# DecaYale/RSLO

Hardware: AMD Instinct MI355X
Metric: frame-pairs/sec fwd+bwd (synthetic KITTI-shaped ~122k-pt scans) (higher is better)
Workload: dtype f32; 1 GPU; C3: full fwd+bwd (voxelize + GU encoder + BEV head/vote + chamfer/ICP loss + Adam step), bs=4 frame pairs/GPU, fp32, 64-ring scans (~122412 pts/frame), dp1; frame_pairs_per_gpu=4, points_per_frame=122412, voxelize_in_step=True, voxelize_prefetch_stream=True, distinct_batches=3, optimizer_in_step=True, head_graph=fwd

## Files before the change

### include/rslo_hip.h

```cpp
#ifndef RSLO_HIP_H_
#define RSLO_HIP_H_

#include <stddef.h>
#include <stdint.h>

#ifdef __cplusplus
extern "C" {
#endif

#if defined(__GNUC__)
#define RSLO_API __attribute__((visibility("default")))
#else
#define RSLO_API
#endif

#define RSLO_OK 0
#define RSLO_EINVAL (-1)
#define RSLO_ELAUNCH (-2)
#define RSLO_ERANGE (-3)
#define RSLO_EWS (-4)

RSLO_API int rslo_abi_version(void);
RSLO_API const char *rslo_last_error(void);

RSLO_API size_t rslo_voxelize_ws_bytes(int64_t P);
RSLO_API int rslo_voxelize(const float *points, int64_t P, int F, const float *h_range6,
                  const float *h_vsize3, const int32_t *h_grid_xyz, int T, int max_voxels,
                  void *ws, size_t ws_bytes, float *voxels ,
                  int32_t *coords , int32_t *num_points ,
                  int32_t *d_nvox , void *stream);

RSLO_API int rslo_vfe_mean(const float *voxels , const int32_t *num_points , int64_t M,
                  int T, int F, float *out , void *stream);

RSLO_API int64_t rslo_hash_capacity(int64_t n);
RSLO_API int rslo_hash_build(const int32_t *coords , int64_t N, int B, const int32_t *h_dims3,
                    uint32_t *keys, int32_t *vals, int64_t cap, void *stream);
RSLO_API int rslo_rulebook_subm(const int32_t *coords, int64_t N, int B, const int32_t *h_dims3,
                       const int32_t *h_ks3, const uint32_t *keys, const int32_t *vals, int64_t cap,
                       int32_t *nbr , void *stream);
RSLO_API int64_t rslo_conv_bitmap_words(int B, const int32_t *h_out_dims3);
RSLO_API size_t rslo_scan_ws_bytes(int64_t n);
RSLO_API int rslo_conv_out_count(const int32_t *coords_in, int64_t N, int B, const int32_t *h_ks3,
                        const int32_t *h_stride3, const int32_t *h_pad3, const int32_t *h_out_dims3,
                        uint32_t *bitmap , int32_t *word_prefix , int64_t words,
                        void *scan_ws, size_t scan_ws_bytes, int32_t *d_count , void *stream);
RSLO_API int rslo_conv_out_coords(const uint32_t *bitmap, const int32_t *word_prefix, int64_t words, int B,
                         const int32_t *h_out_dims3, int32_t *out_coords , int64_t M,
                         void *stream);
RSLO_API int rslo_rulebook_conv(const int32_t *coords_out, int64_t M, int B, const int32_t *h_in_dims3,
                       const int32_t *h_ks3, const int32_t *h_stride3, const int32_t *h_pad3,
                       const uint32_t *in_keys, const int32_t *in_vals, int64_t in_cap,
                       int32_t *nbr , void *stream);
RSLO_API int rslo_rulebook_conv_T(const int32_t *coords_in, int64_t N, int B, const int32_t *h_out_dims3,
                         const int32_t *h_ks3, const int32_t *h_stride3, const int32_t *h_pad3,
                         const uint32_t *out_keys, const int32_t *out_vals, int64_t out_cap,
                         int32_t *nbrT , void *stream);

RSLO_API int rslo_spconv_fwd(const float *in, int cin, const float *W, const float *bias, const int32_t *nbr,
                    const int32_t *row_order, int64_t n_out, int K, int cout, int flip_k, float act_slope,
                    float *out, const int32_t *n_live_dev, void *stream);
RSLO_API int rslo_spconv_dgrad(const float *dout, int cout, const float *W, const int32_t *nbrT,
                      const int32_t *row_order, int64_t n_in, int K, int cin, int flip_k, float *din, void *stream);
RSLO_API int rslo_weight_transpose(const float *W, int K, int cin, int cout, float *Wt, void *stream);
RSLO_API size_t rslo_weight_split_bytes(int K, int cin, int cout);
RSLO_API int rslo_weight_split(const float *W, int K, int cin_op, int cout_op, int transpose, void *Ws, void *stream);
typedef struct {
  const float *W;
  void *ws_fwd;
  void *ws_dgrad;
  int32_t K, cin, cout;
} RsloWeightSplitDesc;
RSLO_API int rslo_weight_split_many(const RsloWeightSplitDesc *desc_dev, int n_layers, int64_t max_weight_elems,
                                    void *stream);
RSLO_API int rslo_spconv_fwd_split(const float *in, int cin, const void *Ws, const float *bias, const int32_t *nbr,
                                   const int32_t *row_order, int64_t n_out, int K, int cout, int flip_k,
                                   float act_slope, float *out, const int32_t *n_live_dev, void *stream);
RSLO_API int rslo_tuning_set(const char *name, int value);
RSLO_API int rslo_tuning_get(const char *name, int *value);
RSLO_API const char *rslo_tuning_name(int index);
RSLO_API int rslo_weight_to_bf16(const float *W, int K, int cin_op, int cout_op, int transpose, void *Wb, void *stream);
RSLO_API int rslo_spconv_fwd_bf16(const void *in, int cin, const void *Wb, const float *bias, const int32_t *nbr,
                                  const int32_t *row_order, int64_t n_out, int K, int cout, int flip_k,
                                  float act_slope, void *out, void *stream);
RSLO_API int64_t rslo_leaky_bwd_colsum_bf16_blocks(int64_t rows, int cols);
RSLO_API int rslo_leaky_bwd_colsum_bf16(const void *y, const void *dout, int64_t rows, int cols, float slope, void *g,
                                        float *partial, void *stream);
RSLO_API int rslo_spconv_wgrad_pairs_bf16(const void *in, int cin, const void *dout, int cout, const int32_t *pairs_in,
                                          const int32_t *pairs_out, const int32_t *koff, int64_t n_out, int K, void *ws,
                                          size_t ws_bytes, float *dW, float *dbias, const float *bias_partial,
                                          int n_bias_partial, void *stream);
RSLO_API size_t rslo_spconv_wgrad_ws_bytes(int64_t n_out, int K, int cin, int cout);
RSLO_API int rslo_spconv_wgrad(const float *in, int cin, const float *dout, int cout, const int32_t *nbr,
                      int64_t n_out, int K, void *ws, size_t ws_bytes, float *dW ,
                      float *dbias , void *stream);
RSLO_API int rslo_rulebook_row_order(const int32_t *nbr, int64_t n_rows, int K, int flip_k, int32_t *order,
                                     void *stream);
RSLO_API size_t rslo_rulebook_pairs_ws_bytes(int64_t n_rows, int K);
RSLO_API int rslo_rulebook_pairs(const int32_t *nbr, int64_t n_rows, int K, void *ws, size_t ws_bytes,
                        int32_t *pairs_in, int32_t *pairs_out, int32_t *koff , void *stream);
RSLO_API int rslo_tq_normalize_fwd(const float *tq, int B, int64_t cells, float *out, void *stream);
RSLO_API int rslo_tq_normalize_bwd(const float *tq, const float *grad, int B, int64_t cells, float *dtq, void *stream);
RSLO_API int rslo_conf_softmax_fwd(const float *t_logit, const float *r_logit, const unsigned char *outside, int B,
                                   int cells, float temperature, float *t_conf, float *r_conf, float *conf_temp,
                                   void *stream);
RSLO_API int rslo_conf_softmax_bwd(const float *t_conf, const float *r_conf, const float *g_t, const float *g_r,
                                   const unsigned char *outside, int B, int cells, float *d_t_logit, float *d_r_logit,
                                   void *stream);
typedef struct {
  const float *mask;
  const float *conf;
  const float *tq, *tq_g;
  const float *pred[3];
  float *w[4];
  float *occ[4];
  float *mpred[3];
  float *mtq, *mtq_g;
  int32_t B, H, W, levels;
} RsloHeadMasks;
typedef struct {
  const float *mask;
  const float *occ[4];
  const float *g_mpred[3];
  const float *g_mtq;
  float *d_pred[3];
  float *d_tq;
  int32_t B, H, W, levels;
} RsloHeadMasksBwd;
RSLO_API int rslo_head_masks_fwd(const RsloHeadMasks *h_a, void *stream);
RSLO_API int rslo_head_masks_bwd(const RsloHeadMasksBwd *h_a, void *stream);
RSLO_API int rslo_cat_upsample_fwd(const float *a, const float *b, int B, int Ca, int Cb, int H, int W, int scale, float *out,
                                   void *stream);
RSLO_API int rslo_cat_upsample_bwd(const float *grad, int B, int Ca, int Cb, int H, int W, int scale, float *da, float *db,
                                   void *stream);
RSLO_API int rslo_pose_tail_fwd(const float *odom, int B, float *t, float *r, void *stream);
RSLO_API int rslo_pose_tail_bwd(const float *odom, const float *g_t, const float *g_r, int B, float *d_odom, void *stream);

#define RSLO_LOSS_TAIL_MAX_LEVELS 8
#define RSLO_LOSS_TAIL_ALPHA_STRIDE 4
typedef struct {
  const float *t_pred, *t_tgt;
  const float *q_pred, *q_tgt;
  const float *alpha_T, *alpha_R;
  const float *pyr_loss_b;
  const float *alpha_pT, *alpha_pR;
  const float *pair_loss;
  const float *alpha_C;
  int32_t B, L, n_pairs, reserved;
  float w_T, w_R, w_pT, w_pR;
  float c_scale;
  float level_w[RSLO_LOSS_TAIL_MAX_LEVELS];
} RsloLossTail;
RSLO_API int rslo_loss_tail_fwd(const RsloLossTail *h_p, float *out5, void *stream);
RSLO_API int rslo_loss_tail_bwd(const RsloLossTail *h_p, const float *grad_out , float *d_t ,
                                float *d_q , float *d_pyr , float *d_pair ,
                                float *d_alpha5 , void *stream);

#define RSLO_PLAN_MAX_LEVELS 8
#define RSLO_PLAN_MAX_CLOUDS 64
#define RSLO_PLAN_CNT_OVERFLOW 0
#define RSLO_PLAN_CNT_ROWS 1
#define RSLO_PLAN_CNT_RAW 9
#define RSLO_PLAN_CNT_NVOX 32
#define RSLO_PLAN_CNT_BASE 96
#define RSLO_PLAN_CNT_BOFF 176
#define RSLO_PLAN_CNT_WORDS (176 + RSLO_PLAN_MAX_LEVELS * (RSLO_PLAN_MAX_CLOUDS + 1))
typedef struct {
  int32_t n_levels;
  int32_t dims0[3];
  int32_t subm_ks[RSLO_PLAN_MAX_LEVELS][3];
  int32_t conv_ks[RSLO_PLAN_MAX_LEVELS][3], conv_stride[RSLO_PLAN_MAX_LEVELS][3], conv_pad[RSLO_PLAN_MAX_LEVELS][3];
  int32_t want_pairs, want_orders;
  float range6[6], vsize3[3];
  int32_t grid_xyz[3], max_points, max_voxels, n_features;
  int64_t cap_rows[RSLO_PLAN_MAX_LEVELS];
} RsloEncoderSpec;
typedef struct {
  uint64_t total_bytes;
  int32_t dims[RSLO_PLAN_MAX_LEVELS][3];
  int64_t cap_rows[RSLO_PLAN_MAX_LEVELS], hash_cap[RSLO_PLAN_MAX_LEVELS];
  uint64_t counts_off;
  uint64_t voxels_off, num_points_off;
  uint64_t coords_frame_off;
  uint64_t coords_off[RSLO_PLAN_MAX_LEVELS];
  uint64_t keys_off[RSLO_PLAN_MAX_LEVELS], vals_off[RSLO_PLAN_MAX_LEVELS];
  uint64_t subm_nbr_off[RSLO_PLAN_MAX_LEVELS], subm_pin_off[RSLO_PLAN_MAX_LEVELS], subm_pout_off[RSLO_PLAN_MAX_LEVELS],
      subm_koff_off[RSLO_PLAN_MAX_LEVELS];
  uint64_t conv_nbr_off[RSLO_PLAN_MAX_LEVELS], conv_nbrT_off[RSLO_PLAN_MAX_LEVELS], conv_order_off[RSLO_PLAN_MAX_LEVELS],
      conv_pin_off[RSLO_PLAN_MAX_LEVELS], conv_pout_off[RSLO_PLAN_MAX_LEVELS], conv_koff_off[RSLO_PLAN_MAX_LEVELS];
  int64_t scratch_words;
  uint64_t vox_ws_off, bitmap_off, prefix_off, scan_ws_off, pair_ws_off;
  uint64_t keys_end_off;
  uint64_t bitmap_level_off[RSLO_PLAN_MAX_LEVELS], bitmap_end_off;
} RsloPlanLayout;
RSLO_API int rslo_plan_encoder_layout(const RsloEncoderSpec *h_spec, int n_clouds, const int64_t *h_n_points,
                                      RsloPlanLayout *h_layout);
RSLO_API int rslo_plan_encoder(const RsloEncoderSpec *h_spec, const RsloPlanLayout *h_layout, int n_clouds,
                               int clouds_per_frame, const float *const *h_points ,
                               const int64_t *h_n_points, void *arena, size_t arena_bytes,
                               int32_t *h_counts , void *stream);

RSLO_API int rslo_plan_encoder_pad_tails(const RsloEncoderSpec *h_spec, const RsloPlanLayout *h_layout, void *arena,
                                         void *stream);

RSLO_API size_t rslo_spconv_wgrad_pairs_ws_bytes(int64_t n_out, int K, int cin, int cout);
RSLO_API int rslo_spconv_wgrad_pairs(const float *in, int cin, const float *dout, int cout, const int32_t *pairs_in,
                            const int32_t *pairs_out, const int32_t *koff, int64_t n_out, int K, void *ws,
                            size_t ws_bytes, float *dW , float *dbias ,
                            const float *bias_partial ,
                            int n_bias_partial, void *stream);
RSLO_API int rslo_leaky_bwd(const float *y, const float *dout, int64_t n, float slope, float *g, void *stream);
RSLO_API int64_t rslo_leaky_bwd_colsum_blocks(int64_t rows, int cols);
RSLO_API int rslo_leaky_bwd_colsum(const float *y, const float *dout, int64_t rows, int cols, float slope, float *g,
                                   float *partial, void *stream);

RSLO_API size_t rslo_segbn_ws_bytes(int S, int64_t max_seg_len, int C);
RSLO_API int rslo_segbn_fwd(const float *x, int C, const int32_t *seg_off, int S, int64_t max_seg_len,
                   const float *gamma, const float *beta, float *running_mean ,
                   float *running_var , float momentum, float eps, float act_slope, void *ws,
                   size_t ws_bytes, float *y, float *save_mean, float *save_invstd, void *stream);
RSLO_API int rslo_bn1d_eval_act(const float *x, int64_t n, int C, const float *running_mean, const float *running_var,
                                const float *gamma, const float *beta, float eps, float act_slope, const int32_t *n_live_dev,
                                float *y, void *stream);
RSLO_API int rslo_segbn_bwd(const float *x, const float *y, const float *gy, int C, const int32_t *seg_off, int S,
                   int64_t max_seg_len, const float *gamma, const float *save_mean, const float *save_invstd,
                   float act_slope, void *ws, size_t ws_bytes, float *gx, float *dgamma, float *dbeta,
                   void *stream);

RSLO_API int rslo_dense_scatter(const float *feat, const int32_t *coords, int64_t M, int C, int B,
                       const int32_t *h_dims3, float *out, void *stream);
RSLO_API int rslo_dense_gather(const float *dense, const int32_t *coords, int64_t M, int C, int B,
                      const int32_t *h_dims3, float *dfeat, void *stream);
RSLO_API int rslo_dense_scatter_frames(const float *feat, const int32_t *coords, int64_t M, int C, int B, int frames,
                                       const int32_t *h_dims3, float *out, void *stream);
RSLO_API int rslo_dense_gather_frames(const float *dense, const int32_t *coords, int64_t M, int C, int B, int frames,
                                      const int32_t *h_dims3, float *dfeat, void *stream);
RSLO_API int rslo_bev_channel_sums(const float *in, int B, int G, int Cg, int64_t HW, float *out, void *stream);
RSLO_API int rslo_bev_channel_sums_masks(const float *in, int B, int G, int Cg, int64_t HW, float *out, float *mask_f,
                                         unsigned char *mask_b, unsigned char *outside_b, void *stream);
RSLO_API size_t rslo_bev_display_ws_bytes(int T);
RSLO_API int rslo_bev_display(const float *sums, int B, int T, int Cg, int64_t HW, float *mask, float *disp, void *ws,
                              size_t ws_bytes, void *stream);

RSLO_API size_t rslo_chamfer_ws_bytes(int B, int N, int M);
RSLO_API int rslo_chamfer_nn(const float *xyz1 , const float *xyz2 , int B, int N, int M,
                    float *dist , int32_t *idx , void *ws, size_t ws_bytes,
                    void *stream);
RSLO_API int rslo_chamfer_nn_ragged(const float *xyz1, const float *xyz2, int B, int N, int M, const int32_t *ncnt,
                           const int32_t *mcnt, float *dist, int32_t *idx, void *ws, size_t ws_bytes,
                           void *stream);
RSLO_API int rslo_chamfer_brute_nn(const float *xyz1, const float *xyz2, int B, int N, int M, const int32_t *ncnt,
                                   const int32_t *mcnt, float *dist, int32_t *idx, void *ws, size_t ws_bytes,
                                   void *stream);
RSLO_API size_t rslo_chamfer_grid_ws_bytes(int B, int N, int M);
RSLO_API int rslo_chamfer_grid_nn(const float *xyz1, const float *xyz2, int B, int N, int M, const int32_t *ncnt,
                                  const int32_t *mcnt, float *dist, int32_t *idx, void *ws, size_t ws_bytes,
                                  void *stream);
RSLO_API int rslo_chamfer_grad(const float *xyz1, const float *xyz2, int B, int N, int M,
                      const float *graddist1, const int32_t *idx1, float *gradxyz1 ,
                      float *gradxyz2 , void *stream);

RSLO_API size_t rslo_cov_residual_ws_bytes(int B, int N);
RSLO_API int rslo_cov_residual_fwd(const float *p1, const float *tgt, const float *cov1, const float *cov2,
                          const int32_t *idx, const float *dist, const float *thr, const float *Rd, int B, int N,
                          int M, float reg_weight, void *ws, size_t ws_bytes, float *loss ,
                          float *cnt , void *stream);
RSLO_API int rslo_cov_residual_bwd(const float *p1, const float *tgt, const float *cov1, const float *cov2,
                          const int32_t *idx, const float *dist, const float *thr, const float *Rd,
                          const float *gloss , const float *cnt , int B, int N, int M,
                          float reg_weight, float *gp1 , float *gtgt ,
                          float *gcov1 , float *gcov2 , void *ws, size_t ws_bytes, void *stream);
RSLO_API size_t rslo_cov_residual_bwd_ws_bytes(int B, int N, int M);
RSLO_API size_t rslo_icp_ws_bytes(int B, int N);
RSLO_API int rslo_icp_step(const float *p1, const float *n1, const float *tgt, const int32_t *idx, const float *dist,
                  const float *thr, int B, int N, int M, void *ws, size_t ws_bytes, float *res_r ,
                  float *res_t , float *step_R , float *step_t ,
                  void *stream);
RSLO_API int rslo_icp_step_first(const float *p1, const float *n1, const float *tgt, const int32_t *idx, const float *dist,
                  const float *thr, int B, int N, int M, void *ws, size_t ws_bytes, float *res_r ,
                  float *res_t , float *step_R , float *step_t ,
                  void *stream);
RSLO_API int rslo_roi_threshold(const float *dist, int B, int N, const int32_t *counts, double ratio, float *thr,
                                void *stream);
RSLO_API int rslo_transform_points(const float *x, const float *R, const float *t, int B, int M, float *out,
                          void *stream);
RSLO_API int rslo_transform_rows(const float *x, int row_stride, const float *R, const float *t, int B, int M,
                                 float *out, void *stream);
RSLO_API size_t rslo_transform_rows_bwd_ws_bytes(int B, int M);
RSLO_API int rslo_transform_rows_bwd(const float *x, int row_stride, const float *gout, int B, int M, void *ws,
                                     size_t ws_bytes, int32_t *done, float *dR, float *dt, void *stream);

typedef struct {
  const float *pred;
  const float *mask;
  float *dpred;
  int32_t h, w, mask_channels;
} RsloPyramidLevel;
RSLO_API size_t rslo_pyramid_l2_ws_bytes(const RsloPyramidLevel *h_levels, int n_levels, int B);
RSLO_API int rslo_pyramid_l2_fwd(const RsloPyramidLevel *h_levels, int n_levels, int B, const float *tq, int H0,
                                 int W0, const float *h_origin3, const float *h_vsize3, void *ws, size_t ws_bytes,
                                 int32_t *done, float *loss_b, float *den, void *stream);
RSLO_API int rslo_pyramid_l2_bwd(const RsloPyramidLevel *h_levels, int n_levels, int B, const float *tq, int H0,
                                 int W0, const float *h_origin3, const float *h_vsize3, const float *grad_loss_b,
                                 const float *den, void *stream);

RSLO_API int rslo_pad_rows_fwd(const float *src, int64_t N, int C, const int32_t *off, const int32_t *len, int B,
                               int Lmax, float *out, void *stream);
RSLO_API int rslo_pad_rows_bwd(const float *dout, int64_t N, int C, const int32_t *off, const int32_t *len, int B,
                               int Lmax, float *dsrc, void *stream);
RSLO_API int rslo_pair_rows_fwd(const float *feats, int64_t N, int F, const float *conf, int Cc, const int32_t *off,
                                const int32_t *len, int B, int Lmax, float *xyz, float *nrm, float *cov, void *stream);

RSLO_API size_t rslo_bn2d_ws_bytes(int N, int C, int HW);
RSLO_API int rslo_bn2d_stats(const float *x, int N, int C, int HW, void *ws, size_t ws_bytes, int32_t *done,
                             double *stats, void *stream);
RSLO_API int rslo_bn2d_apply(const float *x, const float *res, const double *stats, const float *gamma,
                             const float *beta, int N, int C, int HW, float eps, float momentum, float act_slope,
                             float *running_mean, float *running_var, float *save_mean, float *save_invstd, float *y,
                             void *stream);
RSLO_API int rslo_bn2d_bwd_reduce(const float *dy, const float *y, const float *x, const float *save_mean,
                                  const float *save_invstd, int N, int C, int HW, float act_slope, int has_act,
                                  void *ws, size_t ws_bytes, int32_t *done, double *red, float *dgamma, float *dbeta,
                                  void *stream);
RSLO_API int rslo_bn2d_bwd_apply(const float *dy, const float *y, const float *x, const float *gamma,
                                 const float *save_mean, const float *save_invstd, const double *red, double count,
                                 const double *count_dev ,
                                 int N, int C, int HW, float act_slope, int has_act, float *dx, float *dres,
                                 void *stream);

RSLO_API int rslo_bn2d_fwd_local(const float *x, const float *res, const float *gamma, const float *beta, int N, int C,
                                 int HW, float eps, float momentum, float act_slope, float *running_mean,
                                 float *running_var, float *save_mean, float *save_invstd, float *y, void *ws,
                                 size_t ws_bytes, void *stream);
RSLO_API int rslo_bn2d_bwd_local(const float *dy, const float *y, const float *x, const float *gamma,
                                 const float *save_mean, const float *save_invstd, int N, int C, int HW,
                                 float act_slope, int has_act, float *dx, float *dres, float *dgamma, float *dbeta,
                                 void *ws, size_t ws_bytes, void *stream);

RSLO_API size_t rslo_vote_ws_bytes(int B, int H, int W);
RSLO_API int rslo_vote_fwd(const float *tq_map, const float *t_conf, const float *r_conf, int B, int H, int W,
                           const float *h_origin3, const float *h_vsize3, void *ws, size_t ws_bytes, int32_t *done,
                           float *tq_map_g, float *odom, float *sums, void *stream);
RSLO_API int rslo_vote_bwd(const float *tq_map, const float *t_conf, const float *r_conf, int B, int H, int W,
                           const float *h_origin3, const float *h_vsize3, const float *odom, const float *sums,
                           const float *g_odom, float *d_tq_map, float *d_t_conf, float *d_r_conf, void *stream);

RSLO_API int rslo_conv2d_wgrad_supported(int cin, int cout, int H, int W, int stride);
RSLO_API size_t rslo_conv2d_wgrad_ws_bytes(int B, int cin, int cout, int H, int W, int stride);
RSLO_API int rslo_conv2d_wgrad(const float *in, const float *dout, int B, int cin, int cout, int H, int W, int stride,
                               float *dW, float *dbias, void *ws, size_t ws_bytes, void *stream);

RSLO_API int rslo_conv2d_fwd_supported(int cin, int cout, int H, int W);
RSLO_API size_t rslo_conv2d_wsplit_bytes(int cin, int cout);
RSLO_API int rslo_conv2d_wsplit(const float *W, int cin, int cout, int transpose, void *Ws, void *stream);
typedef struct {
  const float *W;
  void *ws_fwd;
  void *ws_dgrad;
  int32_t cin, cout;
  int32_t ntap;
  int32_t reserved;
} RsloConv2dSplitDesc;
RSLO_API int rslo_conv2d_wsplit_many(const RsloConv2dSplitDesc *desc_dev, int n_layers, int64_t max_weight_elems,
                                     void *stream);
RSLO_API int rslo_conv2d_fwd(const float *in, const void *Ws, const float *bias, int B, int cin, int cout, int H, int W,
                             float *out, void *stream);
RSLO_API int rslo_conv2d_fwd_add(const float *in, const void *Ws, const float *bias, const float *res, int B, int cin,
                                 int cout, int H, int W, float *out, void *stream);
RSLO_API size_t rslo_opl_bytes(int B, int C, int H, int W);
RSLO_API int rslo_opl_from_nchw(const float *in, int B, int C, int H, int W, void *planes, void *stream);
RSLO_API int rslo_conv2d_fwd_p_supported(int cin, int cout, int H, int W);
RSLO_API int rslo_conv2d_fwd_p(const void *planes, const void *Ws, const float *bias, const float *res ,
                               int B, int cin, int cout, int H, int W, float *out, void *stream);
RSLO_API int rslo_conv2d_s2_supported(int cin, int cout, int ksize);
RSLO_API int rslo_conv2d_wsplit_k(const float *W, int cin, int cout, int ksize, int transpose, void *Ws, void *stream);
RSLO_API int rslo_conv2d_fwd_s2(const float *in, const void *Ws, int B, int cin, int cout, int H, int W, int ksize,
                                float *out, void *stream);
RSLO_API int rslo_conv2d_dgrad_s2(const float *dout, const void *Ws, int B, int cin, int cout, int H, int W, int ksize,
                                  float *din, void *stream);
RSLO_API int rslo_conv2d_dgrad_s2_add(const float *dout, const void *Ws, const float *res, int B, int cin, int cout, int H,
                                      int W, int ksize, float *din, void *stream);
RSLO_API int rslo_conv2d_fwd_bn(const float *in, const void *Ws, const float *bias, const float *scale, const float *shift,
                                const float *res, int B, int cin, int cout, int H, int W, int act, float slope, float *out,
                                void *stream);
RSLO_API int rslo_conv2d_fwd_s2_bn(const float *in, const void *Ws, const float *bias, const float *scale,
                                   const float *shift, const float *res, int B, int cin, int cout, int H, int W, int ksize,
                                   int act, float slope, float *out, void *stream);
typedef struct {
  const float *gamma, *beta;
  const float *mean, *var;
  float *scale, *shift;
  int32_t C;
  float eps;
} RsloBnFoldDesc;
RSLO_API int rslo_bn_fold_many(const RsloBnFoldDesc *desc_dev, int n_layers, int max_c, void *stream);
RSLO_API int rslo_pose_chain(const float *t, const float *q, double *state, int32_t *count, float *rel_rows, double *traj,
                             int cap, void *stream);
RSLO_API int rslo_conv2d_fwd_bf16(const float *in, const void *Ws, const float *bias, int B, int cin, int cout, int H,
                                  int W, float *out, void *stream);
RSLO_API int rslo_conv1x1s2_wgrad_supported(int cin, int cout, int H, int W);
RSLO_API size_t rslo_conv1x1s2_wgrad_ws_bytes(int B, int cin, int cout, int H, int W);
RSLO_API int rslo_conv1x1s2_wgrad(const float *in, const float *dout, int B, int cin, int cout, int H, int W, float *dW,
                                  void *ws, size_t ws_bytes, void *stream);
RSLO_API int rslo_conv2d_fwd_add_bf16(const float *in, const void *Ws, const float *bias, const float *res, int B,
                                      int cin, int cout, int H, int W, float *out, void *stream);
RSLO_API int rslo_conv2d_wgrad_bf16(const float *in, const float *dout, int B, int cin, int cout, int H, int W,
                                    int stride, float *dW, float *dbias, void *ws, size_t ws_bytes, void *stream);

RSLO_API int rslo_conv1x1_supported(int cin, int cout);
RSLO_API int rslo_conv1x1_fwd(const float *x, const float *W, const float *bias, int B, int cin, int cout, int HW,
                              float *out, void *stream);
RSLO_API int rslo_conv1x1_dgrad(const float *dy, const float *W, int B, int cin, int cout, int HW, float *dx, void *stream);
RSLO_API size_t rslo_conv1x1_wgrad_ws_bytes(int B, int cin, int cout, int HW);
RSLO_API int rslo_conv1x1_wgrad(const float *x, const float *dy, int B, int cin, int cout, int HW, float *dW, float *dbias,
                                void *ws, size_t ws_bytes, void *stream);

RSLO_API int rslo_quat_to_rot(const float *q_wxyz, int B, float *R, void *stream);
RSLO_API int rslo_quat_to_rot_bwd(const float *q_wxyz, const float *gR, int B, float *gq, void *stream);
RSLO_API int rslo_pose_targets(const float *res_r, const float *res_t, const float *R_pred, const float *T_pred, int B,
                               float *rot_targets_wxyz, float *trans_targets, void *stream);
RSLO_API int rslo_pose_targets_tq(const float *res_r, const float *res_t, const float *R_pred, const float *T_pred, int B,
                                  float *rot_targets_wxyz, float *trans_targets, float *tq, void *stream);

typedef struct {
  float *param, *grad, *exp_avg, *exp_avg_sq, *step;
  int32_t group;
  int32_t step_offset;
} RsloOptTensor;
typedef struct {
  int32_t tensor, count;
  int64_t offset;
} RsloOptChunk;
typedef struct {
  double lr, beta1, beta2, eps, weight_decay;
} RsloOptGroup;
#define RSLO_OPT_MAX_GROUPS 16
typedef struct {
  RsloOptGroup group[RSLO_OPT_MAX_GROUPS];
} RsloOptHyper;
RSLO_API int rslo_opt_clip_grad_norm(const RsloOptTensor *tensors_dev, const RsloOptChunk *chunks_dev, int n_chunks,
                                     float max_norm, double *partial_ws, float *total_norm, void *stream);
RSLO_API int rslo_opt_adam_step(const RsloOptTensor *tensors_dev, const RsloOptChunk *chunks_dev, int n_chunks,
                                const RsloOptHyper *hyper, float step, void *stream);

typedef struct RsloWgradReduce {
  int32_t kind;
  int32_t n_blocks;
  const void *ws;
  void *dW;
  const void *aux;
  void *dbias;
  const void *koff;
  int32_t p[8];
} RsloWgradReduce;
RSLO_API int rslo_wgrad_reduce_defer(RsloWgradReduce *sink, int capacity, int *count);
RSLO_API int rslo_wgrad_reduce_many(const RsloWgradReduce *reduces, int n, void *stream);

RSLO_API int rslo_peer_create_host(const char *name, int rank, int world, int max_n, void **comm_out);
RSLO_API int rslo_peer_host_unlink(void *comm);
RSLO_API int rslo_peer_ipc_handle_bytes(void);
RSLO_API int rslo_peer_create_device_begin(int rank, int world, int max_n, void **comm_out, void *handle_out);
RSLO_API int rslo_peer_create_device_finish(void *comm, const void *all_handles);
RSLO_API int rslo_peer_set_timeout_ms(void *comm, int ms);
RSLO_API int rslo_peer_allreduce_f64(void *comm, double *t, int n, void *stream);
RSLO_API unsigned long long rslo_peer_status(void *comm, int *peer);
RSLO_API int rslo_peer_wait_samples(void *comm, float *out_us, int max_out);
RSLO_API int rslo_bn2d_peer_supported(int N, int C, int HW);
RSLO_API int rslo_bn2d_fwd_peer(void *comm, const float *x, const float *res, const float *gamma, const float *beta, int N,
                                int C, int HW, float eps, float momentum, float act_slope, float *running_mean,
                                float *running_var, float *save_mean, float *save_invstd, double *count_out, float *y,
                                void *stream);
RSLO_API int rslo_bn2d_bwd_peer(void *comm, const float *dy, const float *y, const float *x, const float *gamma,
                                const float *save_mean, const float *save_invstd, const double *count_all, int N, int C,
                                int HW, float act_slope, int has_act, float *dx, float *dres, float *dgamma, float *dbeta,
                                void *stream);
RSLO_API int rslo_peer_capture_begin(void *comm);
RSLO_API int rslo_peer_capture_end(void *comm, int *n_exchanges);
RSLO_API int rslo_peer_replay_prepare(void *comm, int n_exchanges, void *stream);
RSLO_API int rslo_peer_destroy(void *comm);

RSLO_API size_t rslo_normals_ws_bytes(int N);
RSLO_API int rslo_estimate_normals(const float *points, int stride_floats, int N, float radius, int max_nn,
                                   const float *h_viewpoint3, int zero_vertical, float *normals ,
                                   int32_t *counts , void *ws, size_t ws_bytes, void *stream);

RSLO_API size_t rslo_voxel_downsample_ws_bytes(int N);
RSLO_API int rslo_voxel_downsample(const float *points, int stride_floats, const float *normals ,
                                   int nstride_floats, int N, double voxel_size, float *out ,
                                   int32_t *voxel_of_point , int32_t *npts ,
                                   int32_t *counts , void *ws, size_t ws_bytes, void *stream);

#define RSLO_MAP_MAX_PROBE 128
#define RSLO_MAP_HDR_COUNTERS 8
#define RSLO_MAP_HDR_PRUNE 5
RSLO_API size_t rslo_map_bytes(int64_t capacity);
RSLO_API int rslo_map_reset(void *map, size_t map_bytes, int64_t capacity, double voxel_size, double min_range,
                            double max_range, void *stream);
RSLO_API size_t rslo_map_insert_ws_bytes(int N);
RSLO_API int rslo_map_insert(void *map, size_t map_bytes, const float *points, int stride_floats, int width, int N,
                             const double *pose7, void *ws, size_t ws_bytes, void *stream);
RSLO_API int rslo_map_lookup(const void *map, size_t map_bytes, const float *points, int stride_floats, int N,
                             const double *pose7, int32_t *hits_out , uint64_t *tags_out ,
                             void *stream);
RSLO_API int rslo_map_export(const void *map, size_t map_bytes, int min_hits, const double *center3 ,
                             double radius, float *rows , uint64_t *tags ,
                             int32_t *hits , int64_t max_rows, int64_t *counts , void *stream);
RSLO_API int rslo_map_insert_frames(void *map, size_t map_bytes, const void *store, size_t store_bytes, int64_t capacity,
                                    int K, const double *poses , int n_poses, void *stream);
RSLO_API size_t rslo_map_prune_ws_bytes(int64_t capacity);
RSLO_API int rslo_map_prune(void *map, size_t map_bytes, const double *center3 , double radius,
                            int min_hits, int grace, void *ws, size_t ws_bytes, void *stream);

#define RSLO_MAP_HDR_CARVE 14
RSLO_API int rslo_range_image(const float *points, int stride_floats, int N, int H, int W, double tan_lo, double tan_hi,
                              uint32_t *img , void *stream);
RSLO_API size_t rslo_map_carve_ws_bytes(int64_t capacity);
RSLO_API int rslo_map_carve(void *map, size_t map_bytes, const uint32_t *img , int H, int W, double tan_lo,
                            double tan_hi, const double *pose7 , int win_rows, int win_cols, double margin_abs,
                            double margin_rel, double max_range, int grace, void *ws, size_t ws_bytes, void *stream);

RSLO_API int rslo_map_params(const void *map, size_t map_bytes, double *params3_host, void *stream);
RSLO_API int rslo_map_nearest(const void *map, size_t map_bytes, double voxel_size, const float *points,
                              int stride_floats, int N, const double *pose7, double max_dist, int min_hits,
                              int64_t *tags_out , double *d2_out , float *rows_out ,
                              void *stream);
RSLO_API size_t rslo_map_register_ws_bytes(int N);
RSLO_API int rslo_map_normal_eq(const void *map, size_t map_bytes, double voxel_size, const float *points,
                                int stride_floats, int width, int N, const double *pose7, int metric, double max_dist,
                                int min_hits, double *out29, void *ws, size_t ws_bytes, void *stream);
RSLO_API int rslo_map_register(const void *map, size_t map_bytes, double voxel_size, const float *points,
                               int stride_floats, int width, int N, double *pose7, int iters, int metric,
                               double max_dist, int min_hits, double damping, int min_pairs, double tol_t, double tol_r,
                               double *info , void *ws, size_t ws_bytes, void *stream);
RSLO_API int rslo_map_normal_eq_w(const void *map, size_t map_bytes, double voxel_size, const float *points,
                                  int stride_floats, int width, int N, const double *pose7, int metric, double max_dist,
                                  int min_hits, double robust_scale, double *out29, void *ws, size_t ws_bytes,
                                  void *stream);
RSLO_API int rslo_map_register_w(const void *map, size_t map_bytes, double voxel_size, const float *points,
                                 int stride_floats, int width, int N, double *pose7, int iters, int metric,
                                 double max_dist, int min_hits, double damping, int min_pairs, double tol_t, double tol_r,
                                 double robust_scale, double *info , void *ws, size_t ws_bytes, void *stream);
RSLO_API int rslo_map_register_sched(const void *const *maps , const size_t *map_bytes ,
                                     const double *voxel_sizes , int n_levels,
                                     const double *stages , int n_stages, const float *points,
                                     int stride_floats, int width, int N, double *pose7, int metric, int min_hits,
                                     double damping, int min_pairs, double tol_t, double tol_r,
                                     double *info , void *ws, size_t ws_bytes, void *stream);

RSLO_API size_t rslo_place_bytes(int64_t capacity, int R, int S);
RSLO_API int rslo_place_reset(void *db, size_t db_bytes, int64_t capacity, int R, int S, void *stream);
RSLO_API int rslo_place_describe(const float *points, int stride_floats, int N, int R, int S,
                                 const double *tables , float z_offset, float *D ,
                                 int32_t *key , double *norm , int64_t *counters4, void *stream);
RSLO_API int rslo_place_add(void *db, size_t db_bytes, int64_t capacity, int R, int S, const float *D,
                            const int32_t *key, const double *norm, void *stream);
RSLO_API size_t rslo_place_query_ws_bytes(int64_t capacity);
RSLO_API int rslo_place_query(const void *db, size_t db_bytes, int64_t capacity, int R, int S, const float *Dq,
                              const int32_t *keyq, const double *normq, int64_t exclude_recent, int num_candidates,
                              int top_k, double *out , void *ws, size_t ws_bytes, void *stream);

// ... 94 lines not shown
```

### rslo_amd/capi.py

```python
import ctypes as C
import os

import torch

_HERE = os.path.dirname(os.path.abspath(__file__))
LIB_PATH = os.environ.get("RSLO_HIP_LIB") or os.path.join(_HERE, "librslo_hip.so")
_lib = None

_I3 = C.c_int32 * 3
_F3 = C.c_float * 3
_F6 = C.c_float * 6

_vp, _i, _i64, _sz, _f = C.c_void_p, C.c_int, C.c_int64, C.c_size_t, C.c_float
SIGNATURES = {
    "rslo_abi_version": (C.c_int, []),
    "rslo_last_error": (C.c_char_p, []),
    "rslo_voxelize_ws_bytes": (_sz, [_i64]),
    "rslo_voxelize": (C.c_int, [_vp, _i64, _i, _vp, _vp, _vp, _i, _i, _vp, _sz, _vp, _vp, _vp, _vp, _vp]),
    "rslo_vfe_mean": (C.c_int, [_vp, _vp, _i64, _i, _i, _vp, _vp]),
    "rslo_hash_capacity": (_i64, [_i64]),
    "rslo_hash_build": (C.c_int, [_vp, _i64, _i, _vp, _vp, _vp, _i64, _vp]),
    "rslo_rulebook_subm": (C.c_int, [_vp, _i64, _i, _vp, _vp, _vp, _vp, _i64, _vp, _vp]),
    "rslo_conv_bitmap_words": (_i64, [_i, _vp]),
    "rslo_scan_ws_bytes": (_sz, [_i64]),
    "rslo_conv_out_count": (C.c_int, [_vp, _i64, _i, _vp, _vp, _vp, _vp, _vp, _vp, _i64, _vp, _sz, _vp, _vp]),
    "rslo_conv_out_coords": (C.c_int, [_vp, _vp, _i64, _i, _vp, _vp, _i64, _vp]),
    "rslo_rulebook_conv": (C.c_int, [_vp, _i64, _i, _vp, _vp, _vp, _vp, _vp, _vp, _i64, _vp, _vp]),
    "rslo_rulebook_conv_T": (C.c_int, [_vp, _i64, _i, _vp, _vp, _vp, _vp, _vp, _vp, _i64, _vp, _vp]),
    "rslo_spconv_fwd": (C.c_int, [_vp, _i, _vp, _vp, _vp, _vp, _i64, _i, _i, _i, _f, _vp, _vp, _vp]),
    "rslo_spconv_dgrad": (C.c_int, [_vp, _i, _vp, _vp, _vp, _i64, _i, _i, _i, _vp, _vp]),
    "rslo_weight_transpose": (C.c_int, [_vp, _i, _i, _i, _vp, _vp]),
    "rslo_weight_split_bytes": (_sz, [_i, _i, _i]),
    "rslo_weight_split": (C.c_int, [_vp, _i, _i, _i, _i, _vp, _vp]),
    "rslo_weight_split_many": (C.c_int, [_vp, _i, _i64, _vp]),
    "rslo_spconv_fwd_split": (C.c_int, [_vp, _i, _vp, _vp, _vp, _vp, _i64, _i, _i, _i, C.c_float, _vp, _vp, _vp]),
    "rslo_peer_create_host": (C.c_int, [C.c_char_p, _i, _i, _i, C.POINTER(C.c_void_p)]),
    "rslo_peer_host_unlink": (C.c_int, [_vp]),
    "rslo_peer_ipc_handle_bytes": (C.c_int, []),
    "rslo_peer_create_device_begin": (C.c_int, [_i, _i, _i, C.POINTER(C.c_void_p), _vp]),
    "rslo_peer_create_device_finish": (C.c_int, [_vp, _vp]),
    "rslo_peer_set_timeout_ms": (C.c_int, [_vp, _i]),
    "rslo_peer_allreduce_f64": (C.c_int, [_vp, _vp, _i, _vp]),
    "rslo_peer_status": (C.c_ulonglong, [_vp, C.POINTER(C.c_int)]),
    "rslo_peer_destroy": (C.c_int, [_vp]),
    "rslo_tuning_set": (C.c_int, [C.c_char_p, _i]),
    "rslo_tuning_get": (C.c_int, [C.c_char_p, _vp]),
    "rslo_tuning_name": (C.c_char_p, [_i]),
    "rslo_weight_to_bf16": (C.c_int, [_vp, _i, _i, _i, _i, _vp, _vp]),
    "rslo_spconv_fwd_bf16": (C.c_int, [_vp, _i, _vp, _vp, _vp, _vp, _i64, _i, _i, _i, C.c_float, _vp, _vp]),
    "rslo_spconv_wgrad_ws_bytes": (_sz, [_i64, _i, _i, _i]),
    "rslo_spconv_wgrad": (C.c_int, [_vp, _i, _vp, _i, _vp, _i64, _i, _vp, _sz, _vp, _vp, _vp]),
    "rslo_rulebook_row_order": (C.c_int, [_vp, _i64, _i, _i, _vp, _vp]),
    "rslo_leaky_bwd_colsum_bf16_blocks": (_i64, [_i64, _i]),
    "rslo_leaky_bwd_colsum_bf16": (C.c_int, [_vp, _vp, _i64, _i, C.c_float, _vp, _vp, _vp]),
    "rslo_spconv_wgrad_pairs_bf16": (C.c_int, [_vp, _i, _vp, _i, _vp, _vp, _vp, _i64, _i, _vp, _sz, _vp, _vp, _vp, _i,
                                               _vp]),
    "rslo_rulebook_pairs_ws_bytes": (_sz, [_i64, _i]),
    "rslo_rulebook_pairs": (C.c_int, [_vp, _i64, _i, _vp, _sz, _vp, _vp, _vp, _vp]),
    "rslo_spconv_wgrad_pairs_ws_bytes": (_sz, [_i64, _i, _i, _i]),
    "rslo_spconv_wgrad_pairs": (C.c_int, [_vp, _i, _vp, _i, _vp, _vp, _vp, _i64, _i, _vp, _sz, _vp, _vp, _vp, _i, _vp]),
    "rslo_leaky_bwd_colsum_blocks": (_i64, [_i64, _i]),
    "rslo_leaky_bwd_colsum": (C.c_int, [_vp, _vp, _i64, _i, C.c_float, _vp, _vp, _vp]),
    "rslo_leaky_bwd": (C.c_int, [_vp, _vp, _i64, _f, _vp, _vp]),
    "rslo_segbn_ws_bytes": (_sz, [_i, _i64, _i]),
    "rslo_segbn_fwd": (C.c_int, [_vp, _i, _vp, _i, _i64, _vp, _vp, _vp, _vp, _f, _f, _f, _vp, _sz, _vp, _vp, _vp, _vp]),
    "rslo_segbn_bwd": (C.c_int, [_vp, _vp, _vp, _i, _vp, _i, _i64, _vp, _vp, _vp, _f, _vp, _sz, _vp, _vp, _vp, _vp]),
    "rslo_dense_scatter": (C.c_int, [_vp, _vp, _i64, _i, _i, _vp, _vp, _vp]),
    "rslo_dense_gather": (C.c_int, [_vp, _vp, _i64, _i, _i, _vp, _vp, _vp]),
    "rslo_dense_scatter_frames": (C.c_int, [_vp, _vp, _i64, _i, _i, _i, _vp, _vp, _vp]),
    "rslo_dense_gather_frames": (C.c_int, [_vp, _vp, _i64, _i, _i, _i, _vp, _vp, _vp]),
    "rslo_bev_channel_sums": (C.c_int, [_vp, _i, _i, _i, _i64, _vp, _vp]),
    "rslo_chamfer_ws_bytes": (_sz, [_i, _i, _i]),
    "rslo_chamfer_nn": (C.c_int, [_vp, _vp, _i, _i, _i, _vp, _vp, _vp, _sz, _vp]),
    "rslo_chamfer_nn_ragged": (C.c_int, [_vp, _vp, _i, _i, _i, _vp, _vp, _vp, _vp, _vp, _sz, _vp]),
    "rslo_chamfer_brute_nn": (C.c_int, [_vp, _vp, _i, _i, _i, _vp, _vp, _vp, _vp, _vp, _sz, _vp]),
    "rslo_chamfer_grid_ws_bytes": (_sz, [_i, _i, _i]),
    "rslo_chamfer_grid_nn": (C.c_int, [_vp, _vp, _i, _i, _i, _vp, _vp, _vp, _vp, _vp, _sz, _vp]),
    "rslo_chamfer_grad": (C.c_int, [_vp, _vp, _i, _i, _i, _vp, _vp, _vp, _vp, _vp]),
    "rslo_cov_residual_ws_bytes": (_sz, [_i, _i]),
    "rslo_cov_residual_fwd": (C.c_int, [_vp] * 8 + [_i, _i, _i, _f, _vp, _sz, _vp, _vp, _vp]),
    "rslo_cov_residual_bwd": (C.c_int, [_vp] * 10 + [_i, _i, _i, _f, _vp, _vp, _vp, _vp, _vp, _sz, _vp]),
    "rslo_cov_residual_bwd_ws_bytes": (_sz, [_i, _i, _i]),
    "rslo_icp_ws_bytes": (_sz, [_i, _i]),
    "rslo_icp_step": (C.c_int, [_vp] * 6 + [_i, _i, _i, _vp, _sz, _vp, _vp, _vp, _vp, _vp]),
    "rslo_icp_step_first": (C.c_int, [_vp] * 6 + [_i, _i, _i, _vp, _sz, _vp, _vp, _vp, _vp, _vp]),
    "rslo_transform_points": (C.c_int, [_vp, _vp, _vp, _i, _i, _vp, _vp]),
    "rslo_transform_rows": (C.c_int, [_vp, _i, _vp, _vp, _i, _i, _vp, _vp]),
    "rslo_transform_rows_bwd_ws_bytes": (_sz, [_i, _i]),
    "rslo_transform_rows_bwd": (C.c_int, [_vp, _i, _vp, _i, _i, _vp, _sz, _vp, _vp, _vp, _vp]),
    "rslo_bn2d_ws_bytes": (_sz, [_i, _i, _i]),
    "rslo_bn2d_stats": (C.c_int, [_vp, _i, _i, _i, _vp, _sz, _vp, _vp, _vp]),
    "rslo_bn2d_apply": (C.c_int, [_vp, _vp, _vp, _vp, _vp, _i, _i, _i, C.c_float, C.c_float, C.c_float, _vp, _vp, _vp,
                                  _vp, _vp, _vp]),
    "rslo_bn2d_bwd_reduce": (C.c_int, [_vp, _vp, _vp, _vp, _vp, _i, _i, _i, C.c_float, _i, _vp, _sz, _vp, _vp, _vp, _vp,
                                       _vp]),
    "rslo_bn2d_bwd_apply": (C.c_int, [_vp, _vp, _vp, _vp, _vp, _vp, _vp, C.c_double, _vp, _i, _i, _i, C.c_float, _i, _vp,
                                      _vp, _vp]),
    "rslo_bn2d_fwd_local": (C.c_int, [_vp, _vp, _vp, _vp, _i, _i, _i, C.c_float, C.c_float, C.c_float, _vp, _vp, _vp, _vp,
                                      _vp, _vp, _sz, _vp]),
    "rslo_bn2d_bwd_local": (C.c_int, [_vp, _vp, _vp, _vp, _vp, _vp, _i, _i, _i, C.c_float, _i, _vp, _vp, _vp, _vp, _vp,
                                      _sz, _vp]),
    "rslo_roi_threshold": (C.c_int, [_vp, _i, _i, _vp, C.c_double, _vp, _vp]),
    "rslo_vote_ws_bytes": (_sz, [_i, _i, _i]),
    "rslo_vote_fwd": (C.c_int, [_vp, _vp, _vp, _i, _i, _i, _vp, _vp, _vp, _sz, _vp, _vp, _vp, _vp, _vp]),
    "rslo_vote_bwd": (C.c_int, [_vp, _vp, _vp, _i, _i, _i, _vp, _vp, _vp, _vp, _vp, _vp, _vp, _vp, _vp]),
    "rslo_conv2d_wgrad_supported": (C.c_int, [_i, _i, _i, _i, _i]),
    "rslo_conv2d_wgrad_ws_bytes": (_sz, [_i, _i, _i, _i, _i, _i]),
    "rslo_conv1x1s2_wgrad_supported": (C.c_int, [_i, _i, _i, _i]),
    "rslo_conv1x1s2_wgrad_ws_bytes": (_sz, [_i, _i, _i, _i, _i]),
    "rslo_conv1x1s2_wgrad": (C.c_int, [_vp, _vp, _i, _i, _i, _i, _i, _vp, _vp, _sz, _vp]),
    "rslo_conv2d_wgrad": (C.c_int, [_vp, _vp, _i, _i, _i, _i, _i, _i, _vp, _vp, _vp, _sz, _vp]),
    "rslo_conv2d_fwd_supported": (C.c_int, [_i, _i, _i, _i]),
    "rslo_conv2d_wsplit_bytes": (_sz, [_i, _i]),
    "rslo_conv2d_wsplit": (C.c_int, [_vp, _i, _i, _i, _vp, _vp]),
    "rslo_conv2d_wsplit_k": (C.c_int, [_vp, _i, _i, _i, _i, _vp, _vp]),
    "rslo_conv2d_s2_supported": (C.c_int, [_i, _i, _i]),
    "rslo_conv2d_fwd_s2": (C.c_int, [_vp, _vp, _i, _i, _i, _i, _i, _i, _vp, _vp]),
    "rslo_conv2d_dgrad_s2": (C.c_int, [_vp, _vp, _i, _i, _i, _i, _i, _i, _vp, _vp]),
    "rslo_conv2d_wsplit_many": (C.c_int, [_vp, _i, _i64, _vp]),
    "rslo_conv2d_fwd": (C.c_int, [_vp, _vp, _vp, _i, _i, _i, _i, _i, _vp, _vp]),
    "rslo_conv2d_fwd_bf16": (C.c_int, [_vp, _vp, _vp, _i, _i, _i, _i, _i, _vp, _vp]),
    "rslo_cat_upsample_fwd": (C.c_int, [_vp, _vp, _i, _i, _i, _i, _i, _i, _vp, _vp]),
    "rslo_cat_upsample_bwd": (C.c_int, [_vp, _i, _i, _i, _i, _i, _i, _vp, _vp, _vp]),
    "rslo_bev_channel_sums_masks": (C.c_int, [_vp, _i, _i, _i, C.c_int64, _vp, _vp, _vp, _vp, _vp]),
    "rslo_pose_tail_fwd": (C.c_int, [_vp, _i, _vp, _vp, _vp]),
    "rslo_pose_tail_bwd": (C.c_int, [_vp, _vp, _vp, _i, _vp, _vp]),
    "rslo_bev_display_ws_bytes": (_sz, [_i]),
    "rslo_bev_display": (C.c_int, [_vp, _i, _i, _i, C.c_int64, _vp, _vp, _vp, _sz, _vp]),
    "rslo_conv2d_dgrad_s2_add": (C.c_int, [_vp, _vp, _vp, _i, _i, _i, _i, _i, _i, _vp, _vp]),
    "rslo_conv2d_fwd_add": (C.c_int, [_vp, _vp, _vp, _vp, _i, _i, _i, _i, _i, _vp, _vp]),
    "rslo_conv2d_fwd_add_bf16": (C.c_int, [_vp, _vp, _vp, _vp, _i, _i, _i, _i, _i, _vp, _vp]),
    "rslo_conv2d_wgrad_bf16": (C.c_int, [_vp, _vp, _i, _i, _i, _i, _i, _i, _vp, _vp, _vp, _sz, _vp]),
    "rslo_conv1x1_supported": (C.c_int, [_i, _i]),
    "rslo_conv1x1_fwd": (C.c_int, [_vp, _vp, _vp, _i, _i, _i, _i, _vp, _vp]),
    "rslo_conv1x1_dgrad": (C.c_int, [_vp, _vp, _i, _i, _i, _i, _vp, _vp]),
    "rslo_conv1x1_wgrad_ws_bytes": (_sz, [_i, _i, _i, _i]),
    "rslo_conv1x1_wgrad": (C.c_int, [_vp, _vp, _i, _i, _i, _i, _vp, _vp, _vp, _sz, _vp]),
    "rslo_quat_to_rot": (C.c_int, [_vp, _i, _vp, _vp]),
    "rslo_quat_to_rot_bwd": (C.c_int, [_vp, _vp, _i, _vp, _vp]),
    "rslo_pose_targets": (C.c_int, [_vp, _vp, _vp, _vp, _i, _vp, _vp, _vp]),
    "rslo_pose_targets_tq": (C.c_int, [_vp, _vp, _vp, _vp, _i, _vp, _vp, _vp, _vp]),
    "rslo_pair_rows_fwd": (C.c_int, [_vp, _i64, _i, _vp, _i, _vp, _vp, _i, _i, _vp, _vp, _vp, _vp]),
    "rslo_pad_rows_fwd": (C.c_int, [_vp, _i64, _i, _vp, _vp, _i, _i, _vp, _vp]),
    "rslo_pad_rows_bwd": (C.c_int, [_vp, _i64, _i, _vp, _vp, _i, _i, _vp, _vp]),
    "rslo_pyramid_l2_ws_bytes": (_sz, [_vp, _i, _i]),
    "rslo_pyramid_l2_fwd": (C.c_int, [_vp, _i, _i, _vp, _i, _i, _vp, _vp, _vp, _sz, _vp, _vp, _vp, _vp]),
    "rslo_pyramid_l2_bwd": (C.c_int, [_vp, _i, _i, _vp, _i, _i, _vp, _vp, _vp, _vp, _vp]),
    "rslo_plan_encoder_layout": (C.c_int, [_vp, _i, _vp, _vp]),
    "rslo_plan_encoder_pad_tails": (C.c_int, [_vp, _vp, _vp, _vp]),
    "rslo_plan_encoder": (C.c_int, [_vp, _vp, _i, _i, _vp, _vp, _vp, _sz, _vp, _vp]),
    "rslo_tq_normalize_fwd": (C.c_int, [_vp, _i, _i64, _vp, _vp]),
    "rslo_tq_normalize_bwd": (C.c_int, [_vp, _vp, _i, _i64, _vp, _vp]),
    "rslo_conf_softmax_fwd": (C.c_int, [_vp, _vp, _vp, _i, _i, _f, _vp, _vp, _vp, _vp]),
    "rslo_conf_softmax_bwd": (C.c_int, [_vp, _vp, _vp, _vp, _vp, _i, _i, _vp, _vp, _vp]),
    "rslo_head_masks_fwd": (C.c_int, [_vp, _vp]),
    "rslo_head_masks_bwd": (C.c_int, [_vp, _vp]),
    "rslo_loss_tail_fwd": (C.c_int, [_vp, _vp, _vp]),
    "rslo_loss_tail_bwd": (C.c_int, [_vp, _vp, _vp, _vp, _vp, _vp, _vp, _vp]),
    "rslo_peer_wait_samples": (C.c_int, [_vp, _vp, _i]),
    "rslo_bn1d_eval_act": (C.c_int, [_vp, _i64, _i, _vp, _vp, _vp, _vp, _f, _f, _vp, _vp, _vp]),
    "rslo_wgrad_reduce_defer": (C.c_int, [_vp, _i, _vp]),
    "rslo_wgrad_reduce_many": (C.c_int, [_vp, _i, _vp]),
    "rslo_peer_capture_begin": (C.c_int, [_vp]),
    "rslo_peer_capture_end": (C.c_int, [_vp, _vp]),
    "rslo_peer_replay_prepare": (C.c_int, [_vp, _i, _vp]),
    "rslo_bn2d_peer_supported": (C.c_int, [_i, _i, _i]),
    "rslo_bn2d_fwd_peer": (C.c_int, [_vp, _vp, _vp, _vp, _vp, _i, _i, _i, C.c_float, C.c_float, C.c_float, _vp, _vp, _vp, _vp,
                                     _vp, _vp, _vp]),
    "rslo_bn2d_bwd_peer": (C.c_int, [_vp, _vp, _vp, _vp, _vp, _vp, _vp, _vp, _i, _i, _i, C.c_float, _i, _vp, _vp, _vp, _vp,
                                     _vp]),
    "rslo_opl_bytes": (_sz, [_i, _i, _i, _i]),
    "rslo_opl_from_nchw": (C.c_int, [_vp, _i, _i, _i, _i, _vp, _vp]),
    "rslo_conv2d_fwd_p_supported": (C.c_int, [_i, _i, _i, _i]),
    "rslo_conv2d_fwd_p": (C.c_int, [_vp, _vp, _vp, _vp, _i, _i, _i, _i, _i, _vp, _vp]),
    "rslo_opt_clip_grad_norm": (C.c_int, [_vp, _vp, _i, _f, _vp, _vp, _vp]),
    "rslo_opt_adam_step": (C.c_int, [_vp, _vp, _i, _vp, _f, _vp]),
    "rslo_conv2d_fwd_bn": (C.c_int, [_vp] * 6 + [_i, _i, _i, _i, _i, _i, _f, _vp, _vp]),
    "rslo_conv2d_fwd_s2_bn": (C.c_int, [_vp] * 6 + [_i, _i, _i, _i, _i, _i, _i, _f, _vp, _vp]),
    "rslo_bn_fold_many": (C.c_int, [_vp, _i, _i, _vp]),
    "rslo_pose_chain": (C.c_int, [_vp, _vp, _vp, _vp, _vp, _vp, _i, _vp]),
    "rslo_normals_ws_bytes": (_sz, [_i]),
    "rslo_estimate_normals": (C.c_int, [_vp, _i, _i, _f, _i, _vp, _i, _vp, _vp, _vp, _sz, _vp]),
    "rslo_voxel_downsample_ws_bytes": (_sz, [_i]),
    "rslo_voxel_downsample": (C.c_int, [_vp, _i, _vp, _i, _i, C.c_double, _vp, _vp, _vp, _vp, _vp, _sz, _vp]),
    "rslo_map_bytes": (_sz, [_i64]),
    "rslo_map_reset": (C.c_int, [_vp, _sz, _i64, C.c_double, C.c_double, C.c_double, _vp]),
    "rslo_map_insert_ws_bytes": (_sz, [_i]),
    "rslo_map_insert": (C.c_int, [_vp, _sz, _vp, _i, _i, _i, _vp, _vp, _sz, _vp]),
    "rslo_map_lookup": (C.c_int, [_vp, _sz, _vp, _i, _i, _vp, _vp, _vp, _vp]),
    "rslo_map_export": (C.c_int, [_vp, _sz, _i, _vp, C.c_double, _vp, _vp, _vp, _i64, _vp, _vp]),
    "rslo_map_insert_frames": (C.c_int, [_vp, _sz, _vp, _sz, _i64, _i, _vp, _i, _vp]),
    "rslo_map_prune_ws_bytes": (_sz, [_i64]),
    "rslo_map_prune": (C.c_int, [_vp, _sz, _vp, C.c_double, _i, _i, _vp, _sz, _vp]),
    "rslo_range_image": (C.c_int, [_vp, _i, _i, _i, _i, C.c_double, C.c_double, _vp, _vp]),
    "rslo_map_carve_ws_bytes": (_sz, [_i64]),
    "rslo_map_carve": (C.c_int, [_vp, _sz, _vp, _i, _i, C.c_double, C.c_double, _vp, _i, _i, C.c_double, C.c_double,
                                 C.c_double, _i, _vp, _sz, _vp]),
    "rslo_map_params": (C.c_int, [_vp, _sz, _vp, _vp]),
    "rslo_map_nearest": (C.c_int, [_vp, _sz, C.c_double, _vp, _i, _i, _vp, C.c_double, _i, _vp, _vp, _vp, _vp]),
    "rslo_map_register_ws_bytes": (_sz, [_i]),
    "rslo_map_normal_eq": (C.c_int, [_vp, _sz, C.c_double, _vp, _i, _i, _i, _vp, _i, C.c_double, _i, _vp, _vp, _sz, _vp]),
    "rslo_map_register": (C.c_int, [_vp, _sz, C.c_double, _vp, _i, _i, _i, _vp, _i, _i, C.c_double, _i, C.c_double, _i,
                                    C.c_double, C.c_double, _vp, _vp, _sz, _vp]),
    "rslo_map_normal_eq_w": (C.c_int, [_vp, _sz, C.c_double, _vp, _i, _i, _i, _vp, _i, C.c_double, _i, C.c_double, _vp, _vp,
                                       _sz, _vp]),
    "rslo_map_register_w": (C.c_int, [_vp, _sz, C.c_double, _vp, _i, _i, _i, _vp, _i, _i, C.c_double, _i, C.c_double, _i,
                                      C.c_double, C.c_double, C.c_double, _vp, _vp, _sz, _vp]),
    "rslo_map_register_sched": (C.c_int, [_vp, _vp, _vp, _i, _vp, _i, _vp, _i, _i, _i, _vp, _i, _i, C.c_double, _i,
                                          C.c_double, C.c_double, _vp, _vp, _sz, _vp]),
    "rslo_place_bytes": (_sz, [_i64, _i, _i]),
    "rslo_place_reset": (C.c_int, [_vp, _sz, _i64, _i, _i, _vp]),
    "rslo_place_describe": (C.c_int, [_vp, _i, _i, _i, _i, _vp, _f, _vp, _vp, _vp, _vp, _vp]),
    "rslo_place_add": (C.c_int, [_vp, _sz, _i64, _i, _i, _vp, _vp, _vp, _vp]),
    "rslo_place_query_ws_bytes": (_sz, [_i64]),
    "rslo_place_query": (C.c_int, [_vp, _sz, _i64, _i, _i, _vp, _vp, _vp, _i64, _i, _i, _vp, _vp, _sz, _vp]),
    "rslo_posegraph_ws_bytes": (_sz, [_i, _i]),
    "rslo_posegraph_optimize": (C.c_int, [_vp, _vp, _i, _vp, _vp, _vp, _vp, _vp, _i, _i, _i] + [C.c_double] * 5 +
                                [_vp, _vp, _sz, _vp]),
    "rslo_posegraph_cost": (C.c_int, [_vp, _vp, _i, _vp, _vp, _vp, _vp, _vp, _i, C.c_double, _vp, _vp, _sz, _vp]),
    "rslo_posegraph_linearize": (C.c_int, [_vp, _vp, _i, _vp, _vp, _vp, _vp, _vp, _i, C.c_double, _vp, _vp, _vp, _vp, _sz,
                                           _vp]),
    "rslo_posegraph_matvec": (C.c_int, [_vp, _vp, _i, _i, C.c_double, _vp, _sz, _vp]),
    "rslo_posegraph_chain_solve": (C.c_int, [_vp, _vp, _i, _i, _vp, _sz, _vp]),
    "rslo_pose_between": (C.c_int, [_vp, _vp, _i, _vp, _vp]),
    "rslo_keyframe_bytes": (_sz, [_i64, _i]),
    "rslo_keyframe_reset": (C.c_int, [_vp, _sz, _i64, _i, _vp]),
    "rslo_keyframe_prepare_ws_bytes": (_sz, [_i]),
    "rslo_keyframe_prepare": (C.c_int, [_vp, _i, _i, _i, C.c_double, C.c_double, C.c_double, _vp, _vp, _vp, _sz, _vp]),
    "rslo_keyframe_add": (C.c_int, [_vp, _sz, _i64, _i, _vp, _vp, _vp]),
    "rslo_loop_verify": (C.c_int, [_vp, _sz, _i64, _i, _vp, _vp, _vp, _i, _vp, _vp, _i] + [C.c_double] * 4 +
                         [_i, C.c_double, _vp, _vp, _vp, _vp]),
    "rslo_loop_edges_reset": (C.c_int, [_vp, _vp, _vp, _vp, _i, _vp]),
    "rslo_loop_emit": (C.c_int, [_vp, _i, _vp, _sz, _i64, _i, _vp, _vp, _vp, _vp, _i, C.c_double, C.c_double, _vp]),
    "rslo_surfel_bytes": (_sz, [_i64]),
    "rslo_surfel_reset": (C.c_int, [_vp, _sz, _i64, C.c_double, C.c_double, C.c_double, _i, C.c_double, C.c_double, _vp]),
    "rslo_surfel_insert_ws_bytes": (_sz, [_i]),
    "rslo_surfel_insert": (C.c_int, [_vp, _sz, _vp, _i, _i, _vp, _vp, _sz, _vp]),
    "rslo_surfel_insert_frames": (C.c_int, [_vp, _sz, _vp, _sz, _i64, _i, _vp, _i, _vp]),
    "rslo_surfel_export": (C.c_int, [_vp, _sz, _i, _vp, C.c_double, _vp, _vp, _vp, _i64, _vp, _vp]),
    "rslo_surfel_nearest": (C.c_int, [_vp, _sz, C.c_double, _vp, _i, _i, _vp, C.c_double, _vp, _vp, _vp, _vp]),
    "rslo_surfel_prune_ws_bytes": (_sz, [_i64]),
    "rslo_surfel_prune": (C.c_int, [_vp, _sz, _vp, C.c_double, C.c_double, _i, _vp, _sz, _vp]),
    "rslo_surfel_register_ws_bytes": (_sz, [_i]),
    "rslo_surfel_normal_eq": (C.c_int, [_vp, _sz, C.c_double, _vp, _i, _i, _vp, C.c_double, C.c_double, _vp, _vp, _sz, _vp]),
    "rslo_surfel_register": (C.c_int, [_vp, _sz, C.c_double, _vp, _i, _i, _vp, _i, C.c_double, C.c_double, _i, C.c_double,
                                       C.c_double, C.c_double, _vp, _vp, _sz, _vp]),
    "rslo_surfel_nearest_d": (C.c_int, [_vp, _sz, C.c_double, _vp, _i, _i, _vp, C.c_double, _i, C.c_double, C.c_double, _vp,
                                        _vp, _vp, _vp, _vp]),
    "rslo_surfel_normal_eq_d": (C.c_int, [_vp, _sz, C.c_double, _vp, _i, _i, _vp, C.c_double, _i, C.c_double, C.c_double,
                                          C.c_double, _vp, _vp, _sz, _vp]),
    "rslo_surfel_register_d": (C.c_int, [_vp, _sz, C.c_double, _vp, _i, _i, _vp, _i, C.c_double, C.c_double, _i, C.c_double,
                                         C.c_double, C.c_double, _i, C.c_double, C.c_double, _vp, _vp, _sz, _vp]),
    "rslo_deskew": (C.c_int, [_vp, _i, _i, _i, _i, _vp, _vp, _vp, _vp, C.c_double, C.c_double, _i, C.c_double, _vp, _i, _vp,
                              _vp]),
}


class RsloHipError(RuntimeError):
    pass


def lib():
    global _lib
    if _lib is None:
        if not os.path.exists(LIB_PATH):
            raise RsloHipError(
                "librslo_hip.so not found at %s -- build it with `python -m rslo_amd.build` "
                "(there is no CPU fallback for the RSLO hot path)" % LIB_PATH)
        l = C.CDLL(LIB_PATH)
        for name, (res, args) in SIGNATURES.items():
            fn = getattr(l, name)
            fn.restype = res
            fn.argtypes = args
        _lib = l
    return _lib if _proxy is None else _proxy


_proxy = None


def probe_streams(on, points_only=None):
    global _proxy
    from rslo_amd import streamprobe
    if on:
        _proxy = streamprobe.LibProxy(lib() if _proxy is None else _proxy._lib, SIGNATURES, points_only)
        streamprobe.start()
    else:
        streamprobe.stop()
        _proxy = None


def tuning_set(name, value):
    _chk(lib().rslo_tuning_set(name.encode(), int(value)), "rslo_tuning_set")


def tuning_get(name):
    v = C.c_int(0)
    _chk(lib().rslo_tuning_get(name.encode(), C.byref(v)), "rslo_tuning_get")
    return v.value


class tuning:

    def __init__(self, **kw):
        self.kw, self.old = kw, {}

    def __enter__(self):
        for k, v in self.kw.items():
            self.old[k] = tuning_get(k)
            tuning_set(k, v)
        return self

    def __exit__(self, *exc):
        for k, v in self.old.items():
            tuning_set(k, v)
        return False


def _chk(rc, name):
    if rc != 0:
        raise RsloHipError("%s failed (%d): %s" % (name, rc, lib().rslo_last_error().decode()))


_raw_stream = getattr(torch._C, "_cuda_getCurrentRawStream", None)
_raw_device = getattr(torch._C, "_cuda_getDevice", None)


def _stream():
    if _raw_stream is not None and _raw_device is not None:
        return _raw_stream(_raw_device())
    return torch.cuda.current_stream().cuda_stream


def _ptr(t, dtype=None, name="tensor"):
    if t is None:
        return None
    if not t.is_cuda:
        raise RsloHipError("%s must live on the GPU (the RSLO hot path has no CPU fallback)" % name)
    if dtype is not None and t.dtype != dtype:
        raise RsloHipError("%s must be %s, got %s" % (name, dtype, t.dtype))
    if not t.is_contiguous():
        raise RsloHipError("%s must be contiguous" % name)
    return t.data_ptr()


def _dp(t):
    return None if t is None else t.data_ptr()


def _i3(x):
    return _I3(*[int(v) for v in x])


def _ws(nbytes, device):
    return torch.empty((max(int(nbytes), 16),), dtype=torch.uint8, device=device)


class RsloWgradReduce(C.Structure):
    _fields_ = [("kind", C.c_int32), ("n_blocks", C.c_int32), ("ws", C.c_void_p), ("dW", C.c_void_p), ("aux", C.c_void_p),
                ("dbias", C.c_void_p), ("koff", C.c_void_p), ("p", C.c_int32 * 8)]


import threading as _threading
_tls = _threading.local()


class ReduceSink:
    CAP = 256

    def __init__(self):
        self.arr = (RsloWgradReduce * self.CAP)()
        self.count = C.c_int(0)
        self.keep = []

    class _Collect:
        def __init__(self, sink):
            self.sink = sink

        def __enter__(self):
            self.prev = getattr(_tls, "sink", None)
# ... 259 lines not shown
                                    _ptr(order, torch.int32, "order"), n_out, K, cout_op,
                                    int(flip_k), float(act_slope), _ptr(out), _stream()), "rslo_spconv_fwd_bf16")
    return out


def _splittable(cin, cout):
    return SPLIT_BF16 and cin in (32, 64) and cout in (32, 64)


def spconv_fwd(x, W, bias, nbr, flip_k=False, act_slope=1.0, order=None, n_live=None):
    n_out, K = nbr.shape
    Kw, cin, cout = W.shape
    if Kw != K or x.shape[1] != cin:
        raise RsloHipError("spconv_fwd: shape mismatch x%s W%s nbr%s" % (tuple(x.shape), tuple(W.shape), tuple(nbr.shape)))
    if _splittable(cin, cout):
        return spconv_fwd_split(x, weight_split(W), bias, nbr, cin, cout, flip_k, act_slope, order, n_live)
    return spconv_fwd_direct(x, W, bias, nbr, flip_k, act_slope, order, n_live)


def spconv_fwd_direct(x, W, bias, nbr, flip_k=False, act_slope=1.0, order=None, n_live=None):
    n_out, K = nbr.shape
    Kw, cin, cout = W.shape
    out = torch.empty((n_out, cout), dtype=torch.float32, device=x.device)
    _chk(lib().rslo_spconv_fwd(_ptr(x, torch.float32, "x"), cin, _ptr(W, torch.float32, "W"),
                               _ptr(bias, torch.float32, "bias"), _ptr(nbr, torch.int32, "nbr"),
                               _ptr(order, torch.int32, "order"), n_out, K, cout,
                               int(flip_k), float(act_slope), _ptr(out),
                               _ptr(n_live, torch.int32, "n_live") if order is None else None, _stream()),
         "rslo_spconv_fwd")
    return out


def weight_transpose(W):
    K, cin, cout = W.shape
    Wt = torch.empty((K, cout, cin), dtype=torch.float32, device=W.device)
    _chk(lib().rslo_weight_transpose(_ptr(W, torch.float32, "W"), K, cin, cout, _ptr(Wt), _stream()),
         "rslo_weight_transpose")
    return Wt


def spconv_dgrad(dout, W, nbrT, flip_k=False, order=None):
    Kw, cin, cout = W.shape
    if _splittable(cout, cin):
        return spconv_fwd_split(dout, weight_split(W, transpose=True), None, nbrT, cout, cin, flip_k, order=order)
    if cin % 16 == 0 and cout % 16 == 0:
        return spconv_fwd(dout, weight_transpose(W), None, nbrT, flip_k=flip_k, order=order)
    return spconv_dgrad_direct(dout, W, nbrT, flip_k, order)


def spconv_dgrad_direct(dout, W, nbrT, flip_k=False, order=None):
    n_in, K = nbrT.shape
    Kw, cin, cout = W.shape
    if Kw != K or dout.shape[1] != cout:
        raise RsloHipError("spconv_dgrad: shape mismatch")
    din = torch.empty((n_in, cin), dtype=torch.float32, device=dout.device)
    _chk(lib().rslo_spconv_dgrad(_ptr(dout, torch.float32, "dout"), cout, _ptr(W, torch.float32, "W"),
                                 _ptr(nbrT, torch.int32, "nbrT"), _ptr(order, torch.int32, "order"), n_in, K, cin,
                                 int(flip_k), _ptr(din), _stream()), "rslo_spconv_dgrad")
    return din


def spconv_wgrad(x, dout, nbr, cin, cout, with_bias=True):
    n_out, K = nbr.shape
    dev = x.device
    dW = torch.empty((K, cin, cout), dtype=torch.float32, device=dev)
    db = torch.empty((cout,), dtype=torch.float32, device=dev) if with_bias else None
    wsb = lib().rslo_spconv_wgrad_ws_bytes(n_out, K, cin, cout)
    ws = _ws(wsb, dev)
    _chk(lib().rslo_spconv_wgrad(_ptr(x, torch.float32, "x"), cin, _ptr(dout, torch.float32, "dout"), cout,
                                 _ptr(nbr, torch.int32, "nbr"), n_out, K, _ptr(ws), wsb, _ptr(dW), _ptr(db),
                                 _stream()), "rslo_spconv_wgrad")
    return dW, db


def rulebook_pairs(nbr):
    n, K = nbr.shape
    dev = nbr.device
    cap = max(n * K, 1)
    pin = torch.empty((cap,), dtype=torch.int32, device=dev)
    pout = torch.empty((cap,), dtype=torch.int32, device=dev)
    koff = torch.empty((K + 1,), dtype=torch.int32, device=dev)
    wsb = lib().rslo_rulebook_pairs_ws_bytes(n, K)
    ws = _ws(wsb, dev)
    _chk(lib().rslo_rulebook_pairs(_ptr(nbr, torch.int32, "nbr"), n, K, _ptr(ws), wsb, _ptr(pin), _ptr(pout),
                                   _ptr(koff), _stream()), "rslo_rulebook_pairs")
    return pin, pout, koff


def spconv_wgrad_pairs(x, dout, pairs, n_out, K, cin, cout, with_bias=True, bias_partial=None):
    pin, pout, koff = pairs
    dev = x.device
    dW = torch.empty((K, cin, cout), dtype=torch.float32, device=dev)
    db = torch.empty((cout,), dtype=torch.float32, device=dev) if with_bias else None
    wsb = lib().rslo_spconv_wgrad_pairs_ws_bytes(n_out, K, cin, cout)
    ws = _ws(wsb, dev)
    _chk(lib().rslo_spconv_wgrad_pairs(_ptr(x, torch.float32, "x"), cin, _ptr(dout, torch.float32, "dout"), cout,
                                       _ptr(pin, torch.int32, "pairs_in"), _ptr(pout, torch.int32, "pairs_out"),
                                       _ptr(koff, torch.int32, "koff"), n_out, K, _ptr(ws), wsb, _ptr(dW), _ptr(db),
                                       _ptr(bias_partial if with_bias else None),
                                       0 if bias_partial is None else bias_partial.shape[0], _stream()),
         "rslo_spconv_wgrad_pairs")
    _keep_for_reduce(ws, bias_partial, koff)
    return dW, db


def leaky_bwd(y, dout, slope, colsum=False):
    g = torch.empty_like(dout)
    if colsum:
        rows, cols = dout.shape
        if cols >= 4 and 1024 % cols == 0:
            nblk = int(lib().rslo_leaky_bwd_colsum_blocks(rows, cols))
            part = torch.empty((nblk, cols), dtype=torch.float32, device=dout.device)
            _chk(lib().rslo_leaky_bwd_colsum(_ptr(y, torch.float32, "y"), _ptr(dout, torch.float32, "dout"), rows, cols,
                                             float(slope), _ptr(g), _ptr(part), _stream()), "rslo_leaky_bwd_colsum")
            return g, part
        colsum = None
    _chk(lib().rslo_leaky_bwd(_ptr(y, torch.float32, "y"), _ptr(dout, torch.float32, "dout"), y.numel(),
                              float(slope), _ptr(g), _stream()), "rslo_leaky_bwd")
    return (g, None) if colsum is None else g


def leaky_bwd_bf16(y, dout, slope, colsum=False):
    rows, cols = dout.shape
    g = torch.empty_like(dout)
    part = None
    if colsum:
        nblk = int(lib().rslo_leaky_bwd_colsum_bf16_blocks(rows, cols))
        part = torch.empty((nblk, cols), dtype=torch.float32, device=dout.device)
    _chk(lib().rslo_leaky_bwd_colsum_bf16(_ptr(y, torch.bfloat16, "y"), _ptr(dout, torch.bfloat16, "dout"), rows, cols,
                                          float(slope), _ptr(g), _ptr(part), _stream()), "rslo_leaky_bwd_colsum_bf16")
    return (g, part) if colsum else g


def spconv_wgrad_pairs_bf16(x, dout, pairs, n_out, K, cin, cout, bias_partial=None):
    pin, pout, koff = pairs
    dev = x.device
    dW = torch.empty((K, cin, cout), dtype=torch.float32, device=dev)
    db = torch.empty((cout,), dtype=torch.float32, device=dev) if bias_partial is not None else None
    wsb = lib().rslo_spconv_wgrad_pairs_ws_bytes(n_out, K, cin, cout)
    ws = _ws(wsb, dev)
    _chk(lib().rslo_spconv_wgrad_pairs_bf16(_ptr(x, torch.bfloat16, "x"), cin, _ptr(dout, torch.bfloat16, "dout"), cout,
                                            _ptr(pin, torch.int32, "pairs_in"), _ptr(pout, torch.int32, "pairs_out"),
                                            _ptr(koff, torch.int32, "koff"), n_out, K, _ptr(ws), wsb, _ptr(dW), _ptr(db),
                                            _ptr(bias_partial), 0 if bias_partial is None else bias_partial.shape[0],
                                            _stream()), "rslo_spconv_wgrad_pairs_bf16")
    _keep_for_reduce(ws, bias_partial, koff)
    return dW, db


def segbn_fwd(x, seg_off, S, max_len, gamma, beta, running_mean, running_var, momentum, eps, act_slope):
    n, Cc = x.shape
    dev = x.device
    y = torch.empty_like(x)
    mean = torch.empty((S, Cc), dtype=torch.float32, device=dev)
    invstd = torch.empty((S, Cc), dtype=torch.float32, device=dev)
    wsb = lib().rslo_segbn_ws_bytes(S, max_len, Cc)
    ws = _ws(wsb, dev)
    _chk(lib().rslo_segbn_fwd(_ptr(x, torch.float32, "x"), Cc, _ptr(seg_off, torch.int32, "seg_off"), S, max_len,
                              _ptr(gamma, torch.float32, "gamma"), _ptr(beta, torch.float32, "beta"),
                              _ptr(running_mean, torch.float32, "running_mean"),
                              _ptr(running_var, torch.float32, "running_var"), float(momentum), float(eps),
                              float(act_slope), _ptr(ws), wsb, _ptr(y), _ptr(mean), _ptr(invstd), _stream()),
         "rslo_segbn_fwd")
    return y, mean, invstd


def bn1d_eval_act(x, running_mean, running_var, gamma, beta, eps, act_slope=1.0, n_live=None):
    n, Cc = x.shape
    y = torch.empty_like(x)
    _chk(lib().rslo_bn1d_eval_act(_ptr(x, torch.float32, "x"), n, Cc, _ptr(running_mean, torch.float32, "running_mean"),
                                  _ptr(running_var, torch.float32, "running_var"), _ptr(gamma, torch.float32, "gamma"),
                                  _ptr(beta, torch.float32, "beta"), float(eps), float(act_slope),
                                  _ptr(n_live, torch.int32, "n_live"), _ptr(y), _stream()), "rslo_bn1d_eval_act")
    return y


def segbn_bwd(x, y, gy, seg_off, S, max_len, gamma, mean, invstd, act_slope):
    n, Cc = x.shape
    dev = x.device
    gx = torch.empty_like(x)
    dgamma = torch.empty((Cc,), dtype=torch.float32, device=dev)
    dbeta = torch.empty((Cc,), dtype=torch.float32, device=dev)
    wsb = lib().rslo_segbn_ws_bytes(S, max_len, Cc) + 2 * S * Cc * 4
    ws = _ws(wsb, dev)
    _chk(lib().rslo_segbn_bwd(_ptr(x, torch.float32, "x"), _ptr(y, torch.float32, "y"), _ptr(gy, torch.float32, "gy"),
                              Cc, _ptr(seg_off, torch.int32, "seg_off"), S, max_len,
                              _ptr(gamma, torch.float32, "gamma"), _ptr(mean), _ptr(invstd), float(act_slope),
                              _ptr(ws), wsb, _ptr(gx), _ptr(dgamma), _ptr(dbeta), _stream()), "rslo_segbn_bwd")
    return gx, dgamma, dbeta


def dense_scatter(feat, coords, batch, dims, frames=1, out=None):
    M, Cc = feat.shape
    shape = (batch, Cc, dims[0], dims[1], dims[2]) if frames == 1 else (batch // frames, frames, Cc, dims[0], dims[1], dims[2])
    if out is not None:
        n = 1
        for v in shape:
            n *= int(v)
        if not (out.is_contiguous() and out.dtype == torch.float32 and out.device == feat.device and out.numel() == n):
            raise RsloHipError("dense_scatter: `out` must be a contiguous fp32 buffer of %d elements on %s" % (n, feat.device))
        strides, acc = [], 1
        for v in reversed(shape):
            strides.append(acc)
            acc *= int(v)
        out = torch.empty(0, dtype=torch.float32, device=feat.device).set_(out.untyped_storage(), out.storage_offset(), shape,
                                                                          tuple(reversed(strides)))
    else:
        out = torch.empty(shape, dtype=torch.float32, device=feat.device)
    _chk(lib().rslo_dense_scatter_frames(_ptr(feat, torch.float32, "feat"), _ptr(coords, torch.int32, "coords"), M, Cc,
                                         int(batch), int(frames), _i3(dims), _ptr(out), _stream()), "rslo_dense_scatter")
    return out


def dense_gather(dense, coords, C_, batch, dims, frames=1):
    M = coords.shape[0]
    out = torch.empty((M, C_), dtype=torch.float32, device=dense.device)
    _chk(lib().rslo_dense_gather_frames(_ptr(dense, torch.float32, "dense"), _ptr(coords, torch.int32, "coords"), M, C_,
                                        int(batch), int(frames), _i3(dims), _ptr(out), _stream()), "rslo_dense_gather")
    return out


def bev_channel_sums(bev, groups, masks=False):
    B, Ct, H, W = bev.shape
    out = torch.empty((B, groups, H, W), dtype=torch.float32, device=bev.device)
    if masks:
        mf = torch.empty((B, 1, H, W), dtype=torch.float32, device=bev.device)
        mb = torch.empty((B, 1, H, W), dtype=torch.bool, device=bev.device)
        ob = torch.empty((B, 1, H, W), dtype=torch.bool, device=bev.device)
        _chk(lib().rslo_bev_channel_sums_masks(_ptr(bev, torch.float32, "bev"), B, int(groups), Ct // int(groups), H * W,
                                               _ptr(out), _ptr(mf), _ptr(mb), _ptr(ob), _stream()),
             "rslo_bev_channel_sums_masks")
        return out, mf, mb, ob
    _chk(lib().rslo_bev_channel_sums(_ptr(bev, torch.float32, "bev"), B, int(groups), Ct // int(groups), H * W, _ptr(out),
                                     _stream()), "rslo_bev_channel_sums")
    return out


def pose_tail_fwd(odom):
    B = odom.shape[0]
    t = torch.empty((B, 3), dtype=torch.float32, device=odom.device)
    r = torch.empty((B, 4), dtype=torch.float32, device=odom.device)
    _chk(lib().rslo_pose_tail_fwd(_ptr(odom, torch.float32, "odom"), B, _ptr(t), _ptr(r), _stream()), "rslo_pose_tail_fwd")
    return t, r


def pose_tail_bwd(odom, g_t, g_r):
    B = odom.shape[0]
    d = torch.empty((B, 7), dtype=torch.float32, device=odom.device)
    _chk(lib().rslo_pose_tail_bwd(_ptr(odom, torch.float32, "odom"), _dp(g_t), _dp(g_r), B, _ptr(d), _stream()),
         "rslo_pose_tail_bwd")
    return d


def cat_upsample_fwd(a, b, scale):
    B, Ca, H, W = a.shape
    Cb = b.shape[1]
    if tuple(b.shape) != (B, Cb, H, W):
        raise ValueError("cat_upsample_fwd: shapes %s / %s" % (tuple(a.shape), tuple(b.shape)))
    out = torch.empty((B, Ca + Cb, H * scale, W * scale), dtype=torch.float32, device=a.device)
    _chk(lib().rslo_cat_upsample_fwd(_ptr(a, torch.float32, "a"), _ptr(b, torch.float32, "b"), B, Ca, Cb, H, W, int(scale),
                                     _ptr(out), _stream()), "rslo_cat_upsample_fwd")
    return out


def cat_upsample_bwd(grad, Ca, Cb, scale, need_a=True, need_b=True):
    B, Ct, Hs, Ws = grad.shape
    H, W = Hs // scale, Ws // scale
    da = torch.empty((B, Ca, H, W), dtype=torch.float32, device=grad.device) if need_a else None
    db = torch.empty((B, Cb, H, W), dtype=torch.float32, device=grad.device) if need_b else None
    _chk(lib().rslo_cat_upsample_bwd(_ptr(grad, torch.float32, "grad"), B, Ca, Cb, H, W, int(scale), _dp(da), _dp(db),
                                     _stream()), "rslo_cat_upsample_bwd")
    return da, db


def bev_display(sums, channels):
    B, T, H, W = sums.shape
    mask = torch.empty((B, 1, H, W), dtype=torch.float32, device=sums.device)
    disp = torch.empty((T, B, 1, H, W), dtype=torch.float32, device=sums.device)
    wsb = lib().rslo_bev_display_ws_bytes(T)
    ws = torch.empty((wsb,), dtype=torch.uint8, device=sums.device)
    _chk(lib().rslo_bev_display(_ptr(sums, torch.float32, "sums"), B, T, int(channels), H * W, _ptr(mask), _ptr(disp),
                                ws.data_ptr(), wsb, _stream()), "rslo_bev_display")
    return mask, list(disp.unbind(0))


def chamfer_nn(xyz1, xyz2, dist=None, idx=None, ncnt=None, mcnt=None, method=None):
    entry = {None: "rslo_chamfer_nn_ragged", "brute": "rslo_chamfer_brute_nn", "grid": "rslo_chamfer_grid_nn"}[method]
    B, N, _ = xyz1.shape
    M = xyz2.shape[1]
    dev = xyz1.device
    if dist is None:
        dist = torch.empty((B, N), dtype=torch.float32, device=dev)
    if idx is None:
        idx = torch.empty((B, N), dtype=torch.int32, device=dev)
    wsb = lib().rslo_chamfer_ws_bytes(B, N, M)
    ws = _ws(wsb, dev)
    _chk(getattr(lib(), entry)(_ptr(xyz1, torch.float32, "xyz1"), _ptr(xyz2, torch.float32, "xyz2"), B, N, M,
                               _ptr(ncnt, torch.int32, "ncnt"), _ptr(mcnt, torch.int32, "mcnt"),
                               _ptr(dist, torch.float32, "dist"), _ptr(idx, torch.int32, "idx"), _ptr(ws), wsb,
                               _stream()), entry)
    return dist, idx


def estimate_normals(points, radius=0.6, max_nn=30, viewpoint=None, zero_vertical=False, out=None, counts=None, ws=None):
    src = _ptr(points, torch.float32, "points")
    if points.dim() != 2 or points.shape[1] < 3:
        raise RsloHipError("estimate_normals: points must be [P, F >= 3], got %s" % (tuple(points.shape),))
    P, F = points.shape
    dev = points.device
    if out is None:
        out = torch.empty((P, 3), dtype=torch.float32, device=dev)
    if counts is None:
        counts = torch.empty((P,), dtype=torch.int32, device=dev)
    if out.shape != (P, 3) or counts.shape != (P,):
        raise RsloHipError("estimate_normals: out must be [P, 3] and counts [P]")
    wsb = lib().rslo_normals_ws_bytes(P)
    if ws is None:
        ws = _ws(wsb, dev)
    vp = None if viewpoint is None else _F3(*[float(v) for v in viewpoint])
    _chk(lib().rslo_estimate_normals(src, F, P, float(radius), int(max_nn), vp, int(bool(zero_vertical)),
                                     _ptr(out, torch.float32, "out"), _ptr(counts, torch.int32, "counts"), _ptr(ws),
                                     ws.numel() * ws.element_size(), _stream()), "rslo_estimate_normals")
    return out, counts


def append_normals(points_xyzi, radius=0.6, max_nn=30, viewpoint=None, out=None, counts=None, ws=None, normals=None):
    _ptr(points_xyzi, torch.float32, "points")
    if points_xyzi.dim() != 2 or points_xyzi.shape[1] not in (3, 4):
        raise RsloHipError("append_normals: a raw scan is [P, 4] (x, y, z, intensity) or [P, 3], got %s"
                           % (tuple(points_xyzi.shape),))
    P, F = points_xyzi.shape
    if out is None:
        out = torch.empty((P, 7), dtype=torch.float32, device=points_xyzi.device)
    if out.dim() != 2 or out.shape[1] != 7 or out.shape[0] < P or not out.is_contiguous():
        raise RsloHipError("append_normals: out must be a contiguous [>= P, 7] buffer")
    cloud = out[:P]
    cloud[:, :F].copy_(points_xyzi)
    if F == 3:
        cloud[:, 3].zero_()
    nrm, _ = estimate_normals(points_xyzi, radius, max_nn, viewpoint, True, out=None if normals is None else normals[:P],
                              counts=None if counts is None else counts[:P], ws=ws)
    cloud[:, 4:].copy_(nrm)
    return cloud


def _rows3(t, name):
    if not t.is_cuda:
        raise RsloHipError("%s must live on the GPU (the RSLO hot path has no CPU fallback)" % name)
    if t.dtype != torch.float32 or t.dim() != 2 or t.shape[1] < 3:
        raise RsloHipError("%s must be fp32 [P, >= 3], got %s %s" % (name, t.dtype, tuple(t.shape)))
    if t.shape[0] > 1 and (t.stride(1) != 1 or t.stride(0) < 3):
        raise RsloHipError("%s: rows must be unit-stride with a row stride >= 3, got strides %s" % (name, t.stride()))
    return t.data_ptr(), (int(t.stride(0)) if t.shape[0] > 1 else max(int(t.shape[1]), 3))


def voxel_downsample(points, normals=None, voxel_size=0.1, *, out=None, index=None, npts=None, counts=None, ws=None,
                     sync=True):
    src, stride = _rows3(points, "points")
    P = points.shape[0]
    dev = points.device
    nsrc, nstride = None, 0
    if normals is not None:
        nsrc, nstride = _rows3(normals, "normals")
        if normals.shape != (P, 3):
            raise RsloHipError("voxel_downsample: normals must be [P, 3], got %s" % (tuple(normals.shape),))
    width = 3 if normals is None else 6
    if out is None:
        out = torch.empty((P, width), dtype=torch.float32, device=dev)
    if out.shape != (P, width):
        raise RsloHipError("voxel_downsample: out must be [P, %d], got %s" % (width, tuple(out.shape)))
    if index is True:
        index = torch.empty((P,), dtype=torch.int32, device=dev)
    if npts is True:
        npts = torch.empty((P,), dtype=torch.int32, device=dev)
    for name, t in (("index", index), ("npts", npts)):
        if t is not None and t.shape != (P,):
            raise RsloHipError("voxel_downsample: %s must be [P]" % name)
    if counts is None:
        counts = torch.empty((2,), dtype=torch.int32, device=dev)
    if counts.shape != (2,):
        raise RsloHipError("voxel_downsample: counts must be [2]")
    if ws is None:
        ws = _ws(lib().rslo_voxel_downsample_ws_bytes(P), dev)
    _chk(lib().rslo_voxel_downsample(src, stride, nsrc, nstride, P, float(voxel_size), _ptr(out, torch.float32, "out"),
                                     _ptr(index, torch.int32, "index"), _ptr(npts, torch.int32, "npts"),
                                     _ptr(counts, torch.int32, "counts"), _ptr(ws), ws.numel() * ws.element_size(),
                                     _stream()), "rslo_voxel_downsample")
    if not sync:
        return out, index, npts, counts
    Q, flags = counts.tolist()
    if flags & 1:
        raise RsloHipError("voxel_downsample: the cloud spans 2^21 or more cells of %g along an axis" % float(voxel_size))
    res = (out[:Q],) + (() if index is None else (index,)) + (() if npts is None else (npts[:Q],))
    return res[0] if len(res) == 1 else res


MAP_HDR_COUNTERS = 8
MAP_COUNTERS = ("n_scans", "n_cells", "n_points", "dropped_invalid", "dropped_range", "dropped_full")


def map_bytes(capacity):
    return int(lib().rslo_map_bytes(int(capacity)))


def _map_buf(buf):
    if not (torch.is_tensor(buf) and buf.is_cuda and buf.dtype == torch.int64 and buf.dim() == 1 and buf.is_contiguous()):
        raise RsloHipError("map: the buffer must be a contiguous int64 CUDA vector of rslo_map_bytes(capacity) bytes")
    return buf.data_ptr(), buf.numel() * 8


def _pose7(pose, name):
    if not (torch.is_tensor(pose) and pose.is_cuda and pose.dtype == torch.float64 and pose.numel() == 7
            and pose.is_contiguous()):
        raise RsloHipError("%s: pose must be 7 contiguous float64 values (t, q wxyz) on the GPU" % name)
    return pose.data_ptr()


def _insert_frames(name, buf, store_buf, capacity, K, poses):
    ptr, nbytes = _map_buf(buf)
    sptr, sbytes = _map_buf(store_buf)
    if not (torch.is_tensor(poses) and poses.is_cuda and poses.dtype == torch.float64 and poses.dim() == 2
            and poses.shape[1] == 7 and poses.is_contiguous()):
        raise RsloHipError("%s: poses must be contiguous float64 [n, 7] rows (t, q wxyz) on the GPU" % name)
    if poses.device != buf.device or store_buf.device != buf.device:
        raise RsloHipError("%s: the map, the store and the poses must live on one device" % name)
    if poses.shape[0] == 0:
        return
    _chk(getattr(lib(), "rslo_" + name)(ptr, nbytes, sptr, sbytes, int(capacity), int(K), poses.data_ptr(),
                                        int(poses.shape[0]), _stream()), "rslo_" + name)


def _prune_ws(name, capacity, device):
    nbytes = int(getattr(lib(), "rslo_%s_bytes" % name)(int(capacity)))
    if nbytes == 0:
        raise RsloHipError("%s: capacity must be a power of two >= 1024, got %r" % (name, capacity))
    return torch.empty((nbytes // 8,), dtype=torch.int64, device=device)


def _center3(name, center, exact):
    if center is None:
        return None
    if not (torch.is_tensor(center) and center.is_cuda and center.dtype == torch.float64 and center.is_contiguous()
            and (center.numel() == 3 if exact else center.numel() >= 3)):
        raise RsloHipError("%s: center must be %s contiguous float64 values on the GPU" % (name, "3" if exact else ">= 3"))
    return center.data_ptr()


def map_reset(buf, capacity, voxel_size, min_range=0.0, max_range=float("inf")):
    ptr, nbytes = _map_buf(buf)
    _chk(lib().rslo_map_reset(ptr, nbytes, int(capacity), float(voxel_size), float(min_range), float(max_range),
                              _stream()), "rslo_map_reset")


def map_insert(buf, points, pose, ws):
    ptr, nbytes = _map_buf(buf)
    src, stride = _rows3(points, "points")
    _chk(lib().rslo_map_insert(ptr, nbytes, src, stride, int(points.shape[1]), int(points.shape[0]),
                               _pose7(pose, "map_insert"), _ptr(ws), ws.numel() * ws.element_size(), _stream()),
         "rslo_map_insert")


def map_insert_frames(buf, store_buf, capacity, K, poses):
    _insert_frames("map_insert_frames", buf, store_buf, capacity, K, poses)


def map_lookup(buf, points, pose, hits=None, tags=None):
    ptr, nbytes = _map_buf(buf)
    src, stride = _rows3(points, "points")
    P = points.shape[0]
    if hits is None:
        hits = torch.empty((P,), dtype=torch.int32, device=points.device)
    if tags is True:
        tags = torch.empty((P,), dtype=torch.int64, device=points.device)
    if hits.shape != (P,) or (tags is not None and tags.shape != (P,)):
        raise RsloHipError("map_lookup: hits and tags must be [P]")
    _chk(lib().rslo_map_lookup(ptr, nbytes, src, stride, P, _pose7(pose, "map_lookup"), _ptr(hits, torch.int32, "hits"),
                               _ptr(tags, torch.int64, "tags"), _stream()), "rslo_map_lookup")
    return hits if tags is None else (hits, tags)


def map_export(buf, min_hits=1, center=None, radius=0.0, rows=None, tags=None, hits=None, counts=None):
    ptr, nbytes = _map_buf(buf)
    R = 0 if rows is None else rows.shape[0]
    if R and (rows.shape != (R, 4) or tags is None or hits is None or tags.shape != (R,) or hits.shape != (R,)):
        raise RsloHipError("map_export: rows [R, 4], tags [R] and hits [R] go together")
    cptr = _center3("map_export", center, exact=True)
    if counts is None:
        counts = torch.empty((2,), dtype=torch.int64, device=buf.device)
    _chk(lib().rslo_map_export(ptr, nbytes, int(min_hits), cptr, float(radius),
                               _ptr(rows, torch.float32, "rows") if R else None,
                               _ptr(tags, torch.int64, "tags") if R else None,
                               _ptr(hits, torch.int32, "hits") if R else None, R,
                               _ptr(counts, torch.int64, "counts"), _stream()), "rslo_map_export")
    return counts


MAP_HDR_PRUNE = 5
MAP_PRUNE_COUNTERS = ("n_prunes", "n_evicted", "n_lost")


def map_prune_ws(capacity, device):
    return _prune_ws("map_prune_ws", capacity, device)


def map_prune(buf, ws, center=None, radius=0.0, min_hits=1, grace=0):
    ptr, nbytes = _map_buf(buf)
    cptr = _center3("map_prune", center, exact=False)
    if not (torch.is_tensor(ws) and ws.is_cuda and ws.is_contiguous()):
        raise RsloHipError("map_prune: ws must be a contiguous CUDA tensor (map_prune_ws)")
    _chk(lib().rslo_map_prune(ptr, nbytes, cptr, float(radius), int(min_hits),
                              int(grace), ws.data_ptr(), ws.numel() * ws.element_size(), _stream()), "rslo_map_prune")


MAP_HDR_CARVE = 14
MAP_CARVE_COUNTERS = ("n_carves", "n_carved")


def _range_img(img, H, W, name):
    if not (torch.is_tensor(img) and img.is_cuda and img.dtype == torch.int32 and img.shape == (int(H), int(W))
            and img.is_contiguous()):
        raise RsloHipError("%s: the image must be a contiguous int32 CUDA [%d, %d] tensor (the uint32 range words)"
                           % (name, H, W))
    return img.data_ptr()


def range_image(points, img, tan_lo, tan_hi):
    src, stride = _rows3(points, "range_image: points")
    H, W = img.shape if torch.is_tensor(img) and img.dim() == 2 else (0, 0)
    N = int(points.shape[0])
    _chk(lib().rslo_range_image(src if N else None, stride, N, int(H), int(W), float(tan_lo), float(tan_hi),
                                _range_img(img, H, W, "range_image"), _stream()), "rslo_range_image")
    return img


def map_carve(buf, ws, img, tan_lo, tan_hi, pose, win_rows=1, win_cols=1, margin_abs=0.3, margin_rel=0.0,
              max_range=60.0, grace=1):
    ptr, nbytes = _map_buf(buf)
    H, W = img.shape if torch.is_tensor(img) and img.dim() == 2 else (0, 0)
    if not (torch.is_tensor(ws) and ws.is_cuda and ws.is_contiguous()):
        raise RsloHipError("map_carve: ws must be a contiguous CUDA tensor (map_prune_ws)")
    _chk(lib().rslo_map_carve(ptr, nbytes, _range_img(img, H, W, "map_carve"), int(H), int(W), float(tan_lo), float(tan_hi),
                              _pose7(pose, "map_carve"), int(win_rows), int(win_cols), float(margin_abs), float(margin_rel),
                              float(max_range), int(grace), ws.data_ptr(), ws.numel() * ws.element_size(), _stream()),
         "rslo_map_carve")


MAP_METRICS = {"point": 0, "plane": 1}


def map_params(buf):
    ptr, nbytes = _map_buf(buf)
    out = (C.c_double * 3)()
    _chk(lib().rslo_map_params(ptr, nbytes, out, _stream()), "rslo_map_params")
    return tuple(out)


def _map_metric(metric):
    if metric not in MAP_METRICS:
        raise RsloHipError("map: metric must be \"point\" or \"plane\", got %r" % (metric,))
    return MAP_METRICS[metric]


def map_nearest(buf, points, pose, voxel_size=None, max_dist=None, min_hits=1, rows=None, tags=None, d2=None):
    ptr, nbytes = _map_buf(buf)
    src, stride = _rows3(points, "points")
    P = points.shape[0]
    if voxel_size is None:
        voxel_size = map_params(buf)[0]
    if tags is None:
        tags = torch.empty((P,), dtype=torch.int64, device=points.device)
    if d2 is None:
        d2 = torch.empty((P,), dtype=torch.float64, device=points.device)
    if rows is True:
        rows = torch.empty((P, 4), dtype=torch.float32, device=points.device)
    if tags.shape != (P,) or d2.shape != (P,) or (rows is not None and rows.shape != (P, 4)):
        raise RsloHipError("map_nearest: tags and d2 must be [P], rows [P, 4]")
    _chk(lib().rslo_map_nearest(ptr, nbytes, float(voxel_size), src, stride, P, _pose7(pose, "map_nearest"),
                                float(voxel_size if max_dist is None else max_dist), int(min_hits),
                                _ptr(tags, torch.int64, "tags"), _ptr(d2, torch.float64, "d2"),
                                _ptr(rows, torch.float32, "rows"), _stream()), "rslo_map_nearest")
    return (tags, d2) if rows is None else (tags, d2, rows)


def map_register_ws(n_points, device):
    return torch.empty((int(lib().rslo_map_register_ws_bytes(int(n_points))) // 8,), dtype=torch.int64, device=device)


def _register_ws(family, ws, P, device):
    if ws is None:
        return (map_register_ws if family == "map" else surfel_register_ws)(P, device)
    if not (ws.is_cuda and ws.is_contiguous()):
        raise RsloHipError("%s: the workspace must be a contiguous CUDA tensor" % family)
    return ws


def _gn_args(name, buf, points, voxel_size, max_dist, result, ws, iters=None):
    family = name.split("_")[0]
    ptr, nbytes = _map_buf(buf)
    src, stride = _rows3(points, "points")
    P = points.shape[0]
    if voxel_size is None and family == "map":
        voxel_size = map_params(buf)[0]
    shape, what = ((29,), "out must be [29]") if iters is None else ((iters, 8), "info must be [iters, 8]")
    if result is None:
        result = torch.empty(tuple(max(n, 0) for n in shape), dtype=torch.float64, device=points.device)
    if result.shape != shape:
# ... 1258 lines not shown
```

### rslo_amd/csrc/chamfer.hip

```cpp
#include "rslo_common.h"

#define CH_THREADS 256
#define CH_QPT 4
#define CH_TILE 2048
#define CH_CHUNK 64

typedef float f32x2 __attribute__((ext_vector_type(2)));

__device__ __forceinline__ f32x2 dist2(f32x2 tx, f32x2 ty, f32x2 tz, float qx, float qy, float qz) {
#pragma clang fp contract(off)
  const f32x2 dx = tx - qx, dy = ty - qy, dz = tz - qz;
  return (dx * dx + dy * dy) + dz * dz;
}

__global__ __launch_bounds__(CH_THREADS) void k_chamfer_part(const float *__restrict__ xyz1,
                                                             const float *__restrict__ xyz2, int N, int M,
                                                             int seg_len, int S, const int32_t *__restrict__ mcnt,
                                                             float *__restrict__ pdist,
                                                             int32_t *__restrict__ pidx) {
  __shared__ f32x2 tx[CH_TILE / 2], ty[CH_TILE / 2], tz[CH_TILE / 2];
  const int b = blockIdx.z, s = blockIdx.y;
  const int Mb = mcnt ? mcnt[b] : M;
  const int m0 = s * seg_len;
  const int m1 = (m0 + seg_len < Mb) ? m0 + seg_len : Mb;
  const float *q = xyz1 + (int64_t)b * N * 3;
  const float *t = xyz2 + (int64_t)b * M * 3;
  const int q0 = blockIdx.x * (CH_THREADS * CH_QPT) + threadIdx.x;
  const float INF = __builtin_inff();

  float qx[CH_QPT], qy[CH_QPT], qz[CH_QPT], best[CH_QPT];
  int bchunk[CH_QPT];
#pragma unroll
  for (int j = 0; j < CH_QPT; ++j) {
    const int qi = q0 + j * CH_THREADS;
    const bool ok = qi < N;
    qx[j] = ok ? q[qi * 3 + 0] : 0.f;
    qy[j] = ok ? q[qi * 3 + 1] : 0.f;
    qz[j] = ok ? q[qi * 3 + 2] : 0.f;
    best[j] = INF;
    bchunk[j] = m0;
  }

  for (int k0 = m0; k0 < m1; k0 += CH_TILE) {
    const int cnt = (m1 - k0 < CH_TILE) ? (m1 - k0) : CH_TILE;
    __syncthreads();
    for (int e = threadIdx.x; e < CH_TILE / 2; e += CH_THREADS) {
      const int a = 2 * e, c = 2 * e + 1;
      const float *pa = t + (int64_t)(k0 + a) * 3, *pc = t + (int64_t)(k0 + c) * 3;
      const bool va = a < cnt, vc = c < cnt;
      tx[e] = (f32x2){va ? pa[0] : INF, vc ? pc[0] : INF};
      ty[e] = (f32x2){va ? pa[1] : INF, vc ? pc[1] : INF};
      tz[e] = (f32x2){va ? pa[2] : INF, vc ? pc[2] : INF};
    }
    __syncthreads();
    const int nchunk = (cnt + CH_CHUNK - 1) / CH_CHUNK;
    for (int c = 0; c < nchunk; ++c) {
      float cmin[CH_QPT];
#pragma unroll
      for (int j = 0; j < CH_QPT; ++j) cmin[j] = INF;
#pragma unroll 8
      for (int e = c * (CH_CHUNK / 2); e < (c + 1) * (CH_CHUNK / 2); ++e) {
        const f32x2 x = tx[e], y = ty[e], z = tz[e];
#pragma unroll
        for (int j = 0; j < CH_QPT; ++j) {
          const f32x2 d = dist2(x, y, z, qx[j], qy[j], qz[j]);
          cmin[j] = fminf(cmin[j], fminf(d.x, d.y));
        }
      }
#pragma unroll
      for (int j = 0; j < CH_QPT; ++j)
        if (cmin[j] < best[j]) {
          best[j] = cmin[j];
          bchunk[j] = k0 + c * CH_CHUNK;
        }
    }
  }

#pragma unroll
  for (int j = 0; j < CH_QPT; ++j) {
    const int qi = q0 + j * CH_THREADS;
    if (qi >= N) continue;
    int bi = m0;
    if (best[j] < INF) {
      const int c0 = bchunk[j];
      const int c1 = (c0 + CH_CHUNK < m1) ? c0 + CH_CHUNK : m1;
      bi = c0;
      for (int k = c1 - 1; k >= c0; --k) {
#pragma clang fp contract(off)
        const float dx = t[(int64_t)k * 3 + 0] - qx[j], dy = t[(int64_t)k * 3 + 1] - qy[j],
                    dz = t[(int64_t)k * 3 + 2] - qz[j];
        const float d = (dx * dx + dy * dy) + dz * dz;
        if (d == best[j]) bi = k;
      }
    }
    pdist[((int64_t)b * S + s) * N + qi] = best[j];
    pidx[((int64_t)b * S + s) * N + qi] = bi;
  }
}

__global__ void k_chamfer_merge(const float *__restrict__ pdist, const int32_t *__restrict__ pidx, int N, int S,
                                const int32_t *__restrict__ ncnt, float *__restrict__ dist,
                                int32_t *__restrict__ idx) {
  const int b = blockIdx.y;
  const int i = blockIdx.x * blockDim.x + threadIdx.x;
  if (i >= N) return;
  if (ncnt && i >= ncnt[b]) {
    dist[(int64_t)b * N + i] = __builtin_inff();
    idx[(int64_t)b * N + i] = 0;
    return;
  }
  float best = pdist[((int64_t)b * S) * N + i];
  int besti = pidx[((int64_t)b * S) * N + i];
  for (int s = 1; s < S; ++s) {
    const float d = pdist[((int64_t)b * S + s) * N + i];
    if (d < best) {
      best = d;
      besti = pidx[((int64_t)b * S + s) * N + i];
    }
  }
  dist[(int64_t)b * N + i] = best;
  idx[(int64_t)b * N + i] = besti;
}

static int chamfer_segments(int B, int N, int M) {
  const int64_t qblocks = rslo_cdiv(N > 0 ? N : 1, CH_THREADS * CH_QPT) * (B > 0 ? B : 1);
  int S = (int)rslo_cdiv(1024, qblocks);
  const int maxS = (int)rslo_cdiv(M > 0 ? M : 1, 256);
  if (S > maxS) S = maxS;
  if (S < 1) S = 1;
  return S;
}

extern "C" size_t rslo_chamfer_grid_ws_bytes(int B, int N, int M);
extern "C" int rslo_chamfer_brute_nn(const float *xyz1, const float *xyz2, int B, int N, int M, const int32_t *ncnt,
                                     const int32_t *mcnt, float *dist, int32_t *idx, void *ws, size_t ws_bytes,
                                     void *stream);
extern "C" int rslo_chamfer_grid_nn(const float *xyz1, const float *xyz2, int B, int N, int M, const int32_t *ncnt,
                                    const int32_t *mcnt, float *dist, int32_t *idx, void *ws, size_t ws_bytes,
                                    void *stream);

static bool chamfer_use_grid(int N, int M) {
  const int force = rslo_tune(RSLO_TUNE_CHAMFER);
  if (force == 1) return false;
  if (force == 2) return true;
  return N >= 1024 && M >= 2048;
}

static size_t chamfer_brute_ws_bytes(int B, int N, int M) {
  return (size_t)chamfer_segments(B, N, M) * (size_t)(B > 0 ? B : 1) * (size_t)(N > 0 ? N : 1) * 8;
}

extern "C" size_t rslo_chamfer_ws_bytes(int B, int N, int M) {
  const size_t a = chamfer_brute_ws_bytes(B, N, M), g = rslo_chamfer_grid_ws_bytes(B, N, M);
  return a > g ? a : g;
}

extern "C" int rslo_chamfer_nn_ragged(const float *xyz1, const float *xyz2, int B, int N, int M,
                                      const int32_t *ncnt, const int32_t *mcnt, float *dist, int32_t *idx,
                                      void *ws, size_t ws_bytes, void *stream);

extern "C" int rslo_chamfer_nn(const float *xyz1, const float *xyz2, int B, int N, int M, float *dist,
                               int32_t *idx, void *ws, size_t ws_bytes, void *stream) {
  return rslo_chamfer_nn_ragged(xyz1, xyz2, B, N, M, nullptr, nullptr, dist, idx, ws, ws_bytes, stream);
}

extern "C" int rslo_chamfer_nn_ragged(const float *xyz1, const float *xyz2, int B, int N, int M,
                                      const int32_t *ncnt, const int32_t *mcnt, float *dist, int32_t *idx,
                                      void *ws, size_t ws_bytes, void *stream) {
  hipStream_t st = (hipStream_t)stream;
  RSLO_CHECK_ARG(B >= 0 && N >= 0 && M >= 1, "chamfer_nn: need M >= 1");
  if (B == 0 || N == 0) return RSLO_OK;
  if (chamfer_use_grid(N, M)) return rslo_chamfer_grid_nn(xyz1, xyz2, B, N, M, ncnt, mcnt, dist, idx, ws, ws_bytes, stream);
  return rslo_chamfer_brute_nn(xyz1, xyz2, B, N, M, ncnt, mcnt, dist, idx, ws, ws_bytes, stream);
}

extern "C" int rslo_chamfer_brute_nn(const float *xyz1, const float *xyz2, int B, int N, int M, const int32_t *ncnt,
                                     const int32_t *mcnt, float *dist, int32_t *idx, void *ws, size_t ws_bytes,
                                     void *stream) {
  hipStream_t st = (hipStream_t)stream;
  RSLO_CHECK_ARG(B >= 0 && N >= 0 && M >= 1, "chamfer_nn: need M >= 1");
  if (B == 0 || N == 0) return RSLO_OK;
  const int S = chamfer_segments(B, N, M);
  if (ws_bytes < chamfer_brute_ws_bytes(B, N, M)) {
    rslo_set_error("chamfer_nn: workspace too small");
    return RSLO_EWS;
  }
  const int seg_len = (int)rslo_cdiv(M, S);
  float *pdist = (float *)ws;
  int32_t *pidx = (int32_t *)(pdist + (int64_t)S * B * N);
  dim3 grid((unsigned)rslo_cdiv(N, CH_THREADS * CH_QPT), (unsigned)S, (unsigned)B);
  hipLaunchKernelGGL(k_chamfer_part, grid, dim3(CH_THREADS), 0, st, xyz1, xyz2, N, M, seg_len, S, mcnt, pdist,
                     pidx);
  hipLaunchKernelGGL(k_chamfer_merge, dim3((unsigned)rslo_cdiv(N, 256), (unsigned)B), dim3(256), 0, st, pdist,
                     pidx, N, S, ncnt, dist, idx);
  RSLO_CHECK_LAUNCH("chamfer_nn");
  return RSLO_OK;
}

__global__ void k_chamfer_grad(const float *__restrict__ xyz1, const float *__restrict__ xyz2, int N, int M,
                               const float *__restrict__ gd, const int32_t *__restrict__ idx,
                               float *__restrict__ g1, float *__restrict__ g2) {
  const int b = blockIdx.y;
  const int i = blockIdx.x * blockDim.x + threadIdx.x;
  if (i >= N) return;
  const float *p = xyz1 + ((int64_t)b * N + i) * 3;
  const int j2 = idx[(int64_t)b * N + i];
  const float *q = xyz2 + ((int64_t)b * M + j2) * 3;
  const float g = gd[(int64_t)b * N + i] * 2.f;
#pragma unroll
  for (int a = 0; a < 3; ++a) {
    const float v = g * (p[a] - q[a]);
    g1[((int64_t)b * N + i) * 3 + a] = v;
    atomicAdd(&g2[((int64_t)b * M + j2) * 3 + a], -v);
  }
}

extern "C" int rslo_chamfer_grad(const float *xyz1, const float *xyz2, int B, int N, int M,
                                 const float *graddist1, const int32_t *idx1, float *gradxyz1,
                                 float *gradxyz2, void *stream) {
  hipStream_t st = (hipStream_t)stream;
  RSLO_HIP(hipMemsetAsync(gradxyz2, 0, (size_t)B * M * 3 * sizeof(float), st));
  if (B == 0 || N == 0) return RSLO_OK;
  hipLaunchKernelGGL(k_chamfer_grad, dim3((unsigned)rslo_cdiv(N, 256), (unsigned)B), dim3(256), 0, st, xyz1,
                     xyz2, N, M, graddist1, idx1, gradxyz1, gradxyz2);
  RSLO_CHECK_LAUNCH("chamfer_grad");
  return RSLO_OK;
}
```

### rslo_amd/csrc/chamfer_grid.hip

```cpp
#include "rslo_common.h"

#pragma clang fp contract(off)

#define CG_XB 7
#define CG_YB 7
#define CG_ZB 3
#define CG_BINS (1 << (CG_XB + CG_YB + CG_ZB))
#define CG_CELL_XY 1.25f
#define CG_CELL_Z 2.5f
#define CG_TILE 64
#define CG_LDS_TILES 1024

__device__ __forceinline__ unsigned cg_spread7(unsigned v) {
  v &= 0x7f;
  v = (v | (v << 4)) & 0x070f;
  v = (v | (v << 2)) & 0x1333;
  v = (v | (v << 1)) & 0x1555;
  return v;
}

__device__ __forceinline__ int cg_key(float x, float y, float z) {
  int cx = (int)floorf((x + 80.0f) * (1.0f / CG_CELL_XY));
  int cy = (int)floorf((y + 80.0f) * (1.0f / CG_CELL_XY));
  int cz = (int)floorf((z + 10.0f) * (1.0f / CG_CELL_Z));
  cx = cx < 0 ? 0 : (cx > 127 ? 127 : cx);
  cy = cy < 0 ? 0 : (cy > 127 ? 127 : cy);
  cz = cz < 0 ? 0 : (cz > 7 ? 7 : cz);
  if (!(x == x)) cx = 0;
  if (!(y == y)) cy = 0;
  if (!(z == z)) cz = 0;
  return (int)(((cg_spread7((unsigned)cx) | (cg_spread7((unsigned)cy) << 1)) << CG_ZB) | (unsigned)cz);
}

__global__ void k_cg_hist(const float *__restrict__ xyz1, const float *__restrict__ xyz2, int N, int M,
                          const int32_t *__restrict__ ncnt, const int32_t *__restrict__ mcnt,
                          int32_t *__restrict__ hist, int B, float *__restrict__ dist, int32_t *__restrict__ idx) {
  const int cloud = blockIdx.z, b = blockIdx.y;
  const int n = cloud ? M : N;
  const int cnt = cloud ? (mcnt ? mcnt[b] : M) : (ncnt ? ncnt[b] : N);
  const int i = blockIdx.x * blockDim.x + threadIdx.x;
  if (i >= n) return;
  if (i >= cnt) {
    if (!cloud) {
      dist[(int64_t)b * N + i] = __builtin_inff();
      idx[(int64_t)b * N + i] = 0;
    }
    return;
  }
  const float *p = (cloud ? xyz2 : xyz1) + ((int64_t)b * n + i) * 3;
  atomicAdd(&hist[((int64_t)cloud * B + b) * CG_BINS + cg_key(p[0], p[1], p[2])], 1);
}

#define CG_CHUNK 1024
#define CG_NCHUNK (CG_BINS / CG_CHUNK)
__global__ __launch_bounds__(256) void k_cg_chunk_sums(const int32_t *__restrict__ hist, int32_t *__restrict__ sums) {
  __shared__ int32_t red[4];
  const int32_t *h = hist + ((int64_t)blockIdx.y * CG_NCHUNK + blockIdx.x) * CG_CHUNK;
  int32_t s = h[threadIdx.x] + h[threadIdx.x + 256] + h[threadIdx.x + 512] + h[threadIdx.x + 768];
  for (int d = 32; d > 0; d >>= 1) s += __shfl_down(s, d, 64);
  if ((threadIdx.x & 63) == 0) red[threadIdx.x >> 6] = s;
  __syncthreads();
  if (threadIdx.x == 0) sums[blockIdx.y * CG_NCHUNK + blockIdx.x] = red[0] + red[1] + red[2] + red[3];
}

__global__ __launch_bounds__(256) void k_cg_scan(int32_t *__restrict__ hist, const int32_t *__restrict__ sums) {
  __shared__ int32_t wsum[4];
  __shared__ int32_t carry_s;
  int32_t *h = hist + ((int64_t)blockIdx.y * CG_NCHUNK + blockIdx.x) * CG_CHUNK;
  int32_t c = 0;
  for (int k = threadIdx.x; k < (int)blockIdx.x; k += 256) c += sums[blockIdx.y * CG_NCHUNK + k];
  for (int d = 32; d > 0; d >>= 1) c += __shfl_down(c, d, 64);
  if ((threadIdx.x & 63) == 0) wsum[threadIdx.x >> 6] = c;
  __syncthreads();
  if (threadIdx.x == 0) carry_s = wsum[0] + wsum[1] + wsum[2] + wsum[3];
  __syncthreads();
  const int4 v = *reinterpret_cast<const int4 *>(h + threadIdx.x * 4);
  const int32_t tot = v.x + v.y + v.z + v.w;
  int32_t inc = tot;
  const int lane = threadIdx.x & 63;
  for (int d = 1; d < 64; d <<= 1) {
    const int32_t t = __shfl_up(inc, d, 64);
    if (lane >= d) inc += t;
  }
  __syncthreads();
  if (lane == 63) wsum[threadIdx.x >> 6] = inc;
  __syncthreads();
  int32_t base = carry_s + inc - tot;
  for (int w = 0; w < (int)(threadIdx.x >> 6); ++w) base += wsum[w];
  *reinterpret_cast<int4 *>(h + threadIdx.x * 4) = make_int4(base, base + v.x, base + v.x + v.y, base + v.x + v.y + v.z);
}

__global__ void k_cg_scatter(const float *__restrict__ xyz1, const float *__restrict__ xyz2, int N, int M, int Npad,
                             int Mpad, const int32_t *__restrict__ ncnt, const int32_t *__restrict__ mcnt,
                             const int32_t *__restrict__ off, int32_t *__restrict__ cursor, int B,
                             float4 *__restrict__ sq, float4 *__restrict__ st) {
  const int cloud = blockIdx.z, b = blockIdx.y;
  const int n = cloud ? M : N, npad = cloud ? Mpad : Npad;
  const int cnt = cloud ? (mcnt ? mcnt[b] : M) : (ncnt ? ncnt[b] : N);
  const int i = blockIdx.x * blockDim.x + threadIdx.x;
  float4 *dst = (cloud ? st : sq) + (int64_t)b * npad;
  if (i >= npad) return;
  if (i >= cnt) {
    const float inf = __builtin_inff();
    dst[i] = make_float4(inf, inf, inf, __int_as_float(-1));
    return;
  }
  const float *p = (cloud ? xyz2 : xyz1) + ((int64_t)b * n + i) * 3;
  const int64_t slot = ((int64_t)cloud * B + b) * CG_BINS + cg_key(p[0], p[1], p[2]);
  const int pos = off[slot] + atomicAdd(&cursor[slot], 1);
  dst[pos] = make_float4(p[0], p[1], p[2], __int_as_float(i));
}

__global__ __launch_bounds__(256) void k_cg_tiles(const float4 *__restrict__ st, int Mpad, int T,
                                                  float *__restrict__ boxes) {
  const int b = blockIdx.y;
  const int t = blockIdx.x * 4 + (threadIdx.x >> 6), lane = threadIdx.x & 63;
  if (t >= T) return;
  const float4 p = st[(int64_t)b * Mpad + t * CG_TILE + lane];
  const bool ok = __float_as_int(p.w) >= 0;
  const float inf = __builtin_inff();
  float lo[3] = {ok ? p.x : inf, ok ? p.y : inf, ok ? p.z : inf};
  float hi[3] = {ok ? p.x : -inf, ok ? p.y : -inf, ok ? p.z : -inf};
  for (int d = 32; d > 0; d >>= 1) {
#pragma unroll
    for (int k = 0; k < 3; ++k) {
      lo[k] = fminf(lo[k], __shfl_xor(lo[k], d, 64));
      hi[k] = fmaxf(hi[k], __shfl_xor(hi[k], d, 64));
    }
  }
  if (lane == 0) {
    float *o = boxes + ((int64_t)b * T + t) * 6;
    o[0] = lo[0]; o[1] = lo[1]; o[2] = lo[2];
    o[3] = hi[0]; o[4] = hi[1]; o[5] = hi[2];
  }
}

typedef unsigned long long u64;
#define CG_KEY_INIT ((u64)0x7f800000u << 32)

typedef float cg_f2 __attribute__((ext_vector_type(2)));
__device__ __forceinline__ void cg_eval_tile(const float4 *__restrict__ tile, float4 *slot, int lane, float qx, float qy,
                                             float qz, u64 &best) {
  const float4 mine = tile[lane];
  float *sf = reinterpret_cast<float *>(slot) + (lane >> 1) * 8 + (lane & 1);
  sf[0] = mine.x; sf[2] = mine.y; sf[4] = mine.z; sf[6] = mine.w;
  __builtin_amdgcn_wave_barrier();
  const cg_f2 qx2 = {qx, qx}, qy2 = {qy, qy}, qz2 = {qz, qz};
#pragma unroll 8
  for (int j = 0; j < CG_TILE / 2; ++j) {
    const float4 A = slot[2 * j], Bv = slot[2 * j + 1];
    const cg_f2 px = {A.x, A.y}, py = {A.z, A.w}, pz = {Bv.x, Bv.y};
    const cg_f2 dx = px - qx2, dy = py - qy2, dz = pz - qz2;
    const cg_f2 d = (dx * dx + dy * dy) + dz * dz;
    const u64 k0 = ((u64)(unsigned)__float_as_int(d.x) << 32) | (unsigned)__float_as_int(Bv.z);
    const u64 k1 = ((u64)(unsigned)__float_as_int(d.y) << 32) | (unsigned)__float_as_int(Bv.w);
    best = k0 < best ? k0 : best;
    best = k1 < best ? k1 : best;
  }
  __builtin_amdgcn_wave_barrier();
}

__device__ __forceinline__ float cg_box_lb(const float *bx, float qx, float qy, float qz) {
  const float ex = fmaxf(fmaxf(bx[0] - qx, qx - bx[3]), 0.0f);
  const float ey = fmaxf(fmaxf(bx[1] - qy, qy - bx[4]), 0.0f);
  const float ez = fmaxf(fmaxf(bx[2] - qz, qz - bx[5]), 0.0f);
  return (ex * ex + ey * ey) + ez * ez;
}

#define CG_GROUP 8
__global__ __launch_bounds__(256) void k_cg_search(const float4 *__restrict__ sq, const float4 *__restrict__ st,
                                                   const float *__restrict__ boxes, const int32_t *__restrict__ off,
                                                   int Npad, int Mpad, int T, int B, int S, int seg_tiles,
                                                   const int32_t *__restrict__ mcnt, int M, u64 *__restrict__ pkey) {
  __shared__ float sb[CG_LDS_TILES * 6];
  __shared__ float gb[(CG_LDS_TILES / CG_GROUP) * 6];
  __shared__ float4 slots[4][CG_TILE];
  const int b = blockIdx.z, seg = blockIdx.y, lane = threadIdx.x & 63, wid = threadIdx.x >> 6;
  const int qt = blockIdx.x * 4 + wid;
  const bool wave_on = qt * CG_TILE < Npad;
  const float4 q = wave_on ? sq[(int64_t)b * Npad + qt * CG_TILE + lane] : make_float4(0.f, 0.f, 0.f, __int_as_float(-1));
  const bool on = __float_as_int(q.w) >= 0;
  u64 best = CG_KEY_INIT;
  const int Mb = mcnt ? mcnt[b] : M;
  const int Tb = (Mb + CG_TILE - 1) / CG_TILE;
  const float4 *tb = st + (int64_t)b * Mpad;

  if (wave_on && Tb > 0) {
    int ts = on ? off[((int64_t)B + b) * CG_BINS + cg_key(q.x, q.y, q.z)] / CG_TILE : -1;
    ts = ts >= Tb ? Tb - 1 : ts;
    u64 todo = __ballot(on);
    int guard = 0;
    while (todo && guard++ < 12) {
      const int l = __builtin_ctzll(todo);
      const int t = __builtin_amdgcn_readlane(ts, l);
      cg_eval_tile(tb + t * CG_TILE, slots[wid], lane, q.x, q.y, q.z, best);
      todo &= ~__ballot(ts == t);
    }
  }

  const int tbeg = seg * seg_tiles, tend = (tbeg + seg_tiles < Tb) ? tbeg + seg_tiles : Tb;
  for (int t0 = tbeg; t0 < tend; t0 += CG_LDS_TILES) {
    const int nt = (tend - t0 < CG_LDS_TILES) ? (tend - t0) : CG_LDS_TILES;
    const int ng = (nt + CG_GROUP - 1) / CG_GROUP;
    __syncthreads();
    for (int e = threadIdx.x; e < nt * 6; e += 256) sb[e] = boxes[((int64_t)b * T + t0) * 6 + e];
    __syncthreads();
    for (int e = threadIdx.x; e < ng * 6; e += 256) {
      const int g = e / 6, k = e % 6;
      const int t1 = (g + 1) * CG_GROUP < nt ? (g + 1) * CG_GROUP : nt;
      float v = sb[g * CG_GROUP * 6 + k];
      for (int t = g * CG_GROUP + 1; t < t1; ++t) v = k < 3 ? fminf(v, sb[t * 6 + k]) : fmaxf(v, sb[t * 6 + k]);
      gb[e] = v;
    }
    __syncthreads();
    if (!wave_on) continue;
    for (int g = 0; g < ng; ++g) {
      float bd = __int_as_float((int)(best >> 32));
      if (__ballot(on && !(cg_box_lb(gb + g * 6, q.x, q.y, q.z) > bd)) == 0ull) continue;
      const int t1 = (g + 1) * CG_GROUP < nt ? (g + 1) * CG_GROUP : nt;
      for (int t = g * CG_GROUP; t < t1; ++t) {
        bd = __int_as_float((int)(best >> 32));
        if (__ballot(on && !(cg_box_lb(sb + t * 6, q.x, q.y, q.z) > bd)) == 0ull) continue;
        cg_eval_tile(tb + (t0 + t) * CG_TILE, slots[wid], lane, q.x, q.y, q.z, best);
      }
    }
  }
  if (wave_on) pkey[((int64_t)b * S + seg) * Npad + qt * CG_TILE + lane] = best;
}

__global__ void k_cg_merge(const float4 *__restrict__ sq, const u64 *__restrict__ pkey, int N, int Npad, int S,
                           float *__restrict__ dist, int32_t *__restrict__ idx) {
  const int b = blockIdx.y;
  const int i = blockIdx.x * blockDim.x + threadIdx.x;
  if (i >= Npad) return;
  const int qi = __float_as_int(sq[(int64_t)b * Npad + i].w);
  if (qi < 0) return;
  u64 best = pkey[((int64_t)b * S) * Npad + i];
  for (int s = 1; s < S; ++s) {
    const u64 k = pkey[((int64_t)b * S + s) * Npad + i];
    best = k < best ? k : best;
  }
  dist[(int64_t)b * N + qi] = __int_as_float((int)(best >> 32));
  idx[(int64_t)b * N + qi] = (int32_t)(unsigned)best;
}

static int cg_segments(int B, int N, int M) {
  const int forced = rslo_tune(RSLO_TUNE_CHAMFER_SEGMENTS);
  if (forced >= 1 && forced <= 8) {
    const int cap = (int)rslo_cdiv(rslo_cdiv(M > 0 ? M : 1, CG_TILE), CG_GROUP);
    return forced > cap ? (cap < 1 ? 1 : cap) : forced;
  }
  const int64_t qwaves = rslo_cdiv(N > 0 ? N : 1, CG_TILE) * (B > 0 ? B : 1);
  int S = (int)rslo_cdiv(8192, qwaves);
  const int maxS = (int)rslo_cdiv(rslo_cdiv(M > 0 ? M : 1, CG_TILE), 4 * CG_GROUP);
  if (S > maxS) S = maxS;
  if (S > 8) S = 8;
  return S < 1 ? 1 : S;
}

static inline int cg_pad(int n) { return (int)(rslo_cdiv(n > 0 ? n : 1, CG_TILE) * CG_TILE); }

extern "C" size_t rslo_chamfer_grid_ws_bytes(int B, int N, int M) {
  const size_t b = (size_t)(B > 0 ? B : 1);
  const size_t hist = 2 * b * CG_BINS * sizeof(int32_t);
  const size_t sorted = b * ((size_t)cg_pad(N) + (size_t)cg_pad(M)) * sizeof(float4);
  const size_t boxes = b * (size_t)(cg_pad(M) / CG_TILE) * 6 * sizeof(float);
  const size_t keys = b * (size_t)cg_segments(B, N, M) * (size_t)cg_pad(N) * sizeof(u64);
  return 2 * hist + sorted + boxes + 2 * b * CG_NCHUNK * sizeof(int32_t) + keys + 512;
}

extern "C" int rslo_chamfer_grid_nn(const float *xyz1, const float *xyz2, int B, int N, int M, const int32_t *ncnt,
                                    const int32_t *mcnt, float *dist, int32_t *idx, void *ws, size_t ws_bytes,
                                    void *stream) {
  hipStream_t s = (hipStream_t)stream;
  RSLO_CHECK_ARG(B >= 0 && N >= 0 && M >= 1, "chamfer_grid_nn: need M >= 1");
  if (B == 0 || N == 0) return RSLO_OK;
  if (ws_bytes < rslo_chamfer_grid_ws_bytes(B, N, M)) {
    rslo_set_error("chamfer_grid_nn: workspace too small");
    return RSLO_EWS;
  }
  const int Npad = cg_pad(N), Mpad = cg_pad(M), T = Mpad / CG_TILE;
  const size_t hist_n = (size_t)2 * B * CG_BINS;
  int32_t *hist = (int32_t *)ws;
  int32_t *cursor = hist + hist_n;
  float4 *sq = (float4 *)(((uintptr_t)(cursor + hist_n) + 15) & ~(uintptr_t)15);
  float4 *st = sq + (size_t)B * Npad;
  float *boxes = (float *)(st + (size_t)B * Mpad);
  int32_t *sums = (int32_t *)(boxes + (size_t)B * T * 6);
  u64 *pkey = (u64 *)(((uintptr_t)(sums + (size_t)2 * B * CG_NCHUNK) + 15) & ~(uintptr_t)15);
  const int S = cg_segments(B, N, M);
  const int seg_tiles = (int)(rslo_cdiv(rslo_cdiv(T, S), CG_GROUP) * CG_GROUP);
  RSLO_HIP(hipMemsetAsync(hist, 0, 2 * hist_n * sizeof(int32_t), s));
  const int nmax = N > M ? N : M, pmax = Npad > Mpad ? Npad : Mpad;
  hipLaunchKernelGGL(k_cg_hist, dim3((unsigned)rslo_cdiv(nmax, 256), (unsigned)B, 2), dim3(256), 0, s, xyz1, xyz2, N,
                     M, ncnt, mcnt, hist, B, dist, idx);
  hipLaunchKernelGGL(k_cg_chunk_sums, dim3(CG_NCHUNK, (unsigned)(2 * B)), dim3(256), 0, s, hist, sums);
  hipLaunchKernelGGL(k_cg_scan, dim3(CG_NCHUNK, (unsigned)(2 * B)), dim3(256), 0, s, hist, sums);
  hipLaunchKernelGGL(k_cg_scatter, dim3((unsigned)rslo_cdiv(pmax, 256), (unsigned)B, 2), dim3(256), 0, s, xyz1, xyz2,
                     N, M, Npad, Mpad, ncnt, mcnt, hist, cursor, B, sq, st);
  hipLaunchKernelGGL(k_cg_tiles, dim3((unsigned)rslo_cdiv(T, 4), (unsigned)B), dim3(256), 0, s, st, Mpad, T, boxes);
  hipLaunchKernelGGL(k_cg_search, dim3((unsigned)rslo_cdiv(Npad / CG_TILE, 4), (unsigned)S, (unsigned)B), dim3(256), 0, s,
                     sq, st, boxes, hist, Npad, Mpad, T, B, S, seg_tiles, mcnt, M, pkey);
  hipLaunchKernelGGL(k_cg_merge, dim3((unsigned)rslo_cdiv(Npad, 256), (unsigned)B), dim3(256), 0, s, sq, pkey, N, Npad, S,
                     dist, idx);
  RSLO_CHECK_LAUNCH("chamfer_grid_nn");
  return RSLO_OK;
}
```

### rslo_amd/csrc/rslo_common.h

```cpp
#pragma once
#include <hip/hip_runtime.h>
#include <stdint.h>
#include <stdio.h>

#include "../../include/rslo_hip.h"

#define RSLO_EMPTY_KEY 0xFFFFFFFFu

extern "C" void rslo_set_error(const char *fmt, ...);

#define RSLO_CHECK_ARG(cond, ...)        \
  do {                                   \
    if (!(cond)) {                       \
      rslo_set_error(__VA_ARGS__);       \
      return RSLO_EINVAL;                \
    }                                    \
  } while (0)

#define RSLO_CHECK_LAUNCH(name)                                              \
  do {                                                                       \
    hipError_t e_ = hipGetLastError();                                       \
    if (e_ != hipSuccess) {                                                  \
      rslo_set_error("%s: %s", name, hipGetErrorString(e_));                 \
      return RSLO_ELAUNCH;                                                   \
    }                                                                        \
  } while (0)

#define RSLO_HIP(call)                                                       \
  do {                                                                       \
    hipError_t e_ = (call);                                                  \
    if (e_ != hipSuccess) {                                                  \
      rslo_set_error("%s: %s", #call, hipGetErrorString(e_));                \
      return RSLO_ELAUNCH;                                                   \
    }                                                                        \
  } while (0)

static inline int64_t rslo_cdiv(int64_t a, int64_t b) { return (a + b - 1) / b; }

enum RsloTune {
  RSLO_TUNE_CONV2D_WGRAD_S2_FULLRES,
  RSLO_TUNE_CONV2D_WGRAD_NB,
  RSLO_TUNE_CONV2D_WGRAD_WGS,
  RSLO_TUNE_CONV2D_FWD_TR,
  RSLO_TUNE_CONV2D_FWD_MTW,
  RSLO_TUNE_CONV2D_FWD_OCC,
  RSLO_TUNE_CONV2D_FWD_KC,
  RSLO_TUNE_CONV2D_FWD_LEAN,
  RSLO_TUNE_CONV2D_FWD_XSC,
  RSLO_TUNE_CONV2D_S2_MTW,
  RSLO_TUNE_CONV2D_S2_XSC,
  RSLO_TUNE_BN_SMALL_RC,
  RSLO_TUNE_SPCONV_RBW,
  RSLO_TUNE_SPCONV_KS,
  RSLO_TUNE_SPCONV_V,
  RSLO_TUNE_SPCONV_WGRAD_SPLIT,
  RSLO_TUNE_WGRAD_XCD,
  RSLO_TUNE_VFE_LDS,
  RSLO_TUNE_CHAMFER,
  RSLO_TUNE_CHAMFER_SEGMENTS,
  RSLO_TUNE_DENSE_TILED,
  RSLO_TUNE_CONV1X1_SPLIT,
  RSLO_TUNE_CONV2D_FWD_WL,
  RSLO_TUNE_COUNT
};
extern int g_rslo_tune[RSLO_TUNE_COUNT];
static inline int rslo_tune(RsloTune t) { return g_rslo_tune[t]; }

struct Dims3 {
  int d, h, w;
};
struct Int3 {
  int a, b, c;
};

__device__ __forceinline__ uint32_t rslo_lin(int b, int z, int y, int x, Dims3 s) {
  return ((uint32_t)((b * s.d + z) * s.h + y)) * (uint32_t)s.w + (uint32_t)x;
}

__device__ __forceinline__ uint32_t rslo_hslot(uint32_t key, int shift) {
  return (key * 0x9E3779B1u) >> shift;
}

__device__ __forceinline__ int32_t rslo_hfind(const uint32_t *__restrict__ keys,
                                              const int32_t *__restrict__ vals, uint32_t mask,
                                              int shift, uint32_t key) {
  uint32_t s = rslo_hslot(key, shift);
  while (true) {
    uint32_t k = keys[s];
    if (k == key) return vals[s];
    if (k == RSLO_EMPTY_KEY) return -1;
    s = (s + 1) & mask;
  }
}

typedef __bf16 rslo_bf16x2 __attribute__((ext_vector_type(2)));
typedef float rslo_f32x2 __attribute__((ext_vector_type(2)));

__device__ __forceinline__ unsigned rslo_pk_bf16_rn(float x0, float x1) {
  const rslo_f32x2 v = {x0, x1};
  return __builtin_bit_cast(unsigned, __builtin_convertvector(v, rslo_bf16x2));
}

struct RsloSplit2 {
  unsigned h, m, l;
};

__device__ __forceinline__ RsloSplit2 rslo_split2(float x0, float x1) {
  RsloSplit2 o;
  o.h = rslo_pk_bf16_rn(x0, x1);
  const float r0 = x0 - __uint_as_float(o.h << 16), r1 = x1 - __uint_as_float(o.h & 0xffff0000u);
  o.m = rslo_pk_bf16_rn(r0, r1);
  const float s0 = r0 - __uint_as_float(o.m << 16), s1 = r1 - __uint_as_float(o.m & 0xffff0000u);
  o.l = rslo_pk_bf16_rn(s0, s1);
  return o;
}

__device__ __forceinline__ void rslo_split1(float x, unsigned short &h, unsigned short &m, unsigned short &l) {
  const RsloSplit2 s = rslo_split2(x, 0.f);
  h = (unsigned short)(s.h & 0xffffu);
  m = (unsigned short)(s.m & 0xffffu);
  l = (unsigned short)(s.l & 0xffffu);
}

static inline int rslo_log2_i64(int64_t v) {
  int l = 0;
  while ((int64_t(1) << l) < v) ++l;
  return l;
}
```

### rslo_amd/csrc/tuning.hip

```cpp
#include <string.h>

#include "rslo_common.h"

int g_rslo_tune[RSLO_TUNE_COUNT] = {
     1,  2,  768,
     0,  0,  0,  0,  -1,
     0,  0,  0,  1,
     0,  0,  0,  1,  1,
     1,  0,  0,  1,
     1,  0};

static const char *const k_tune_names[RSLO_TUNE_COUNT] = {
    "conv2d_wgrad_s2_fullres", "conv2d_wgrad_nb", "conv2d_wgrad_wgs", "conv2d_fwd_tr", "conv2d_fwd_mtw", "conv2d_fwd_occ",
    "conv2d_fwd_kc", "conv2d_fwd_lean", "conv2d_fwd_xsc", "conv2d_s2_mtw", "conv2d_s2_xsc", "bn_small_rc",
    "spconv_rbw", "spconv_ks", "spconv_v", "spconv_wgrad_split", "wgrad_xcd", "vfe_lds", "chamfer", "chamfer_segments", "dense_tiled",
    "conv1x1_split", "conv2d_fwd_wl"};

static int tune_index(const char *name) {
  if (name)
    for (int i = 0; i < RSLO_TUNE_COUNT; ++i)
      if (strcmp(name, k_tune_names[i]) == 0) return i;
  return -1;
}

extern "C" int rslo_tuning_set(const char *name, int value) {
  const int i = tune_index(name);
  RSLO_CHECK_ARG(i >= 0, "rslo_tuning_set: unknown switch '%s'", name ? name : "(null)");
  g_rslo_tune[i] = value;
  return RSLO_OK;
}

extern "C" int rslo_tuning_get(const char *name, int *value) {
  const int i = tune_index(name);
  RSLO_CHECK_ARG(i >= 0 && value, "rslo_tuning_get: unknown switch '%s'", name ? name : "(null)");
  *value = g_rslo_tune[i];
  return RSLO_OK;
}

extern "C" const char *rslo_tuning_name(int index) {
  return (index >= 0 && index < RSLO_TUNE_COUNT) ? k_tune_names[index] : nullptr;
}
```

### rslo_amd/rslo/core/losses.py

```python
from abc import ABCMeta, abstractmethod

import apex.amp as amp
import kornia
import torch
from torch import nn

from rslo.layers.svd import SVDHead, kabsch_rotation
from rslo_amd import capi


class Loss(nn.Module):
    __metaclass__ = ABCMeta

    def __init__(self, loss_weight=1):
        super().__init__()
        self._loss_weight = loss_weight

    def forward(self, prediction_tensor, target_tensor, ignore_nan_targets=False, scope=None, **params):
        if ignore_nan_targets:
            target_tensor = torch.where(torch.isnan(target_tensor), prediction_tensor, target_tensor)
        ret = self._compute_loss(prediction_tensor, target_tensor, **params)
        if isinstance(ret, (list, tuple)):
            return [self._loss_weight * ret[0]] + list(ret[1:])
        return self._loss_weight * ret

    @abstractmethod
    @amp.float_function
    def _compute_loss(self, prediction_tensor, target_tensor, **params):
        pass


def _adaptive_reduce(loss_b, alpha, focal_gamma):
    fw = (torch.exp(-alpha) * loss_b) ** focal_gamma
    fw = fw / (torch.sum(fw) + 1e-12)
    return (fw * (torch.exp(-alpha) * loss_b)).sum() + alpha


class AdaptiveWeightedL2Loss(Loss):
    def __init__(self, init_alpha, learn_alpha=True, loss_weight=1, focal_gamma=0, balance_scale=1):
        super().__init__(loss_weight)
        self.learn_alpha = learn_alpha
        self.alpha = nn.Parameter(torch.Tensor([init_alpha]), requires_grad=learn_alpha)
        self.focal_gamma = focal_gamma

    def _compute_loss(self, prediction_tensor, target_tensor, mask=None, alpha=None, focal_gamma=None):
        if focal_gamma is None:
            focal_gamma = self.focal_gamma
        mask = torch.ones_like(target_tensor) if mask is None else mask.expand_as(target_tensor)
        diff = prediction_tensor - target_tensor
        dims = list(range(1, prediction_tensor.dim()))
        loss_b = torch.sum(diff * diff * mask, dim=dims) / (torch.sum(mask, dim=dims) + 1e-12)
        return _adaptive_reduce(loss_b, self.alpha, focal_gamma)


class _PyramidL2Fn(torch.autograd.Function):

    @staticmethod
    def forward(ctx, tq, geom, masks, *preds):
        preds = [p.contiguous() for p in preds]
        loss_b, den = capi.pyramid_l2_fwd(preds, masks, tq, *geom)
        ctx.save_for_backward(tq, den, *preds)
        ctx.masks, ctx.geom = masks, geom
        return loss_b

    @staticmethod
    def backward(ctx, g):
        tq, den, *preds = ctx.saved_tensors
        dpreds = capi.pyramid_l2_bwd(preds, ctx.masks, tq, *ctx.geom, g.contiguous(), den)
        return (None, None, None, *dpreds)


class _LossTailFn(torch.autograd.Function):

    @staticmethod
    def _desc(t_pred, q_pred, pyr, pair, alphas, meta):
        d = capi.LossTail()
        d.t_pred, d.q_pred = t_pred.data_ptr(), q_pred.data_ptr()
        d.t_tgt, d.q_tgt = meta["t_tgt"].data_ptr(), meta["q_tgt"].data_ptr()
        d.alpha_T, d.alpha_R, d.alpha_pT, d.alpha_pR, d.alpha_C = [a.data_ptr() for a in alphas]
        d.pyr_loss_b = pyr.data_ptr() if pyr is not None else None
        d.pair_loss = pair.data_ptr() if pair is not None else None
        d.B, d.L = t_pred.shape[0], (pyr.shape[0] if pyr is not None else 0)
        d.n_pairs = pair.shape[0] if pair is not None else 0
        d.w_T, d.w_R, d.w_pT, d.w_pR, d.c_scale = meta["w"]
        for i, w in enumerate(meta["level_w"]):
            d.level_w[i] = w
        return d

    @staticmethod
    def forward(ctx, t_pred, q_pred, pyr, pair, aT, aR, apT, apR, aC, meta):
        t_pred, q_pred = t_pred.contiguous(), q_pred.contiguous()
        pyr = pyr.contiguous() if pyr is not None else None
        pair = pair.contiguous() if pair is not None else None
        alphas = (aT, aR, apT, apR, aC)
        out = capi.loss_tail_fwd(_LossTailFn._desc(t_pred, q_pred, pyr, pair, alphas, meta), t_pred.device)
        ctx.save_for_backward(t_pred, q_pred, pyr, pair, *alphas, meta["t_tgt"], meta["q_tgt"])
        ctx.meta = meta
        ctx.mark_non_differentiable(out)
        ctx.set_materialize_grads(False)
        return out[0:1], out

    @staticmethod
    def backward(ctx, g, _g_terms):
        t_pred, q_pred, pyr, pair, aT, aR, apT, apR, aC, _, _ = ctx.saved_tensors
        if g is None:
            return (None,) * 10
        desc = _LossTailFn._desc(t_pred, q_pred, pyr, pair, (aT, aR, apT, apR, aC), ctx.meta)
        d_t, d_q, d_pyr, d_pair, d_a = capi.loss_tail_bwd(desc, g.reshape(1).contiguous(), desc.B, desc.L, desc.n_pairs)
        need = ctx.needs_input_grad
        ptrs = [a.data_ptr() for a in (aT, aR, apT, apR, aC)]
        da = [d_a[i:i + 1] if need[4 + i] and ptrs[i] not in ptrs[:i] else None for i in range(5)]
        return d_t, d_q, d_pyr, d_pair, da[0], da[1], da[2], da[3], da[4], None


def loss_tail(raw, level_w):
    meta = {"t_tgt": raw["t_tgt"].detach().contiguous().float(), "q_tgt": raw["q_tgt"].detach().contiguous().float(),
            "w": tuple(float(v) for v in raw["w"]), "level_w": [float(v) for v in level_w]}
    return _LossTailFn.apply(raw["t_pred"], raw["q_pred"], raw["pyr_loss_b"], raw["pair_loss"], *raw["alphas"], meta)


class _PadRowsFn(torch.autograd.Function):

    @staticmethod
    def forward(ctx, src, off, length, Lmax):
        src = src.contiguous()
        ctx.save_for_backward(off, length)
        ctx.n = src.shape[0]
        return capi.pad_rows_fwd(src, off, length, Lmax)

    @staticmethod
    def backward(ctx, g):
        off, length = ctx.saved_tensors
        return capi.pad_rows_bwd(g.contiguous(), off, length, ctx.n), None, None, None


class _PairRowsFn(torch.autograd.Function):

    @staticmethod
    def forward(ctx, feats, conf, off, length, Lmax):
        ctx.save_for_backward(off, length)
        ctx.n = conf.shape[0]
        xyz, nrm, cov = capi.pair_rows_fwd(feats.contiguous(), conf.contiguous(), off, length, Lmax)
        ctx.mark_non_differentiable(xyz, nrm)
        ctx.set_materialize_grads(False)
        return xyz, nrm, cov

    @staticmethod
    def backward(ctx, _gx, _gn, g):
        off, length = ctx.saved_tensors
        if g is None:
            return None, None, None, None, None
        return None, capi.pad_rows_bwd(g.contiguous(), off, length, ctx.n), None, None, None


def pair_rows(feats, conf, off, length, Lmax):
    return _PairRowsFn.apply(feats.detach(), conf, off, length, Lmax)


def pad_rows(src, off, length, Lmax):
    if src.is_cuda:
        return _PadRowsFn.apply(src, off, length, Lmax)
    B = off.shape[0]
    out = src.new_zeros(B, Lmax, src.shape[1])
    for b, (o, n) in enumerate(zip(off.tolist(), length.tolist())):
        out[b, :n] = src[o:o + n]
    return out


class _RigidMoveFn(torch.autograd.Function):

    @staticmethod
    def forward(ctx, x, R, t):
        ctx.save_for_backward(x)
        ctx.has_t = t is not None
        return capi.transform_rows(x, R.contiguous(), None if t is None else t.contiguous())

    @staticmethod
    def backward(ctx, g):
        (x,) = ctx.saved_tensors
        dR, dt = capi.transform_rows_bwd(x, g.contiguous())
        return None, dR, (dt if ctx.has_t else None)


def rigid_move(x, R, t=None):
    if x.is_cuda:
        return _RigidMoveFn.apply(x.detach(), R, t)
    out = x.detach() @ R.transpose(-1, -2)
    return out if t is None else out + t[:, None]


class _QuatToRotFn(torch.autograd.Function):
    @staticmethod
    def forward(ctx, q):
        q = q.contiguous()
        ctx.save_for_backward(q)
        return capi.quat_to_rot(q)

    @staticmethod
    def backward(ctx, gR):
        (q,) = ctx.saved_tensors
        return capi.quat_to_rot_bwd(q, gR.contiguous())


def quat_wxyz_to_rot(q):
    if q.is_cuda and q.dtype == torch.float32 and q.dim() == 2:
        return _QuatToRotFn.apply(q)
    import torchplus
    return kornia.quaternion_to_rotation_matrix(torchplus.roll(q, shift=-1, dim=-1))


def icp_pose_targets(res_r, res_t, R_pred, T_pred, with_tq=False):
    R_pred, T_pred = R_pred.detach(), T_pred.detach()
    if res_r.is_cuda:
        return capi.pose_targets(res_r.contiguous(), res_t.contiguous(), R_pred.contiguous(), T_pred.contiguous(),
                                 with_tq=with_tq)
    assert not with_tq
    import torchplus
    rot = kornia.rotation_matrix_to_quaternion((res_r @ R_pred).contiguous())
    rot = torchplus.roll(rot, 1, dim=-1)
    rot = rot * torch.sign(rot[:, 0:1])
    return rot, (res_r @ T_pred[..., None] + res_t[..., None]).squeeze(-1)


_const_cache = {}


def _const(values, device):
    key = (tuple(float(v) for v in values), str(device))
    t = _const_cache.get(key)
    if t is None:
        t = _const_cache[key] = torch.tensor(key[0], dtype=torch.float32, device=device)
    return t


def pyramid_l2_losses(preds, masks, tq, geom, loss_T, loss_R):
    masks = [m.detach().contiguous().float() for m in masks]
    loss_b = _PyramidL2Fn.apply(tq.detach().contiguous().float(), geom, masks, *[p.float() for p in preds])
    return _adaptive_reduce_pair(loss_b, loss_T, loss_R)


def _adaptive_reduce_pair(loss_b, loss_T, loss_R):
    B = loss_b.shape[-2]
    alpha = torch.cat([loss_T.alpha, loss_R.alpha])
    y = torch.exp(-alpha) * loss_b
    if loss_T.focal_gamma == 0 and loss_R.focal_gamma == 0:
        out = y.sum(-2) / (B + 1e-12) + alpha
    else:
        cols = []
        for k, g in enumerate((loss_T.focal_gamma, loss_R.focal_gamma)):
            fw = y[..., k] ** g
            fw = fw / (fw.sum(-1, keepdim=True) + 1e-12)
            cols.append((fw * y[..., k]).sum(-1))
        out = torch.stack(cols, -1) + alpha
    return torch.cat([out[..., :1] * loss_T._loss_weight, out[..., 1:] * loss_R._loss_weight], -1)


def pose_l2_losses(T_pred, T_tgt, R_pred, R_tgt, loss_T, loss_R):
    d = torch.cat([T_pred - T_tgt, R_pred - R_tgt], 1)
    sq = d * d
    sq_t, sq_r = sq.split([3, 4], dim=1)
    loss_b = torch.stack([sq_t.sum(1) / (3 + 1e-12), sq_r.sum(1) / (4 + 1e-12)], 1)
    out = _adaptive_reduce_pair(loss_b, loss_T, loss_R)
    return out[0:1], out[1:2]


def span_cov2(cov_param):
    shp = cov_param.shape[:-1]
    p = cov_param.reshape(-1, 7)
    l1 = p[:, 0]
    l2 = l1 + p[:, 1]
    l3 = l2 + p[:, 2]
    lam = torch.stack([l1, l2, l3], -1)
    pq = p[:, 3:]
    q = pq / (torch.norm(pq, dim=-1, keepdim=True) + 1e-9)
    V = kornia.quaternion_to_rotation_matrix(q)
    sigma = (V * lam[:, None, :]) @ V.transpose(-1, -2)
    return sigma.reshape(*shp, 3, 3), V.reshape(*shp, 3, 3)


def sym3_inverse_det(S):
    a, b, c = S[..., 0, 0], S[..., 0, 1], S[..., 0, 2]
    d, e, f = S[..., 1, 0], S[..., 1, 1], S[..., 1, 2]
    g, h, i = S[..., 2, 0], S[..., 2, 1], S[..., 2, 2]
    A, B, C_ = e * i - f * h, -(d * i - f * g), d * h - e * g
    det = a * A + b * B + c * C_
    adj = torch.stack([torch.stack([A, -(b * i - c * h), b * f - c * e], -1),
                       torch.stack([B, a * i - c * g, -(a * f - c * d)], -1),
                       torch.stack([C_, -(a * h - b * g), a * e - b * d], -1)], -2)
    return adj / det[..., None, None], det


def roi_threshold(dist, penalize_ratio):
    N = dist.shape[-1]
    k = 1 + int(N * penalize_ratio)
    m, _ = torch.kthvalue(dist, min(k, N), dim=-1, keepdim=True)
    return torch.max(m, torch.ones_like(m))


def roi_threshold_ragged(dist, counts, penalize_ratio):
    k = 1 + (counts.double() * penalize_ratio).long()
    k = torch.minimum(k, counts.long()).clamp_min(1)
    srt, _ = torch.sort(dist, dim=-1)
    m = srt.gather(1, (k - 1)[:, None])
    return torch.max(m, torch.ones_like(m))


def points_roi(dist, penalize_ratio):
    return dist < roi_threshold(dist, penalize_ratio)


class _CovResidualFn(torch.autograd.Function):

    @staticmethod
    def forward(ctx, p1, tgt, cov1, cov2, idx, dist, thr, Rd, reg):
        p1, tgt, cov1, cov2 = p1.contiguous(), tgt.contiguous(), cov1.contiguous(), cov2.contiguous()
        Rd = Rd.contiguous()
        loss, cnt = capi.cov_residual_fwd(p1, tgt, cov1, cov2, idx, dist, thr, Rd, reg)
        ctx.save_for_backward(p1, tgt, cov1, cov2, idx, dist, thr, Rd, cnt)
        ctx.reg = reg
        return loss

    @staticmethod
    def backward(ctx, g):
        p1, tgt, cov1, cov2, idx, dist, thr, Rd, cnt = ctx.saved_tensors
        gp1, gtgt, gcov1, gcov2 = capi.cov_residual_bwd(p1, tgt, cov1, cov2, idx, dist, thr, Rd, g.contiguous(), cnt,
                                                        ctx.reg, need_gp1=ctx.needs_input_grad[0])
        return gp1, gtgt, gcov1, gcov2, None, None, None, None, None


def gather_rows(x, idx):
    tail = x.shape[2:]
    flat = x.reshape(x.shape[0], x.shape[1], -1)
    out = torch.gather(flat, 1, idx[..., None].expand(-1, -1, flat.shape[-1]))
    return out.reshape(x.shape[0], idx.shape[1], *tail)


def masked_kabsch(src, tgt, w, mask):
    m = mask.to(src.dtype)
    cnt = m.sum(-1, keepdim=True).clamp_min(1.0)
    cs = (src * m[..., None]).sum(1) / cnt
    ct = (tgt * m[..., None]).sum(1) / cnt
    sc = (src - cs[:, None]) * (m * w)[..., None]
    H = sc.transpose(1, 2) @ (tgt - ct[:, None])
    R = kabsch_rotation(H)
    t = -(R @ cs[..., None]) + ct[..., None]
    Rt = R.transpose(-1, -2).contiguous()
    return Rt, -(Rt @ t).squeeze(-1)


class ChamferL2Loss(Loss):
    def __init__(self, *args, **kwargs):
        raise NotImplementedError("ChamferL2Loss is not configured on the RSLO hot path")


class Aleat5_1ChamferL2NormalWeightedALLSVDLoss(Loss):
    def __init__(self, init_alpha=0, learn_alpha=False, loss_weight=1, focal_gamma=0, n_samples=-1,
                 penalize_ratio=0.95, sample_block_size=(0.1, 1, 1), norm=True, pred_downsample_ratio=1,
                 reg_weight=0.001, sph_weight=1):
        super().__init__(loss_weight=loss_weight)
        from thirdparty.chamfer_distance.chamfer_distance import OneDirectionChamferDistanceWithIdx
        self.learn_alpha = learn_alpha
        self.alpha = nn.Parameter(torch.Tensor([init_alpha]), requires_grad=learn_alpha)
        self.focal_gamma = focal_gamma
        self.n_samples = n_samples
        self.penalize_ratio = penalize_ratio
        self.sample_block_size = sample_block_size
        self.cd = OneDirectionChamferDistanceWithIdx()
        self.norm = norm
        self.svd = SVDHead()
        if pred_downsample_ratio < 1:
            raise NotImplementedError("pred_downsample_ratio < 1 is not configured on the RSLO hot path")
        self.pred_downsample_ratio = pred_downsample_ratio
        self.reg_weight = reg_weight
        self.sph_weight = sph_weight
        self.use_fused = True

    def _points_roi(self, dist, penalize_ratio=0.95, dist_threshold=None):
        if dist_threshold is not None:
            return dist < dist_threshold
        return points_roi(dist, penalize_ratio)

    def _associate(self, xyz_pred, target, normal_pred):
        with torch.no_grad():
            dist, idx = self.cd(xyz_pred.detach(), target.detach())
            idx = idx.long()
            roi = points_roi(dist, self.penalize_ratio)
        assoc = gather_rows(target, idx)
        w = nn.functional.cosine_similarity(normal_pred, (assoc - xyz_pred).detach(), dim=-1).abs()
        return idx, roi, assoc, w

    def _compute_loss(self, xyz_pred, xyz_target, cov_pred, cov_target, R_pred, t_pred, normal_pred,
                      normal_target, mask=None, alpha=None, focal_gamma=None, icp_iter=1):
        assert mask is None, "per-point masks are not used by the configured loss (voxel_odom_net.py:706)"
        loss_b, res_r, res_t = self.pair_losses(xyz_pred, xyz_target, cov_pred, cov_target, R_pred, t_pred,
                                                normal_pred, normal_target, icp_iter=icp_iter)
        return self.reduce(loss_b, focal_gamma), res_r, res_t

    def reduce(self, loss_b, focal_gamma=None):
        if focal_gamma is None:
            focal_gamma = self.focal_gamma
        loss = loss_b.sum() / loss_b.shape[0]
        fw = (torch.exp(-self.alpha) * loss) ** focal_gamma
        fw = fw / (torch.sum(fw) + 1e-12)
        return (fw * (torch.exp(-self.alpha) * loss)).sum() + self.alpha

    def pair_losses(self, xyz_pred, xyz_target, cov_pred, cov_target, R_pred, t_pred, normal_pred,
                    normal_target, icp_iter=1, counts=None, counts_host=None):
        if xyz_pred.is_cuda and self.use_fused:
            return self.pair_losses_fused(xyz_pred, xyz_target, cov_pred, cov_target, R_pred, normal_pred, icp_iter,
                                          counts)
        if counts_host is None:
            return self.pair_losses_torch(xyz_pred, xyz_target, cov_pred, cov_target, R_pred, t_pred, normal_pred,
                                          normal_target, icp_iter)
        outs = [self.pair_losses_torch(xyz_pred[b:b + 1, :n], xyz_target[b:b + 1, :n], cov_pred[b:b + 1, :n],
                                       cov_target[b:b + 1, :n], R_pred[b:b + 1], t_pred[b:b + 1],
                                       normal_pred[b:b + 1, :n], normal_target[b:b + 1, :n], icp_iter)
                for b, n in enumerate(counts_host)]
        return torch.cat([o[0] for o in outs]), torch.cat([o[1] for o in outs]), torch.cat([o[2] for o in outs])

    def _thr(self, dist, counts):
        if dist.is_cuda:
            return capi.roi_threshold(dist.contiguous(), counts, self.penalize_ratio)
        if counts is None:
            return roi_threshold(dist, self.penalize_ratio).reshape(-1).contiguous()
        return roi_threshold_ragged(dist, counts, self.penalize_ratio).reshape(-1).contiguous()

    def pair_losses_fused(self, xyz_pred, xyz_target, cov_pred, cov_target, R_pred, normal_pred, icp_iter=1,
                          counts=None):
        p1 = xyz_pred.detach().contiguous().float()
        n1 = normal_pred.detach().contiguous().float()
        tgt0 = xyz_target.detach().contiguous().float()
        dist, idx = capi.chamfer_nn(p1, tgt0, ncnt=counts, mcnt=counts)
        thr = self._thr(dist, counts)
        loss_b = _CovResidualFn.apply(xyz_pred, xyz_target, cov_pred, cov_target, idx, dist, thr,
                                      R_pred.detach(), float(self.reg_weight))
        B = p1.shape[0]
        if icp_iter > 0:
            res_r = torch.empty(B, 3, 3, device=p1.device, dtype=torch.float32)
            res_t = torch.empty(B, 3, device=p1.device, dtype=torch.float32)
        else:
            res_r = torch.eye(3, device=p1.device, dtype=torch.float32).repeat(B, 1, 1)
            res_t = torch.zeros(B, 3, device=p1.device, dtype=torch.float32)
        cur = tgt0
        for it in range(icp_iter):
            capi.icp_step(p1, n1, cur, idx, dist, thr, res_r, res_t, first=(it == 0))
            if it < icp_iter - 1:
                cur = capi.transform_points(tgt0, res_r, res_t)
                dist, idx = capi.chamfer_nn(p1, cur, ncnt=counts, mcnt=counts)
                thr = self._thr(dist, counts)
        return loss_b, res_r, res_t

    def pair_losses_torch(self, xyz_pred, xyz_target, cov_pred, cov_target, R_pred, t_pred, normal_pred,
                          normal_target, icp_iter=1):
        sig1, _ = span_cov2(cov_pred)
        sig2, _ = span_cov2(cov_target)

        idx, roi, xyz_assoc, weight = self._associate(xyz_pred, xyz_target, normal_pred)
        sig2_assoc = gather_rows(sig2, idx)
        diff_vec = xyz_pred - xyz_assoc
        Rd = R_pred.detach()[:, None]
        sigma = sig1 + Rd @ sig2_assoc @ Rd.transpose(-1, -2)
        sigma_inv, det = sym3_inverse_det(sigma)
        sq = (diff_vec.unsqueeze(-2) @ sigma_inv @ diff_vec.unsqueeze(-1)).reshape(diff_vec.shape[:2])
        m = roi.to(sq.dtype)
        cnt = m.sum(-1)
        zero = torch.zeros_like(sq)
        loss_b = torch.where(roi, sq, zero).sum(-1) / cnt \
            + self.reg_weight * torch.where(roi, 0.5 * torch.log(det), zero).sum(-1) / cnt

        with torch.no_grad():
            B = xyz_pred.shape[0]
            src = xyz_pred.detach()
            tgt0 = xyz_target.detach()
            res_r = torch.eye(3, device=src.device, dtype=src.dtype).expand(B, 3, 3).contiguous()
            res_t = torch.zeros(B, 3, device=src.device, dtype=src.dtype)
            assoc, w, sel = xyz_assoc.detach(), weight.detach(), roi
            for it in range(icp_iter):
                R, t = masked_kabsch(src, assoc, w * w, sel)
                res_r = R @ res_r
                res_t = (R @ res_t[..., None]).squeeze(-1) + t
                if it < icp_iter - 1:
                    moved = tgt0 @ res_r.transpose(-1, -2) + res_t[:, None]
                    _, sel, assoc, w = self._associate(src, moved, normal_pred.detach())

        return loss_b, res_r, res_t


from rslo import reference_fallback as _reference_fallback

__getattr__ = _reference_fallback(__name__)
```

### rslo_amd/switches.py

```python

SWITCHES = {
    "RSLO_HIPCC_EXTRA": ("", "location", "extra hipcc flags of rslo_amd/build.py (experiments: -DSPC_PREW_ALL=1); part of the source hash"),
    "RSLO_HIP_LIB": ("", "location", "path of librslo_hip.so (default: next to the package)"),
    "RSLO_REFERENCE_ROOT": ("", "location", "a reference checkout whose non-hot-path modules (protos, logging, ...) are forwarded to"),
    "RSLO_SYNCBN_EXCHANGE": ("auto", "mode", "SyncBN statistics exchange: auto | device | host | rccl (rslo_amd/peer.py)"),
    "RSLO_SYNCBN_FUSED_PEER": ("1", "mode", "0: multi-rank SyncBN as statistics kernel -> exchange kernel -> apply kernel on every map, instead of ONE kernel per direction that meets its peers per channel (rslo_bn2d_fwd_peer) on the register-cached maps"),
    "RSLO_FORCE_SYNCBN_PATH": ("0", "mode", "1: a one-rank process group runs the multi-rank SyncBN path (world-size-1 peer comm): what a rank of an N > 1 job executes, measurable on one GPU (bench.py multirank_path)"),
    "RSLO_SYNCBN_MAX_BATCH": ("0", "mode", "largest per-rank batch of a job whose ranks may hold different batch sizes: the single-launch / three-launch choice of every SyncBN layer is then made for that size on every rank (0: each rank's own batch, equal on all ranks)"),
    "RSLO_PEER_TIMEOUT_MS": ("600000", "mode", "how long a SyncBN exchange waits for a peer before it poisons the statistics with NaN and raises the comm's status (polled once per step)"),
    "RSLO_SYNCBN_HP_GROUP": ("0", "mode", "1: a dedicated high-priority RCCL group for the SyncBN collectives (only when they are collectives)"),
    "RSLO_OVERLAP_GRADS": ("1", "mode", "0: one gradient bucket after backward instead of the overlapped head bucket"),
    "RSLO_WGRAD_STREAM": ("1", "mode", "0: dense weight gradients on the issuing stream instead of the leaf stream (rslo_amd/streams.py)"),
    "RSLO_DEFER_WGRAD_REDUCE": ("8", "mode", "the partials -> gradient stage of the weight gradients: n >= 2: one launch per n layers and stream (rslo_amd/streams.py, csrc/wgrad_reduce.hip; same bits), 1: one launch per stream at the end of the backward pass, 0: one launch per layer"),
    "RSLO_SHARE_SIDE_STREAM": ("auto", "mode", "dense weight gradients on the covariance branch's stream (three streams of ours, the fourth slot left to the collective library's: a fifth active stream halves the step's speed, profiles/r06_fifth_stream.txt): auto = in a process with an initialised process group, 1 = always, 0 = never"),
    "RSLO_COV_STREAM": ("1", "mode", "0: covariance branch on the training stream; 2: issued behind the whole head (A/B)"),
    "RSLO_HOST_LEAD": ("1", "mode", "forward passes the issuing thread may run ahead of the GPU (0: unbounded)"),
    "RSLO_NATIVE_PLAN": ("1", "mode", "0: Python-issued voxelization + rulebook plan instead of rslo_plan_encoder"),
    "RSLO_PRESPLIT_EARLY": ("1", "mode", "0: head weight operands split in front of the head instead of beside the encoder"),
    "RSLO_PLAN_GATE": ("loss", "mode", "where a structure-plan job of a coming batch may start on the GPU: 'loss' where the current step's loss begins, 'head' at the head's small-map stages, 'fwd_end' behind the loss, 'none' at once"),
    "RSLO_HEAD_GRAPH": ("fwd", "mode", "0: the head issued launch by launch; fwd: the BEV head's training forward replayed from one hipGraph, its backward issued launch by launch over the capture's retained autograd graph; 1 / full: backward replayed as well (rslo_amd/headgraph.py; same bits as the eager pass)"),
    "RSLO_HEAD_GRAPH_INPUT": ("direct", "mode", "direct: the encoder's dense() writes the BEV map into the static input of the head's replayed graph; copy: into a fresh tensor that is then copied there (70 MB per step; A/B runs)"),
    "RSLO_HEAD_GRAPH_COV": ("before", "mode", "where the covariance branch's forward is issued when the head is a replayed graph: 'before' or 'after' the head"),
    "RSLO_INFER_PLAN_STREAMS": ("1", "mode", "side streams the inference runner (rslo_amd/inference.py) issues the coming scans' structure plans on, round-robin"),
    "RSLO_INFER_PLAN_PRIORITY": ("", "mode", "HIP stream priority of the inference runner's structure-plan stream(s) (default: the runtime's default; measured without effect on C2)"),
    "RSLO_PREFETCH_PRIORITY": ("", "mode", "HIP stream priority of the structure-plan stream (default: lowest)"),
    "RSLO_SWITCH_INTERVAL": ("0.0002", "mode", "interpreter switch interval while helper threads issue GPU work"),
    "RSLO_SPCONV_SPLIT": ("1", "path", "0: 32/64-channel sparse layers on the fp32-MFMA kernels instead of the split-bf16 ones"),
    "RSLO_ROW_ORDER": ("1", "path", "0: no mask-sorted tile order on the transposed tables"),
    "RSLO_CONV2D_PASSES": ("wfd", "path", "which passes of the dense 3x3 layers run on conv2d.hip (w, f, d); empty: the library"),
    "RSLO_CONV2D_S2": ("1", "path", "0: stride-2 layers on the library"),
    "RSLO_FUSED_BN": ("1", "path", "0: torch BatchNorm / SyncBatchNorm instead of bn2d.hip (auto: only with > 1 rank)"),
    "RSLO_FUSED_BLOCK": ("1", "path", "0: a BasicBlock as layer-by-layer autograd nodes instead of one node"),
    "RSLO_FUSED_HEAD_TAIL": ("1", "path", "0: the head's element-wise tail as torch ops instead of headtail.hip"),
    "RSLO_FUSED_LOSS_TAIL": ("1", "path", "0: loss assembly as torch ops instead of k_loss_tail_*"),
    "RSLO_FUSED_OPTIM": ("1", "path", "0: torch.optim.Adam without fused=True under the wrapper"),
    "RSLO_HIP_OPTIM": ("1", "path", "0: torch clip_grad_norm_ + Adam instead of optim.hip"),
    "RSLO_CAT_UPSAMPLE": ("1", "path", "0: torch cat + Upsample in front of a deblock"),
    "RSLO_PAIR_BEV": ("1", "path", "0: per-frame BEV maps + torch.cat instead of dense() writing the pair layout"),
    "RSLO_BEV_DISPLAY": ("1", "path", "0: logged display maps as torch ops"),
    "RSLO_HEAD_NHWC": ("0", "path", "bench.py only: the dense head in channels-last on the library path (measured slower)"),
}
```

Measured before the change: 373.5 frame-pairs/s.

## Reuse chamfer query-side grid index across ICP rounds and seed from previous partners

After: 367.8 frame-pairs/s. -1.5%, worse.

```diff
diff --git a/include/rslo_hip.h b/include/rslo_hip.h
--- a/include/rslo_hip.h
+++ b/include/rslo_hip.h
@@ -256,6 +256,13 @@
 RSLO_API int rslo_chamfer_grid_nn(const float *xyz1, const float *xyz2, int B, int N, int M, const int32_t *ncnt,
                                   const int32_t *mcnt, float *dist, int32_t *idx, void *ws, size_t ws_bytes,
                                   void *stream);
+RSLO_API size_t rslo_chamfer_grid_qindex_bytes(int B, int N);
+RSLO_API int rslo_chamfer_nn_keep(const float *xyz1, const float *xyz2, int B, int N, int M, const int32_t *ncnt,
+                                  const int32_t *mcnt, float *dist, int32_t *idx, void *qindex, size_t qindex_bytes,
+                                  int *kept, void *ws, size_t ws_bytes, void *stream);
+RSLO_API int rslo_chamfer_grid_requery(const void *qindex, size_t qindex_bytes, const float *xyz2, int B, int N, int M,
+                                       const int32_t *ncnt, const int32_t *mcnt, const int32_t *prev_idx, float *dist,
+                                       int32_t *idx, void *ws, size_t ws_bytes, void *stream);
 RSLO_API int rslo_chamfer_grad(const float *xyz1, const float *xyz2, int B, int N, int M,
                       const float *graddist1, const int32_t *idx1, float *gradxyz1 ,
                       float *gradxyz2 , void *stream);
diff --git a/rslo_amd/capi.py b/rslo_amd/capi.py
--- a/rslo_amd/capi.py
+++ b/rslo_amd/capi.py
@@ -76,6 +76,9 @@
     "rslo_chamfer_brute_nn": (C.c_int, [_vp, _vp, _i, _i, _i, _vp, _vp, _vp, _vp, _vp, _sz, _vp]),
     "rslo_chamfer_grid_ws_bytes": (_sz, [_i, _i, _i]),
     "rslo_chamfer_grid_nn": (C.c_int, [_vp, _vp, _i, _i, _i, _vp, _vp, _vp, _vp, _vp, _sz, _vp]),
+    "rslo_chamfer_grid_qindex_bytes": (_sz, [_i, _i]),
+    "rslo_chamfer_nn_keep": (C.c_int, [_vp, _vp, _i, _i, _i, _vp, _vp, _vp, _vp, _vp, _sz, _vp, _vp, _sz, _vp]),
+    "rslo_chamfer_grid_requery": (C.c_int, [_vp, _sz, _vp, _i, _i, _i, _vp, _vp, _vp, _vp, _vp, _vp, _sz, _vp]),
     "rslo_chamfer_grad": (C.c_int, [_vp, _vp, _i, _i, _i, _vp, _vp, _vp, _vp, _vp]),
     "rslo_cov_residual_ws_bytes": (_sz, [_i, _i]),
     "rslo_cov_residual_fwd": (C.c_int, [_vp] * 8 + [_i, _i, _i, _f, _vp, _sz, _vp, _vp, _vp]),
@@ -941,6 +944,49 @@
     return dist, idx
 
 
+class ChamferQueryIndex:
+    __slots__ = ("buf", "B", "N", "ncnt")
+
+    def __init__(self, buf, B, N, ncnt):
+        self.buf, self.B, self.N, self.ncnt = buf, B, N, ncnt
+
+
+def chamfer_nn_keep(xyz1, xyz2, ncnt=None, mcnt=None):
+    B, N, _ = xyz1.shape
+    M = xyz2.shape[1]
+    dev = xyz1.device
+    dist = torch.empty((B, N), dtype=torch.float32, device=dev)
+    idx = torch.empty((B, N), dtype=torch.int32, device=dev)
+    qb = lib().rslo_chamfer_grid_qindex_bytes(B, N)
+    buf = _ws(qb, dev)
+    wsb = lib().rslo_chamfer_ws_bytes(B, N, M)
+    ws = _ws(wsb, dev)
+    kept = C.c_int(0)
+    _chk(lib().rslo_chamfer_nn_keep(_ptr(xyz1, torch.float32, "xyz1"), _ptr(xyz2, torch.float32, "xyz2"), B, N, M,
+                                    _ptr(ncnt, torch.int32, "ncnt"), _ptr(mcnt, torch.int32, "mcnt"), _ptr(dist), _ptr(idx),
+                                    _ptr(buf), qb, C.addressof(kept), _ptr(ws), wsb, _stream()), "rslo_chamfer_nn_keep")
+    return dist, idx, (ChamferQueryIndex(buf, B, N, ncnt) if kept.value else None)
+
+
+def chamfer_requery(qindex, xyz2, prev_idx=None, mcnt=None):
+    B, N = qindex.B, qindex.N
+    if xyz2.shape[0] != B:
+        raise RsloHipError("chamfer_requery: %d pairs, the query index has %d" % (xyz2.shape[0], B))
+    if prev_idx is not None and tuple(prev_idx.shape) != (B, N):
+        raise RsloHipError("chamfer_requery: prev_idx must be [%d, %d]" % (B, N))
+    M = xyz2.shape[1]
+    dev = xyz2.device
+    dist = torch.empty((B, N), dtype=torch.float32, device=dev)
+    idx = torch.empty((B, N), dtype=torch.int32, device=dev)
+    wsb = lib().rslo_chamfer_grid_ws_bytes(B, N, M)
+    ws = _ws(wsb, dev)
+    _chk(lib().rslo_chamfer_grid_requery(_ptr(qindex.buf), qindex.buf.numel(), _ptr(xyz2, torch.float32, "xyz2"), B, N, M,
+                                         _ptr(qindex.ncnt, torch.int32, "ncnt"), _ptr(mcnt, torch.int32, "mcnt"),
+                                         _ptr(prev_idx, torch.int32, "prev_idx"), _ptr(dist), _ptr(idx), _ptr(ws), wsb,
+                                         _stream()), "rslo_chamfer_grid_requery")
+    return dist, idx
+
+
 def estimate_normals(points, radius=0.6, max_nn=30, viewpoint=None, zero_vertical=False, out=None, counts=None, ws=None):
     src = _ptr(points, torch.float32, "points")
     if points.dim() != 2 or points.shape[1] < 3:
diff --git a/rslo_amd/csrc/chamfer.hip b/rslo_amd/csrc/chamfer.hip
--- a/rslo_amd/csrc/chamfer.hip
+++ b/rslo_amd/csrc/chamfer.hip
@@ -197,6 +197,23 @@
   return RSLO_OK;
 }
 
+extern "C" int rslo_chamfer_grid_nn_keep(const float *xyz1, const float *xyz2, int B, int N, int M, const int32_t *ncnt,
+                                         const int32_t *mcnt, float *dist, int32_t *idx, void *qindex,
+                                         size_t qindex_bytes, void *ws, size_t ws_bytes, void *stream);
+
+extern "C" int rslo_chamfer_nn_keep(const float *xyz1, const float *xyz2, int B, int N, int M, const int32_t *ncnt,
+                                    const int32_t *mcnt, float *dist, int32_t *idx, void *qindex, size_t qindex_bytes,
+                                    int *kept, void *ws, size_t ws_bytes, void *stream) {
+  RSLO_CHECK_ARG(B >= 0 && N >= 0 && M >= 1 && kept, "chamfer_nn_keep: need M >= 1 and kept");
+  *kept = 0;
+  if (B == 0 || N == 0) return RSLO_OK;
+  if (!chamfer_use_grid(N, M)) return rslo_chamfer_brute_nn(xyz1, xyz2, B, N, M, ncnt, mcnt, dist, idx, ws, ws_bytes, stream);
+  const int rc = rslo_chamfer_grid_nn_keep(xyz1, xyz2, B, N, M, ncnt, mcnt, dist, idx, qindex, qindex_bytes, ws, ws_bytes,
+                                           stream);
+  *kept = rc == RSLO_OK;
+  return rc;
+}
+
 __global__ void k_chamfer_grad(const float *__restrict__ xyz1, const float *__restrict__ xyz2, int N, int M,
                                const float *__restrict__ gd, const int32_t *__restrict__ idx,
                                float *__restrict__ g1, float *__restrict__ g2) {
diff --git a/rslo_amd/csrc/chamfer_grid.hip b/rslo_amd/csrc/chamfer_grid.hip
--- a/rslo_amd/csrc/chamfer_grid.hip
+++ b/rslo_amd/csrc/chamfer_grid.hip
@@ -10,6 +10,7 @@
 #define CG_CELL_Z 2.5f
 #define CG_TILE 64
 #define CG_LDS_TILES 1024
+#define CG_SEED_NEAR2 (0.25f * CG_CELL_XY * CG_CELL_XY)
 
 __device__ __forceinline__ unsigned cg_spread7(unsigned v) {
   v &= 0x7f;
@@ -32,43 +33,50 @@
   return (int)(((cg_spread7((unsigned)cx) | (cg_spread7((unsigned)cy) << 1)) << CG_ZB) | (unsigned)cz);
 }
 
+__device__ __forceinline__ int64_t cg_hist_at(int cloud, int b, int B) { return ((int64_t)cloud * 2 * B + b) * CG_BINS; }
+__device__ __forceinline__ int64_t cg_cursor_at(int cloud, int b, int B) {
+  return ((int64_t)cloud * 2 * B + B + b) * CG_BINS;
+}
+
 __global__ void k_cg_hist(const float *__restrict__ xyz1, const float *__restrict__ xyz2, int N, int M,
                           const int32_t *__restrict__ ncnt, const int32_t *__restrict__ mcnt,
-                          int32_t *__restrict__ hist, int B, float *__restrict__ dist, int32_t *__restrict__ idx) {
-  const int cloud = blockIdx.z, b = blockIdx.y;
+                          int32_t *__restrict__ hist, int B, int z0, float *__restrict__ dist,
+                          int32_t *__restrict__ idx) {
+  const int cloud = blockIdx.z + z0, b = blockIdx.y;
   const int n = cloud ? M : N;
   const int cnt = cloud ? (mcnt ? mcnt[b] : M) : (ncnt ? ncnt[b] : N);
   const int i = blockIdx.x * blockDim.x + threadIdx.x;
-  if (i >= n) return;
-  if (i >= cnt) {
-    if (!cloud) {
-      dist[(int64_t)b * N + i] = __builtin_inff();
-      idx[(int64_t)b * N + i] = 0;
-    }
-    return;
-  }
+  if (cloud == z0 && i < N && i >= (ncnt ? ncnt[b] : N)) {
+    dist[(int64_t)b * N + i] = __builtin_inff();
+    idx[(int64_t)b * N + i] = 0;
+  }
+  if (i >= n || i >= cnt) return;
   const float *p = (cloud ? xyz2 : xyz1) + ((int64_t)b * n + i) * 3;
-  atomicAdd(&hist[((int64_t)cloud * B + b) * CG_BINS + cg_key(p[0], p[1], p[2])], 1);
+  atomicAdd(&hist[cg_hist_at(cloud, b, B) + cg_key(p[0], p[1], p[2])], 1);
 }
 
 #define CG_CHUNK 1024
 #define CG_NCHUNK (CG_BINS / CG_CHUNK)
-__global__ __launch_bounds__(256) void k_cg_chunk_sums(const int32_t *__restrict__ hist, int32_t *__restrict__ sums) {
+__global__ __launch_bounds__(256) void k_cg_chunk_sums(const int32_t *__restrict__ hist, int B, int y0,
+                                                       int32_t *__restrict__ sums) {
   __shared__ int32_t red[4];
-  const int32_t *h = hist + ((int64_t)blockIdx.y * CG_NCHUNK + blockIdx.x) * CG_CHUNK;
+  const int seg = blockIdx.y + y0;
+  const int32_t *h = hist + cg_hist_at(seg / B, seg % B, B) + (int64_t)blockIdx.x * CG_CHUNK;
   int32_t s = h[threadIdx.x] + h[threadIdx.x + 256] + h[threadIdx.x + 512] + h[threadIdx.x + 768];
   for (int d = 32; d > 0; d >>= 1) s += __shfl_down(s, d, 64);
   if ((threadIdx.x & 63) == 0) red[threadIdx.x >> 6] = s;
   __syncthreads();
-  if (threadIdx.x == 0) sums[blockIdx.y * CG_NCHUNK + blockIdx.x] = red[0] + red[1] + red[2] + red[3];
-}
-
-__global__ __launch_bounds__(256) void k_cg_scan(int32_t *__restrict__ hist, const int32_t *__restrict__ sums) {
+  if (threadIdx.x == 0) sums[seg * CG_NCHUNK + blockIdx.x] = red[0] + red[1] + red[2] + red[3];
+}
+
+__global__ __launch_bounds__(256) void k_cg_scan(int32_t *__restrict__ hist, int B, int y0,
+                                                 const int32_t *__restrict__ sums) {
   __shared__ int32_t wsum[4];
   __shared__ int32_t carry_s;
-  int32_t *h = hist + ((int64_t)blockIdx.y * CG_NCHUNK + blockIdx.x) * CG_CHUNK;
+  const int seg = blockIdx.y + y0;
+  int32_t *h = hist + cg_hist_at(seg / B, seg % B, B) + (int64_t)blockIdx.x * CG_CHUNK;
   int32_t c = 0;
-  for (int k = threadIdx.x; k < (int)blockIdx.x; k += 256) c += sums[blockIdx.y * CG_NCHUNK + k];
+  for (int k = threadIdx.x; k < (int)blockIdx.x; k += 256) c += sums[seg * CG_NCHUNK + k];
   for (int d = 32; d > 0; d >>= 1) c += __shfl_down(c, d, 64);
   if ((threadIdx.x & 63) == 0) wsum[threadIdx.x >> 6] = c;
   __syncthreads();
@@ -92,9 +100,9 @@
 
 __global__ void k_cg_scatter(const float *__restrict__ xyz1, const float *__restrict__ xyz2, int N, int M, int Npad,
                              int Mpad, const int32_t *__restrict__ ncnt, const int32_t *__restrict__ mcnt,
-                             const int32_t *__restrict__ off, int32_t *__restrict__ cursor, int B,
-                             float4 *__restrict__ sq, float4 *__restrict__ st) {
-  const int cloud = blockIdx.z, b = blockIdx.y;
+                             int32_t *__restrict__ hist, int B, int z0, float4 *__restrict__ sq,
+                             float4 *__restrict__ st) {
+  const int cloud = blockIdx.z + z0, b = blockIdx.y;
   const int n = cloud ? M : N, npad = cloud ? Mpad : Npad;
   const int cnt = cloud ? (mcnt ? mcnt[b] : M) : (ncnt ? ncnt[b] : N);
   const int i = blockIdx.x * blockDim.x + threadIdx.x;
@@ -106,16 +114,13 @@
     return;
   }
   const float *p = (cloud ? xyz2 : xyz1) + ((int64_t)b * n + i) * 3;
-  const int64_t slot = ((int64_t)cloud * B + b) * CG_BINS + cg_key(p[0], p[1], p[2]);
-  const int pos = off[slot] + atomicAdd(&cursor[slot], 1);
+  const int key = cg_key(p[0], p[1], p[2]);
+  const int pos = hist[cg_hist_at(cloud, b, B) + key] + atomicAdd(&hist[cg_cursor_at(cloud, b, B) + key], 1);
   dst[pos] = make_float4(p[0], p[1], p[2], __int_as_float(i));
 }
 
-__global__ __launch_bounds__(256) void k_cg_tiles(const float4 *__restrict__ st, int Mpad, int T,
-                                                  float *__restrict__ boxes) {
-  const int b = blockIdx.y;
-  const int t = blockIdx.x * 4 + (threadIdx.x >> 6), lane = threadIdx.x & 63;
-  if (t >= T) return;
+__device__ __forceinline__ void cg_tile_box(const float4 *__restrict__ st, int Mpad, int T, int b, int t, int lane,
+                                            float *__restrict__ boxes) {
   const float4 p = st[(int64_t)b * Mpad + t * CG_TILE + lane];
   const bool ok = __float_as_int(p.w) >= 0;
   const float inf = __builtin_inff();
@@ -167,11 +172,64 @@
   return (ex * ex + ey * ey) + ez * ez;
 }
 
+__device__ __forceinline__ void cg_seed_tiles(const float4 q, bool on, bool want, const int32_t *__restrict__ toff,
+                                              const float4 *__restrict__ tb, int Tb, float4 *slot, int lane, u64 &best) {
+  int ts = on ? toff[cg_key(q.x, q.y, q.z)] / CG_TILE : -1;
+  ts = ts >= Tb ? Tb - 1 : ts;
+  u64 todo = __ballot(on && want);
+  int guard = 0;
+  while (todo && guard++ < 12) {
+    const int l = __builtin_ctzll(todo);
+    const int t = __builtin_amdgcn_readlane(ts, l);
+    cg_eval_tile(tb + t * CG_TILE, slot, lane, q.x, q.y, q.z, best);
+    todo &= ~__ballot(ts == t);
+  }
+}
+
+__global__ __launch_bounds__(256) void k_cg_tiles(const float4 *__restrict__ st, int Mpad, int T,
+                                                  float *__restrict__ boxes, int tile_blocks,
+                                                  const float4 *__restrict__ sq, int Npad, int N,
+                                                  const int32_t *__restrict__ hist, int B,
+                                                  const int32_t *__restrict__ mcnt, int M,
+                                                  const float *__restrict__ xyz2, const int32_t *__restrict__ prev,
+                                                  int seed_tiles, u64 *__restrict__ pseed) {
+  __shared__ float4 slots[4][CG_TILE];
+  const int b = blockIdx.y, lane = threadIdx.x & 63, wid = threadIdx.x >> 6;
+  if ((int)blockIdx.x < tile_blocks) {
+    const int t = blockIdx.x * 4 + wid;
+    if (t < T) cg_tile_box(st, Mpad, T, b, t, lane, boxes);
+    return;
+  }
+  const int qt = ((int)blockIdx.x - tile_blocks) * 4 + wid;
+  if (qt * CG_TILE >= Npad) return;
+  const float4 q = sq[(int64_t)b * Npad + qt * CG_TILE + lane];
+  const bool on = __float_as_int(q.w) >= 0;
+  const int Mb = mcnt ? mcnt[b] : M;
+  const int Tb = (Mb + CG_TILE - 1) / CG_TILE;
+  u64 best = CG_KEY_INIT;
+  if (prev && on && Mb > 0) {
+    int j = prev[(int64_t)b * N + __float_as_int(q.w)];
+    j = j < 0 ? 0 : (j >= Mb ? Mb - 1 : j);
+    const float *p = xyz2 + ((int64_t)b * M + j) * 3;
+    const float dx = p[0] - q.x, dy = p[1] - q.y, dz = p[2] - q.z;
+    const float d = (dx * dx + dy * dy) + dz * dz;
+    const u64 k = ((u64)(unsigned)__float_as_int(d) << 32) | (unsigned)j;
+    best = k < best ? k : best;
+  }
+  if (seed_tiles && Tb > 0) {
+    const bool want = seed_tiles == 1 || !(__int_as_float((int)(best >> 32)) <= CG_SEED_NEAR2);
+    cg_seed_tiles(q, on, want, hist + cg_hist_at(1, b, B), st + (int64_t)b * Mpad, Tb, slots[wid], lane, best);
+  }
+  pseed[(int64_t)b * Npad + qt * CG_TILE + lane] = best;
+}
+
 #define CG_GROUP 8
+template <bool OWN_SEEDS>
 __global__ __launch_bounds__(256) void k_cg_search(const float4 *__restrict__ sq, const float4 *__restrict__ st,
-                                                   const float *__restrict__ boxes, const int32_t *__restrict__ off,
+                                                   const float *__restrict__ boxes, const int32_t *__restrict__ hist,
                                                    int Npad, int Mpad, int T, int B, int S, int seg_tiles,
-                                                   const int32_t *__restrict__ mcnt, int M, u64 *__restrict__ pkey) {
+                                                   const int32_t *__restrict__ mcnt, int M,
+                                                   const u64 *__restrict__ pseed, u64 *__restrict__ pkey) {
   __shared__ float sb[CG_LDS_TILES * 6];
   __shared__ float gb[(CG_LDS_TILES / CG_GROUP) * 6];
   __shared__ float4 slots[4][CG_TILE];
@@ -185,17 +243,10 @@
   const int Tb = (Mb + CG_TILE - 1) / CG_TILE;
   const float4 *tb = st + (int64_t)b * Mpad;
 
-  if (wave_on && Tb > 0) {
-    int ts = on ? off[((int64_t)B + b) * CG_BINS + cg_key(q.x, q.y, q.z)] / CG_TILE : -1;
-    ts = ts >= Tb ? Tb - 1 : ts;
-    u64 todo = __ballot(on);
-    int guard = 0;
-    while (todo && guard++ < 12) {
-      const int l = __builtin_ctzll(todo);
-      const int t = __builtin_amdgcn_readlane(ts, l);
-      cg_eval_tile(tb + t * CG_TILE, slots[wid], lane, q.x, q.y, q.z, best);
-      todo &= ~__ballot(ts == t);
-    }
+  if (OWN_SEEDS) {
+    if (wave_on && Tb > 0) cg_seed_tiles(q, on, true, hist + cg_hist_at(1, b, B), tb, Tb, slots[wid], lane, best);
+  } else if (wave_on) {
+    best = pseed[(int64_t)b * Npad + qt * CG_TILE + lane];
   }
 
   const int tbeg = seg * seg_tiles, tend = (tbeg + seg_tiles < Tb) ? tbeg + seg_tiles : Tb;
@@ -265,44 +316,88 @@
   const size_t hist = 2 * b * CG_BINS * sizeof(int32_t);
   const size_t sorted = b * ((size_t)cg_pad(N) + (size_t)cg_pad(M)) * sizeof(float4);
   const size_t boxes = b * (size_t)(cg_pad(M) / CG_TILE) * 6 * sizeof(float);
-  const size_t keys = b * (size_t)cg_segments(B, N, M) * (size_t)cg_pad(N) * sizeof(u64);
+  const size_t keys = b * ((size_t)cg_segments(B, N, M) + 1) * (size_t)cg_pad(N) * sizeof(u64);
   return 2 * hist + sorted + boxes + 2 * b * CG_NCHUNK * sizeof(int32_t) + keys + 512;
 }
 
-extern "C" int rslo_chamfer_grid_nn(const float *xyz1, const float *xyz2, int B, int N, int M, const int32_t *ncnt,
-                                    const int32_t *mcnt, float *dist, int32_t *idx, void *ws, size_t ws_bytes,
-                                    void *stream) {
-  hipStream_t s = (hipStream_t)stream;
-  RSLO_CHECK_ARG(B >= 0 && N >= 0 && M >= 1, "chamfer_grid_nn: need M >= 1");
-  if (B == 0 || N == 0) return RSLO_OK;
+extern "C" size_t rslo_chamfer_grid_qindex_bytes(int B, int N) {
+  return (size_t)(B > 0 ? B : 1) * (size_t)cg_pad(N) * sizeof(float4);
+}
+
+static int cg_run(const char *who, const float *xyz1, const float *xyz2, int B, int N, int M, const int32_t *ncnt,
+                  const int32_t *mcnt, const int32_t *prev, bool requery, float4 *qindex, float *dist, int32_t *idx,
+                  void *ws, size_t ws_bytes, hipStream_t s) {
   if (ws_bytes < rslo_chamfer_grid_ws_bytes(B, N, M)) {
-    rslo_set_error("chamfer_grid_nn: workspace too small");
+    rslo_set_error("%s: workspace too small", who);
     return RSLO_EWS;
   }
   const int Npad = cg_pad(N), Mpad = cg_pad(M), T = Mpad / CG_TILE;
-  const size_t hist_n = (size_t)2 * B * CG_BINS;
+  const size_t half = (size_t)2 * B * CG_BINS;
   int32_t *hist = (int32_t *)ws;
-  int32_t *cursor = hist + hist_n;
-  float4 *sq = (float4 *)(((uintptr_t)(cursor + hist_n) + 15) & ~(uintptr_t)15);
-  float4 *st = sq + (size_t)B * Npad;
+  float4 *sq_ws = (float4 *)(((uintptr_t)(hist + 2 * half) + 15) & ~(uintptr_t)15);
+  float4 *sq = qindex ? qindex : sq_ws;
+  float4 *st = sq_ws + (size_t)B * Npad;
   float *boxes = (float *)(st + (size_t)B * Mpad);
   int32_t *sums = (int32_t *)(boxes + (size_t)B * T * 6);
   u64 *pkey = (u64 *)(((uintptr_t)(sums + (size_t)2 * B * CG_NCHUNK) + 15) & ~(uintptr_t)15);
   const int S = cg_segments(B, N, M);
+  u64 *pseed = pkey + (size_t)B * S * Npad;
   const int seg_tiles = (int)(rslo_cdiv(rslo_cdiv(T, S), CG_GROUP) * CG_GROUP);
-  RSLO_HIP(hipMemsetAsync(hist, 0, 2 * hist_n * sizeof(int32_t), s));
-  const int nmax = N > M ? N : M, pmax = Npad > Mpad ? Npad : Mpad;
-  hipLaunchKernelGGL(k_cg_hist, dim3((unsigned)rslo_cdiv(nmax, 256), (unsigned)B, 2), dim3(256), 0, s, xyz1, xyz2, N,
-                     M, ncnt, mcnt, hist, B, dist, idx);
-  hipLaunchKernelGGL(k_cg_chunk_sums, dim3(CG_NCHUNK, (unsigned)(2 * B)), dim3(256), 0, s, hist, sums);
-  hipLaunchKernelGGL(k_cg_scan, dim3(CG_NCHUNK, (unsigned)(2 * B)), dim3(256), 0, s, hist, sums);
-  hipLaunchKernelGGL(k_cg_scatter, dim3((unsigned)rslo_cdiv(pmax, 256), (unsigned)B, 2), dim3(256), 0, s, xyz1, xyz2,
-                     N, M, Npad, Mpad, ncnt, mcnt, hist, cursor, B, sq, st);
-  hipLaunchKernelGGL(k_cg_tiles, dim3((unsigned)rslo_cdiv(T, 4), (unsigned)B), dim3(256), 0, s, st, Mpad, T, boxes);
-  hipLaunchKernelGGL(k_cg_search, dim3((unsigned)rslo_cdiv(Npad / CG_TILE, 4), (unsigned)S, (unsigned)B), dim3(256), 0, s,
-                     sq, st, boxes, hist, Npad, Mpad, T, B, S, seg_tiles, mcnt, M, pkey);
+  const int z0 = requery ? 1 : 0, nz = requery ? 1 : 2;
+  const bool seed_once = requery || rslo_tune(RSLO_TUNE_CHAMFER_SEED_ONCE) != 0;
+  const int rq_seeds = rslo_tune(RSLO_TUNE_CHAMFER_REQUERY_SEEDS);
+  const int seed_tiles = (!requery || !prev) ? 1 : (rq_seeds >= 0 && rq_seeds <= 2 ? rq_seeds : 2);
+  RSLO_HIP(hipMemsetAsync(hist + z0 * half, 0, nz * half * sizeof(int32_t), s));
+  const int nmax = N > M ? N : M, pmax = requery ? Mpad : (Npad > Mpad ? Npad : Mpad);
+  hipLaunchKernelGGL(k_cg_hist, dim3((unsigned)rslo_cdiv(nmax, 256), (unsigned)B, (unsigned)nz), dim3(256), 0, s, xyz1,
+                     xyz2, N, M, ncnt, mcnt, hist, B, z0, dist, idx);
+  hipLaunchKernelGGL(k_cg_chunk_sums, dim3(CG_NCHUNK, (unsigned)(nz * B)), dim3(256), 0, s, hist, B, z0 * B, sums);
+  hipLaunchKernelGGL(k_cg_scan, dim3(CG_NCHUNK, (unsigned)(nz * B)), dim3(256), 0, s, hist, B, z0 * B, sums);
+  hipLaunchKernelGGL(k_cg_scatter, dim3((unsigned)rslo_cdiv(pmax, 256), (unsigned)B, (unsigned)nz), dim3(256), 0, s,
+                     xyz1, xyz2, N, M, Npad, Mpad, ncnt, mcnt, hist, B, z0, sq, st);
+  const int tile_blocks = (int)rslo_cdiv(T, 4), seed_blocks = seed_once ? (int)rslo_cdiv(Npad / CG_TILE, 4) : 0;
+  hipLaunchKernelGGL(k_cg_tiles, dim3((unsigned)(tile_blocks + seed_blocks), (unsigned)B), dim3(256), 0, s, st, Mpad, T,
+                     boxes, tile_blocks, sq, Npad, N, hist, B, mcnt, M, xyz2, requery ? prev : nullptr, seed_tiles, pseed);
+  const dim3 sgrid((unsigned)rslo_cdiv(Npad / CG_TILE, 4), (unsigned)S, (unsigned)B);
+  if (seed_once)
+    hipLaunchKernelGGL(k_cg_search<false>, sgrid, dim3(256), 0, s, sq, st, boxes, hist, Npad, Mpad, T, B, S, seg_tiles, mcnt,
+                       M, pseed, pkey);
+  else
+    hipLaunchKernelGGL(k_cg_search<true>, sgrid, dim3(256), 0, s, sq, st, boxes, hist, Npad, Mpad, T, B, S, seg_tiles, mcnt,
+                       M, pseed, pkey);
   hipLaunchKernelGGL(k_cg_merge, dim3((unsigned)rslo_cdiv(Npad, 256), (unsigned)B), dim3(256), 0, s, sq, pkey, N, Npad, S,
                      dist, idx);
-  RSLO_CHECK_LAUNCH("chamfer_grid_nn");
+  RSLO_CHECK_LAUNCH(who);
   return RSLO_OK;
 }
+
+extern "C" int rslo_chamfer_grid_nn(const float *xyz1, const float *xyz2, int B, int N, int M, const int32_t *ncnt,
+                                    const int32_t *mcnt, float *dist, int32_t *idx, void *ws, size_t ws_bytes,
+                                    void *stream) {
+  RSLO_CHECK_ARG(B >= 0 && N >= 0 && M >= 1, "chamfer_grid_nn: need M >= 1");
+  if (B == 0 || N == 0) return RSLO_OK;
+  return cg_run("chamfer_grid_nn", xyz1, xyz2, B, N, M, ncnt, mcnt, nullptr, false, nullptr, dist, idx, ws, ws_bytes,
+                (hipStream_t)stream);
+}
+
+extern "C" int rslo_chamfer_grid_nn_keep(const float *xyz1, const float *xyz2, int B, int N, int M, const int32_t *ncnt,
+                                         const int32_t *mcnt, float *dist, int32_t *idx, void *qindex,
+                                         size_t qindex_bytes, void *ws, size_t ws_bytes, void *stream) {
+  RSLO_CHECK_ARG(B >= 0 && N >= 0 && M >= 1, "chamfer_grid_nn_keep: need M >= 1");
+  if (B == 0 || N == 0) return RSLO_OK;
+  RSLO_CHECK_ARG(qindex && ((uintptr_t)qindex & 15) == 0 && qindex_bytes >= rslo_chamfer_grid_qindex_bytes(B, N),
+                 "chamfer_grid_nn_keep: qindex must be 16-byte aligned and hold rslo_chamfer_grid_qindex_bytes(B, N)");
+  return cg_run("chamfer_grid_nn_keep", xyz1, xyz2, B, N, M, ncnt, mcnt, nullptr, false, (float4 *)qindex, dist, idx, ws,
+                ws_bytes, (hipStream_t)stream);
+}
+
+extern "C" int rslo_chamfer_grid_requery(const void *qindex, size_t qindex_bytes, const float *xyz2, int B, int N, int M,
+                                         const int32_t *ncnt, const int32_t *mcnt, const int32_t *prev_idx, float *dist,
+                                         int32_t *idx, void *ws, size_t ws_bytes, void *stream) {
+  RSLO_CHECK_ARG(B >= 0 && N >= 0 && M >= 1, "chamfer_grid_requery: need M >= 1");
+  if (B == 0 || N == 0) return RSLO_OK;
+  RSLO_CHECK_ARG(qindex && ((uintptr_t)qindex & 15) == 0 && qindex_bytes >= rslo_chamfer_grid_qindex_bytes(B, N),
+                 "chamfer_grid_requery: qindex must be the one rslo_chamfer_grid_nn_keep filled for this B, N");
+  return cg_run("chamfer_grid_requery", nullptr, xyz2, B, N, M, ncnt, mcnt, prev_idx, true, (float4 *)qindex, dist, idx,
+                ws, ws_bytes, (hipStream_t)stream);
+}
diff --git a/rslo_amd/csrc/rslo_common.h b/rslo_amd/csrc/rslo_common.h
--- a/rslo_amd/csrc/rslo_common.h
+++ b/rslo_amd/csrc/rslo_common.h
@@ -61,6 +61,8 @@
   RSLO_TUNE_DENSE_TILED,
   RSLO_TUNE_CONV1X1_SPLIT,
   RSLO_TUNE_CONV2D_FWD_WL,
+  RSLO_TUNE_CHAMFER_SEED_ONCE,
+  RSLO_TUNE_CHAMFER_REQUERY_SEEDS,
   RSLO_TUNE_COUNT
 };
 extern int g_rslo_tune[RSLO_TUNE_COUNT];
diff --git a/rslo_amd/csrc/tuning.hip b/rslo_amd/csrc/tuning.hip
--- a/rslo_amd/csrc/tuning.hip
+++ b/rslo_amd/csrc/tuning.hip
@@ -8,13 +8,13 @@
      0,  0,  0,  1,
      0,  0,  0,  1,  1,
      1,  0,  0,  1,
-     1,  0};
+     1,  0,  1,  2};
 
 static const char *const k_tune_names[RSLO_TUNE_COUNT] = {
     "conv2d_wgrad_s2_fullres", "conv2d_wgrad_nb", "conv2d_wgrad_wgs", "conv2d_fwd_tr", "conv2d_fwd_mtw", "conv2d_fwd_occ",
     "conv2d_fwd_kc", "conv2d_fwd_lean", "conv2d_fwd_xsc", "conv2d_s2_mtw", "conv2d_s2_xsc", "bn_small_rc",
     "spconv_rbw", "spconv_ks", "spconv_v", "spconv_wgrad_split", "wgrad_xcd", "vfe_lds", "chamfer", "chamfer_segments", "dense_tiled",
-    "conv1x1_split", "conv2d_fwd_wl"};
+    "conv1x1_split", "conv2d_fwd_wl", "chamfer_seed_once", "chamfer_requery_seeds"};
 
 static int tune_index(const char *name) {
   if (name)
diff --git a/rslo_amd/rslo/core/losses.py b/rslo_amd/rslo/core/losses.py
--- a/rslo_amd/rslo/core/losses.py
+++ b/rslo_amd/rslo/core/losses.py
@@ -1,3 +1,4 @@
+import os
 from abc import ABCMeta, abstractmethod
 
 import apex.amp as amp
@@ -374,6 +375,7 @@
         self.reg_weight = reg_weight
         self.sph_weight = sph_weight
         self.use_fused = True
+        self.chamfer_requery = os.environ.get("RSLO_CHAMFER_REQUERY", "1") != "0"
 
     def _points_roi(self, dist, penalize_ratio=0.95, dist_threshold=None):
         if dist_threshold is not None:
@@ -430,7 +432,11 @@
         p1 = xyz_pred.detach().contiguous().float()
         n1 = normal_pred.detach().contiguous().float()
         tgt0 = xyz_target.detach().contiguous().float()
-        dist, idx = capi.chamfer_nn(p1, tgt0, ncnt=counts, mcnt=counts)
+        qindex = None
+        if self.chamfer_requery and icp_iter > 1:
+            dist, idx, qindex = capi.chamfer_nn_keep(p1, tgt0, ncnt=counts, mcnt=counts)
+        else:
+            dist, idx = capi.chamfer_nn(p1, tgt0, ncnt=counts, mcnt=counts)
         thr = self._thr(dist, counts)
         loss_b = _CovResidualFn.apply(xyz_pred, xyz_target, cov_pred, cov_target, idx, dist, thr,
                                       R_pred.detach(), float(self.reg_weight))
@@ -446,7 +452,10 @@
             capi.icp_step(p1, n1, cur, idx, dist, thr, res_r, res_t, first=(it == 0))
             if it < icp_iter - 1:
                 cur = capi.transform_points(tgt0, res_r, res_t)
-                dist, idx = capi.chamfer_nn(p1, cur, ncnt=counts, mcnt=counts)
+                if qindex is not None:
+                    dist, idx = capi.chamfer_requery(qindex, cur, prev_idx=idx, mcnt=counts)
+                else:
+                    dist, idx = capi.chamfer_nn(p1, cur, ncnt=counts, mcnt=counts)
                 thr = self._thr(dist, counts)
         return loss_b, res_r, res_t
 
diff --git a/rslo_amd/switches.py b/rslo_amd/switches.py
--- a/rslo_amd/switches.py
+++ b/rslo_amd/switches.py
@@ -33,6 +33,7 @@
     "RSLO_FUSED_BLOCK": ("1", "path", "0: a BasicBlock as layer-by-layer autograd nodes instead of one node"),
     "RSLO_FUSED_HEAD_TAIL": ("1", "path", "0: the head's element-wise tail as torch ops instead of headtail.hip"),
     "RSLO_FUSED_LOSS_TAIL": ("1", "path", "0: loss assembly as torch ops instead of k_loss_tail_*"),
+    "RSLO_CHAMFER_REQUERY": ("1", "path", "0: every ICP round of the consistency loss searches its moved target from scratch instead of re-querying the kept query index from the previous round's partners (same bits)"),
     "RSLO_FUSED_OPTIM": ("1", "path", "0: torch.optim.Adam without fused=True under the wrapper"),
     "RSLO_HIP_OPTIM": ("1", "path", "0: torch clip_grad_norm_ + Adam instead of optim.hip"),
     "RSLO_CAT_UPSAMPLE": ("1", "path", "0: torch cat + Upsample in front of a deblock"),
```
